# berkeley-hipie/HIPIE

Measured on AMD Instinct MI355X. Metric: images/sec @1024x1024 ViT-H bs=8 (single-image inference hot path: box, class and mask logits), higher is better.
Workload: dtype f16x3 (split-fp16 operands, fp32 accumulate: fp32-class); 1 GPU; BASELINE.json configs[2]: vit_huge, 1024x1024, batch 8 per GPU, 80 class prompts (L=194), detection; global_batch=8, parallelism=dp1, precision_policy=split, launch=eager

## Files before the change

### hipie_amd/_lib.py

```python
import ctypes
import os

_HERE = os.path.dirname(os.path.abspath(__file__))
LIB_PATH = os.environ.get("HIPIE_LIB_PATH") or os.path.join(_HERE, "csrc", "libhipie_mi355.so")

c_p = ctypes.c_void_p
c_i = ctypes.c_int
c_l = ctypes.c_int64
c_f = ctypes.c_float

SIGNATURES = {
    "hipie_version": [],
    "hipie_last_error": [],
    "hipie_msda_forward": [c_p, c_p, c_p, c_p, c_p, c_p] + [c_i] * 8 + [c_p],
    "hipie_msda_fused_forward": [c_p, c_p, c_p, c_p, c_p, c_p, c_p] + [c_i] * 10 + [c_l, c_l, c_p],
    "hipie_msda_fused_forward_strided": [c_p, c_l, c_p, c_p, c_p, c_p, c_p, c_p] + [c_i] * 10 + [c_l, c_l, c_p],
    "hipie_flash_attn": [c_p, c_p, c_p, c_p] + [c_i] * 5 + [c_l] * 12 + [c_p, c_p, c_i, c_i, c_p, c_f, c_f, c_i, c_p],
    "hipie_vit_attn": [c_p, c_p, c_p, c_p] + [c_i] * 5 + [c_f, c_i, c_p],
    "hipie_vit_attn_fused": [c_p, c_p, c_p, c_p] + [c_i] * 5 + [c_f, c_i, c_p],
    "hipie_vit_attn_rel": [c_p, c_p, c_p, c_p] + [c_i] * 7 + [c_p],
    "hipie_bi_xattn": [c_p, c_p, c_p, c_p, c_p, c_p, c_p] + [c_i] * 5 + [c_f, c_i, c_p],
    "hipie_bi_xattn_ws": [c_p, c_p, c_p, c_p, c_p, c_p, c_p, c_p, c_l] + [c_i] * 5 + [c_f, c_i, c_p],
    "hipie_bi_xattn_workspace": [c_i] * 5,
    "hipie_mask_einsum": [c_p, c_p, c_p] + [c_i] * 6 + [c_p],
    "hipie_mask_einsum_workspace": [c_i, c_i, c_i],
    "hipie_mask_einsum_ws": [c_p, c_p, c_p, c_p, c_p, c_l] + [c_i] * 6 + [c_p],
    "hipie_mask_einsum16": [c_p, c_p, c_p, c_p, c_p] + [c_i] * 6 + [c_p],
    "hipie_dynamic_mask": [c_p, c_p, c_p, c_p] + [c_i] * 7 + [c_p],
    "hipie_dynamic_mask16": [c_p, c_p, c_p, c_p] + [c_i] * 7 + [c_p],
    "hipie_dynamic_mask_backward": [c_p] * 7 + [c_i] * 6 + [c_p],
    "hipie_vit_relpos": [c_p, c_p, c_p, c_p, c_p] + [c_i] * 6 + [c_p],
    "hipie_add_layernorm": [c_p, c_p, c_p, c_p, c_p, c_p, c_l, c_i, c_f, c_i, c_i, c_i, c_p],
    "hipie_layernorm_backward": [c_p] * 8 + [c_l, c_l, c_i, c_f, c_p],
    "hipie_layernorm_backward_ws_bytes": [c_l, c_i],
    "hipie_act_forward": [c_p, c_p, c_l, c_i, c_i, c_p],
    "hipie_act_backward": [c_p] * 6 + [c_l, c_i, c_i, c_p],
    "hipie_act_backward_ws_bytes": [c_l, c_i],
    "hipie_add_layernorm_sum": [c_p, c_p, c_p, c_p, c_p, c_p, c_p, c_p, c_l, c_i, c_f, c_i, c_i, c_i, c_p],
    "hipie_add_layernorm_rows": [c_p, c_p, c_p, c_p, c_p, c_p, c_l, c_i, c_f, c_i, c_i, c_i, c_p, c_p, c_p],
    "hipie_batched_nms": [c_p, c_p, c_p, c_p, c_p, c_i, c_i, c_f, c_i, c_p],
    "hipie_mask_finalize": [c_p, c_i, c_p] + [c_i] * 8 + [c_f, c_p, c_p],
    "hipie_sem_pan": [c_p] * 8 + [c_i] * 11 + [c_p],
    "hipie_sine_embed": [c_p, c_p, c_p, c_l, c_i, c_i, c_i, c_f, c_i, c_p],
    "hipie_box_refine": [c_p, c_p, c_p, c_l, c_f, c_i, c_p],
    "hipie_ref_point_mlp": [c_p, c_p, c_p, c_p, c_p, c_p, c_p, c_l, c_i, c_f, c_i, c_p],
    "hipie_box_head": [c_p, c_p, c_p, c_p, c_p, c_p, c_p, c_p, c_p, c_l, c_f, c_p],
    "hipie_add_layernorm_dec": [c_p, c_p, c_p, c_p, c_p, c_p, c_p, c_p, c_l, c_i, c_f, c_i, c_i, c_p],
    "hipie_add_cast": [c_p, c_p, c_p, c_l, c_i, c_p],
    "hipie_group_norm": [c_p, c_p, c_p, c_p, c_p, c_p, c_i, c_i, c_i, c_i, c_i, c_f, c_i, c_i, c_i, c_p],
    "hipie_gemm": [c_p, c_l, c_p, c_l, c_p, c_p, c_l, c_p, c_l, c_p] + [c_i] * 6 + [c_f, c_f, c_p],
    "hipie_gemm_f8x": [c_p, c_l, c_p, c_l, c_p, c_p, c_p, c_l, c_p, c_l, c_p] + [c_i] * 6 + [c_f, c_f, c_p],
    "hipie_to_f8x": [c_p, c_l, c_p, c_l, c_p, c_l, c_i, c_p],
    "hipie_gemm_ln": [c_p, c_l, c_p, c_l, c_p, c_p, c_l, c_p, c_p, c_f, c_p, c_l, c_p, c_l, c_i, c_i, c_i, c_f, c_p],
    "hipie_gemm_gather": [c_p, c_l, c_l, c_p, c_p, c_l, c_p, c_p, c_l, c_p, c_l, c_p] + [c_i] * 6 + [c_f, c_f, c_p],
    "hipie_vit_attn_split": [c_p, c_p, c_p, c_p] + [c_i] * 5 + [c_p],
    "hipie_msda_backward": [c_p] * 9 + [c_i] * 8 + [c_p],
    "hipie_msda_backward_ws": [c_p] * 9 + [c_i] * 8 + [c_p, c_l, c_p],
    "hipie_msda_backward_workspace": [c_i] * 6,
    "hipie_gemm_batched": [c_p, c_l, c_l, c_l, c_p, c_l, c_l, c_l, c_p, c_l, c_l, c_l] + [c_i] * 6 + [c_f, c_p],
    "hipie_gemm_batched_softmax_bias": [c_p, c_l, c_l, c_l, c_p, c_l, c_l, c_l, c_p, c_l, c_l, c_l] + [c_i] * 5 + [c_p, c_i, c_p, c_f, c_f, c_p],
    "hipie_gemm_batched_resid": [c_p, c_l, c_l, c_l, c_p, c_l, c_l, c_l, c_p, c_p, c_l, c_l, c_l, c_p, c_l, c_l, c_l] + [c_i] * 5 + [c_f, c_p],
    "hipie_gemm_batched_softmax": [c_p, c_l, c_l, c_l, c_p, c_l, c_l, c_l, c_p, c_l, c_l, c_l] + [c_i] * 5 + [c_p, c_i, c_f, c_f, c_p],
    "hipie_softmax_hl8": [c_p, c_l, c_p, c_l, c_l, c_i, c_i, c_p, c_l, c_f, c_p],
    "hipie_attn_f32": [c_p] * 5 + [c_i] * 5 + [c_l] * 6 + [c_f, c_p],
    "hipie_attn_split": [c_p] * 5 + [c_i] * 5 + [c_l] * 6 + [c_f, c_p],
    "hipie_attn_f32_rows": [c_p] * 5 + [c_i] * 5 + [c_l] * 6 + [c_f, c_p],
    "hipie_attn_split_rows": [c_p] * 5 + [c_i] * 5 + [c_l] * 6 + [c_f, c_p],
    "hipie_conv3x3_split": [c_p, c_l, c_p, c_p, c_p, c_l, c_l] + [c_i] * 6 + [c_p],
    "hipie_ffn_fused": [c_p, c_l, c_p, c_p, c_p, c_p, c_p, c_l, c_i, c_i, c_i, c_p],
    "hipie_topk": [c_p, c_l, c_i, c_i, c_i, c_p, c_p, c_p],
    "hipie_fill_rows": [c_p, c_l, c_p, c_l, c_p, c_l, c_p],
    "hipie_to_hl8": [c_p, c_l, c_p, c_l, c_l, c_i, c_i, c_f, c_p],
    "hipie_to_hl8_t": [c_p, c_l, c_p, c_l, c_l, c_i, c_l, c_f, c_p],
    "hipie_attn_train_forward": [c_p] * 8 + [c_i, c_i, c_p],
    "hipie_to_f16_pair": [c_p, c_l, c_p, c_p, c_l, c_i, c_i, c_p, c_p],
    "hipie_attn_train_backward": [c_p] * 13 + [c_i, c_i, c_p],
    "hipie_selftest": [c_i, c_p, c_p, c_p, c_p],
}

_lib = None


class HipieLibraryError(RuntimeError):
    pass


def load():
    global _lib
    if _lib is not None:
        return _lib
    if not os.path.exists(LIB_PATH):
        raise HipieLibraryError(
            "libhipie_mi355.so not found at %s -- build it with `make -C hipie_amd/csrc` (hipcc, gfx950). "
            "There is no PyTorch fallback for the hand-written kernels." % LIB_PATH)
    import torch
    try:
        lib = ctypes.CDLL(LIB_PATH)
    except OSError as e:
        raise HipieLibraryError("cannot load %s: %s" % (LIB_PATH, e))
    for name, argtypes in SIGNATURES.items():
        try:
            fn = getattr(lib, name)
        except AttributeError:
            raise HipieLibraryError("%s does not export %s (stale build?)" % (LIB_PATH, name))
        fn.argtypes = argtypes
        fn.restype = (ctypes.c_char_p if name == "hipie_last_error" else
                      ctypes.c_int64 if name in ("hipie_bi_xattn_workspace", "hipie_mask_einsum_workspace", "hipie_msda_backward_workspace",
                                                      "hipie_layernorm_backward_ws_bytes", "hipie_act_backward_ws_bytes") else ctypes.c_int)
    _lib = lib
    return lib


def check(rc, what):
    if rc != 0:
        msg = load().hipie_last_error()
        raise RuntimeError("%s failed (rc=%d): %s" % (what, rc, msg.decode() if msg else ""))
```

### hipie_amd/csrc/gemm.hip

```cpp
#include "gemm_tile.h"

namespace hipie {

template <typename T>
__global__ __launch_bounds__(256) void to_hl8_kernel(const T* __restrict__ x, f16_t* __restrict__ out, long rows, int K, long ldx, long ldo,
                                                     float scale) {
  const long gid = (long)blockIdx.x * 256 + threadIdx.x;
  const int gpr = K / 8;
  if (gid >= rows * gpr) return;
  const long r = gid / gpr;
  const int g = (int)(gid - r * gpr);
  const T* src = x + r * ldx + 8 * g;
  f16x8 h, l;
#pragma unroll
  for (int e = 0; e < 8; ++e) {
    f16_t hh, ll;
    hl_split((float)src[e] * scale, hh, ll);
    h[e] = hh;
    l[e] = ll;
  }
  f16_t* dst = out + r * ldo + 16 * g;
  *reinterpret_cast<f16x8*>(dst) = h;
  *reinterpret_cast<f16x8*>(dst + 8) = l;
}


constexpr int kTrRows = 128, kTrCols = 64;
__global__ __launch_bounds__(256) void to_hl8_t_kernel(const float* __restrict__ x, f16_t* __restrict__ out, long rows, int C, long ldx,
                                                       long ldo, long rows_p, float scale) {
  __shared__ float tile[kTrRows][kTrCols + 1];
  const long r0 = (long)blockIdx.x * kTrRows;
  const int c0 = blockIdx.y * kTrCols;
  const int tid = threadIdx.x;
  for (int k = tid; k < kTrRows * (kTrCols / 4); k += 256) {
    const int i = k / (kTrCols / 4), j = (k % (kTrCols / 4)) * 4;
    float v[4] = {0.f, 0.f, 0.f, 0.f};
    if (r0 + i < rows) {
      const float* src = x + (r0 + i) * ldx + c0 + j;
      if (c0 + j + 3 < C && (((uintptr_t)src) & 15) == 0) {
        const float4 q = *reinterpret_cast<const float4*>(src);
        v[0] = q.x; v[1] = q.y; v[2] = q.z; v[3] = q.w;
      } else {
        for (int e = 0; e < 4; ++e) v[e] = c0 + j + e < C ? src[e] : 0.f;
      }
    }
    for (int e = 0; e < 4; ++e) tile[i][j + e] = v[e];
  }
  __syncthreads();
  for (int u = tid; u < kTrCols * (kTrRows / 8); u += 256) {
    const int g = u % (kTrRows / 8), c = u / (kTrRows / 8);
    const long m = r0 + 8 * g;
    if (c0 + c >= C || m >= rows_p) continue;
    f16x8 h, l;
#pragma unroll
    for (int e = 0; e < 8; ++e) {
      f16_t hh, ll;
      hl_split(tile[8 * g + e][c] * scale, hh, ll);
      h[e] = hh;
      l[e] = ll;
    }
    f16_t* dst = out + (long)(c0 + c) * ldo + 2 * m;
    *reinterpret_cast<f16x8*>(dst) = h;
    *reinterpret_cast<f16x8*>(dst + 8) = l;
  }
}

}

using namespace hipie;

namespace hipie {
int launch_gemm_k256(const void* X, long ldx_b, int x_f32, const void* W, long ldw_b, const float* bias, float* out, long ldo, int M, int N,
                     hipStream_t st);
}

static int gemm_impl(const void* A, int64_t lda, const void* W, int64_t ldw, const float* bias, const float* resid, int64_t ldr,
                     void* out, int64_t ldo, const int32_t* out_row, const int32_t* a_row, int64_t a_rows, int M, int N, int K, int in_fmt,
                     int out_fmt, int act, float alpha, float oscale, void* stream) {
  HIPIE_REQUIRE(A && W && out, "gemm: null pointer");
  HIPIE_REQUIRE(in_fmt == HIPIE_F16 || in_fmt == HIPIE_HL8 || in_fmt == HIPIE_F32, "gemm: operand format %d (HIPIE_F16 | HIPIE_HL8 | HIPIE_F32)",
                in_fmt);
  HIPIE_REQUIRE(out_fmt == HIPIE_F32 || out_fmt == HIPIE_F16 || out_fmt == HIPIE_HL8, "gemm: output format %d", out_fmt);
  HIPIE_REQUIRE(act >= 0 && act <= 3, "gemm: activation %d (0 none, 1 gelu, 2 relu, 3 quick-gelu)", act);
  HIPIE_REQUIRE(M > 0 && N > 0 && K > 0 && N % 8 == 0, "gemm: M=%d N=%d K=%d (N must be a multiple of 8)", M, N, K);
  const bool a_f32 = in_fmt == HIPIE_F32;
  const bool split = in_fmt == HIPIE_HL8 || a_f32;
  if (a_f32) lda *= 2;
  const int kq = split ? 32 : 64;
  HIPIE_REQUIRE(K % kq == 0, "gemm: K=%d must be a multiple of %d", K, kq);
  const int epr = split ? 2 * K : K;
  HIPIE_TRY(gm_check_operands("gemm", lda, ldw, epr, 320));
  HIPIE_TRY(gm_check_out("gemm", ldo, out_fmt, N));
  HIPIE_TRY(gm_check_resid("gemm", resid, ldr, N));
  HIPIE_TRY(gm_check_aligned("gemm", {A, W, out, bias, resid}));
  GemmParams p;
  gm_set_operands(p, A, lda, W, ldw, M, N, K, kq);
  p.bias = bias; p.resid = resid; p.ldr = ldr; p.out = (char*)out; p.ldo = ldo; p.out_row = out_row; p.a_row = a_row;
  p.out_fmt = out_fmt; p.act = act; p.alpha = alpha; p.oscale = oscale;
  hipStream_t st = (hipStream_t)stream;
  static const int k256_mode = [] { const char* e = study_env("HIPIE_GEMM_K256"); return e ? atoi(e) : 2; }();
  const bool k256_on = k256_mode == 1 || (k256_mode == 2 && N >= 384);
  if (k256_on && split && K == 256 && out_fmt == HIPIE_F32 && act == 0 && resid == nullptr && out_row == nullptr && a_row == nullptr &&
      alpha == 1.f && oscale == 1.f && N % 32 == 0 && M >= 8192 && ldw * 2 == 1024 && (long)M * p.lda_b < (1L << 32))
    return launch_gemm_k256(A, p.lda_b, a_f32 ? 1 : 0, W, p.ldw_b, bias, (float*)out, ldo, M, N, st);
  const bool wide = (N % 320 == 0);
  static const int small_on = [] { const char* e = study_env("HIPIE_GEMM_SMALL"); return e ? atoi(e) : 1; }();
  static const long small_tiles = [] { const char* e = study_env("HIPIE_GEMM_SMALL_MAXTILES"); return e ? atol(e) : 96L; }();
  const bool small_ok = small_on && (long)((M + 255) / 256) * ((N + (wide ? 319 : 255)) / (wide ? 320 : 256)) < small_tiles;
#ifdef HIPIE_GEMM_VARIANTS
  { const char* e = study_env("HIPIE_GEMM_VARIANT"); const int v = e ? atoi(e) : 0;
    if (split && wide && v == 1) return launch_gemm<320, true, 1>(p, st);
    if (split && wide && v == 3) return launch_gemm<320, true, 3>(p, st); }
  { const char* e = study_env("HIPIE_GEMM_VARIANT"); if (e) p.variant = atoi(e); }
  p.prio_mode = gemm2_prio();
  if (split && gemm2_mode() == 4) {
    const bool w160 = (N % 160 == 0);
    if (a_f32) return w160 ? launch_gemm4<5, 2>(p, st) : launch_gemm4<4, 2>(p, st);
    return w160 ? launch_gemm4<5, 0>(p, st) : launch_gemm4<4, 0>(p, st);
  }
  if (split && gemm2_mode() == 2) {
    const bool w160 = (N % 160 == 0);
    if (a_f32) return w160 ? launch_gemm3<5, 2>(p, st) : launch_gemm3<4, 2>(p, st);
    return w160 ? launch_gemm3<5, 0>(p, st) : launch_gemm3<4, 0>(p, st);
  }
  if (split && gemm2_mode() == 1) {
    const bool w160 = (N % 160 == 0);
    if (a_f32) return w160 ? launch_gemm2<5, 2>(p, st) : launch_gemm2<4, 2>(p, st);
    return w160 ? launch_gemm2<5, 0>(p, st) : launch_gemm2<4, 0>(p, st);
  }
#endif
  if (split && small_ok && a_row == nullptr) return a_f32 ? launch_gemm_small<2>(p, st) : launch_gemm_small<0>(p, st);
  if (a_f32) return wide ? launch_gemm<320, true, 2>(p, st) : launch_gemm<256, true, 2>(p, st);
  if (split) return wide ? launch_gemm<320, true>(p, st) : launch_gemm<256, true>(p, st);
  return wide ? launch_gemm<320, false>(p, st) : launch_gemm<256, false>(p, st);
}

extern "C" int hipie_gemm(const void* A, int64_t lda, const void* W, int64_t ldw, const float* bias, const float* resid, int64_t ldr,
                          void* out, int64_t ldo, const int32_t* out_row, int M, int N, int K, int in_fmt, int out_fmt, int act, float alpha,
                          float oscale, void* stream) {
  return gemm_impl(A, lda, W, ldw, bias, resid, ldr, out, ldo, out_row, nullptr, 0, M, N, K, in_fmt, out_fmt, act, alpha, oscale, stream);
}

extern "C" int hipie_gemm_gather(const void* A, int64_t lda, int64_t a_rows, const int32_t* a_row, const void* W, int64_t ldw, const float* bias,
                                 const float* resid, int64_t ldr, void* out, int64_t ldo, const int32_t* out_row, int M, int N, int K, int in_fmt,
                                 int out_fmt, int act, float alpha, float oscale, void* stream) {
  HIPIE_REQUIRE(a_row != nullptr && a_rows > 0, "gemm_gather: a_row map / operand row count missing");
  HIPIE_REQUIRE(in_fmt == HIPIE_HL8 || in_fmt == HIPIE_F32, "gemm_gather: split operands only (HIPIE_HL8 | HIPIE_F32 rows)");
  HIPIE_REQUIRE((long)a_rows * lda * (in_fmt == HIPIE_F32 ? 4 : 2) < (1L << 32), "gemm_gather: the gathered operand must stay below 4 GiB");
  return gemm_impl(A, lda, W, ldw, bias, resid, ldr, out, ldo, out_row, a_row, a_rows, M, N, K, in_fmt, out_fmt, act, alpha, oscale, stream);
}

extern "C" int hipie_gemm_batched(const void* A, int64_t lda, int64_t a_outer, int64_t a_inner, const void* W, int64_t ldw, int64_t w_outer,
                                  int64_t w_inner, void* out, int64_t ldo, int64_t o_outer, int64_t o_inner, int n_outer, int n_inner, int M,
                                  int N, int K, int out_fmt, float alpha, void* stream) {
  HIPIE_REQUIRE(A && W && out, "gemm_batched: null pointer");
  HIPIE_REQUIRE(out_fmt == HIPIE_F32 || out_fmt == HIPIE_HL8, "gemm_batched: output format %d (HIPIE_F32 | HIPIE_HL8)", out_fmt);
  HIPIE_REQUIRE(M > 0 && N > 0 && K > 0 && N % 8 == 0 && K % 32 == 0, "gemm_batched: M=%d N=%d K=%d (N %% 8, K %% 32)", M, N, K);
  HIPIE_TRY(gm_check_batch_shape("gemm_batched", n_outer, n_inner));
  HIPIE_TRY(gm_check_operands("gemm_batched", lda, ldw, 2 * K, 320));
  HIPIE_TRY(gm_check_out("gemm_batched", ldo, out_fmt, N));
  HIPIE_TRY(gm_check_batch_offsets("gemm_batched", a_outer, a_inner, w_outer, w_inner, o_outer, o_inner));
  HIPIE_TRY(gm_check_aligned("gemm_batched", {A, W, out}));
  GemmParams p;
  gm_set_operands(p, A, lda, W, ldw, M, N, K);
  gm_set_batch(p, n_inner, a_outer, a_inner, w_outer, w_inner, o_outer, o_inner, out_fmt == HIPIE_F32 ? 4 : 2);
  p.out = (char*)out; p.ldo = ldo; p.out_fmt = out_fmt; p.alpha = alpha;
  hipStream_t st = (hipStream_t)stream;
  const int batches = n_outer * n_inner;
#ifdef HIPIE_GEMM_VARIANTS
  if (gemm2_mode() == 1) return (N % 160 == 0) ? launch_gemm2<5, 0>(p, st, batches) : launch_gemm2<4, 0>(p, st, batches);
#endif
  return (N % 320 == 0) ? launch_gemm<320, true>(p, st, batches) : launch_gemm<256, true>(p, st, batches);
}

extern "C" int hipie_gemm_batched_resid(const void* A, int64_t lda, int64_t a_outer, int64_t a_inner, const void* W, int64_t ldw, int64_t w_outer,
                                        int64_t w_inner, const float* bias, const float* resid, int64_t ldr, int64_t r_outer, int64_t r_inner,
                                        float* out, int64_t ldo, int64_t o_outer, int64_t o_inner, int n_outer, int n_inner, int M, int N, int K,
                                        float alpha, void* stream) {
  HIPIE_REQUIRE(A && W && out, "gemm_batched_resid: null pointer");
  HIPIE_REQUIRE(M > 0 && N > 0 && K > 0 && N % 8 == 0 && K % 32 == 0, "gemm_batched_resid: M=%d N=%d K=%d (N %% 8, K %% 32)", M, N, K);
  HIPIE_TRY(gm_check_batch_shape("gemm_batched_resid", n_outer, n_inner));
  HIPIE_TRY(gm_check_operands("gemm_batched_resid", lda, ldw, 2 * K, 320));
  HIPIE_TRY(gm_check_out("gemm_batched_resid", ldo, HIPIE_F32, N));
  HIPIE_REQUIRE(resid == nullptr || (ldr >= N && ldr % 4 == 0 && ((r_outer | r_inner) % 4) == 0), "gemm_batched_resid: residual strides %ld / %ld / %ld",
                (long)ldr, (long)r_outer, (long)r_inner);
  HIPIE_TRY(gm_check_batch_offsets("gemm_batched_resid", a_outer, a_inner, w_outer, w_inner, o_outer, o_inner));
  HIPIE_TRY(gm_check_aligned("gemm_batched_resid", {A, W, out, bias, resid}));
  GemmParams p;
  gm_set_operands(p, A, lda, W, ldw, M, N, K);
  gm_set_batch(p, n_inner, a_outer, a_inner, w_outer, w_inner, o_outer, o_inner, 4);
  p.out = (char*)out; p.ldo = ldo; p.alpha = alpha;
  p.bias = bias; p.resid = resid; p.ldr = ldr; p.r_bo = r_outer; p.r_bi = r_inner;
  return (N % 320 == 0) ? launch_gemm<320, true>(p, (hipStream_t)stream, n_outer * n_inner) : launch_gemm<256, true>(p, (hipStream_t)stream, n_outer * n_inner);
}

extern "C" int hipie_gemm_batched_softmax(const void* A, int64_t lda, int64_t a_outer, int64_t a_inner, const void* W, int64_t ldw, int64_t w_outer,
                                          int64_t w_inner, void* out, int64_t ldo, int64_t o_outer, int64_t o_inner, int n_outer, int n_inner,
                                          int M, int N, int K, const unsigned char* mask, int L, float clamp, float alpha, void* stream) {
  HIPIE_REQUIRE(A && W && out, "gemm_batched_softmax: null pointer");
  HIPIE_REQUIRE(M > 0 && N > 0 && N <= 256 && N % 8 == 0 && K > 0 && K % 32 == 0 && L > 0 && L <= N,
                "gemm_batched_softmax: M=%d N=%d K=%d L=%d (N <= 256: the row must fit one column tile)", M, N, K, L);
  HIPIE_TRY(gm_check_batch_shape("gemm_batched_softmax", n_outer, n_inner));
  HIPIE_TRY(gm_check_operands("gemm_batched_softmax", lda, ldw, 2 * K, 320));
  HIPIE_TRY(gm_check_out("gemm_batched_softmax", ldo, HIPIE_HL8, N));
  HIPIE_TRY(gm_check_batch_offsets("gemm_batched_softmax", a_outer, a_inner, w_outer, w_inner, o_outer, o_inner));
  HIPIE_TRY(gm_check_aligned("gemm_batched_softmax", {A, W, out}));
  GemmParams p;
  gm_set_operands(p, A, lda, W, ldw, M, N, K);
  gm_set_batch(p, n_inner, a_outer, a_inner, w_outer, w_inner, o_outer, o_inner, 2);
  p.out = (char*)out; p.ldo = ldo; p.out_fmt = HIPIE_HL8; p.alpha = alpha;
  p.softmax = 1; p.sm_L = L; p.sm_clamp = clamp; p.sm_mask = mask;
  return launch_gemm<256, true>(p, (hipStream_t)stream, n_outer * n_inner);
}

extern "C" int hipie_conv3x3_split(const void* x, int64_t ldx, const void* w, const float* bias, void* out, int64_t ldo, int64_t rows, int Wp,
                                   int C, int N, int in_fmt, int out_fmt, int act, void* stream) {
  HIPIE_REQUIRE(x && w && out, "conv3x3_split: null pointer");
  HIPIE_REQUIRE(in_fmt == HIPIE_HL8 || in_fmt == HIPIE_F32, "conv3x3_split: input format %d (HIPIE_HL8 | HIPIE_F32 rows)", in_fmt);
  HIPIE_REQUIRE(out_fmt == HIPIE_F32 || out_fmt == HIPIE_HL8, "conv3x3_split: output format %d (HIPIE_F32 | HIPIE_HL8)", out_fmt);
  HIPIE_REQUIRE(act >= 0 && act <= 2, "conv3x3_split: activation %d", act);
  HIPIE_REQUIRE(rows > 0 && rows < (1L << 31) && Wp >= 3 && C > 0 && C % 32 == 0 && N > 0 && N % 8 == 0, "conv3x3_split: rows=%ld Wp=%d C=%d N=%d",
                (long)rows, Wp, C, N);
  if (in_fmt == HIPIE_F32) ldx *= 2;
  HIPIE_REQUIRE(ldx >= 2 * C && ldx % 8 == 0, "conv3x3_split: input row stride %ld", (long)ldx);
  HIPIE_REQUIRE((long)(256 + Wp + 2) * ldx * 2 < (1L << 31), "conv3x3_split: row stride too large");
  HIPIE_TRY(gm_check_out("conv3x3_split", ldo, out_fmt, N));
  HIPIE_TRY(gm_check_aligned("conv3x3_split", {x, w, out, bias}));
  GemmParams p;
  gm_set_operands(p, x, ldx, w, (long)2 * 9 * C, (int)rows, N, 9 * C);
  p.bias = bias; p.out = (char*)out; p.ldo = ldo; p.out_fmt = out_fmt; p.act = act;
  p.conv_kpt = C / 32; p.conv_wp = Wp;
  hipStream_t st = (hipStream_t)stream;
  const bool wide = (N % 320 == 0);
  if (in_fmt == HIPIE_F32) return wide ? launch_gemm<320, true, 2>(p, st) : launch_gemm<256, true, 2>(p, st);
  return wide ? launch_gemm<320, true>(p, st) : launch_gemm<256, true>(p, st);
}

extern "C" int hipie_to_hl8(const void* x, int64_t ldx, void* out, int64_t ldo, int64_t rows, int K, int x_dtype, float scale, void* stream) {
  HIPIE_REQUIRE(x && out && rows > 0 && K > 0 && K % 8 == 0, "to_hl8: rows=%ld K=%d (K must be a multiple of 8)", (long)rows, K);
  HIPIE_REQUIRE(ldx >= K && ldo >= 2 * K && ldo % 8 == 0, "to_hl8: row strides %ld / %ld", (long)ldx, (long)ldo);
  const long n = rows * (K / 8);
  const dim3 grid((unsigned)((n + 255) / 256));
  hipStream_t st = (hipStream_t)stream;
  switch (x_dtype) {
    case HIPIE_F32: hipLaunchKernelGGL(to_hl8_kernel<float>, grid, dim3(256), 0, st, (const float*)x, (f16_t*)out, rows, K, ldx, ldo, scale); break;
    case HIPIE_F16: hipLaunchKernelGGL(to_hl8_kernel<f16_t>, grid, dim3(256), 0, st, (const f16_t*)x, (f16_t*)out, rows, K, ldx, ldo, scale); break;
    default: return set_err(HIPIE_EINVAL, "to_hl8: dtype %d", x_dtype);
  }
  return check_launch("to_hl8");
}

extern "C" int hipie_to_hl8_t(const void* x, int64_t ldx, void* out, int64_t ldo, int64_t rows, int C, int64_t rows_p, float scale, void* stream) {
  HIPIE_REQUIRE(x && out && rows > 0 && C > 0, "to_hl8_t: rows=%ld C=%d", (long)rows, C);
  HIPIE_REQUIRE(rows_p >= rows && rows_p % 8 == 0 && ldx >= C && ldo >= 2 * rows_p && ldo % 8 == 0, "to_hl8_t: rows_p=%ld (>= rows, multiple of 8), strides %ld / %ld",
                (long)rows_p, (long)ldx, (long)ldo);
  HIPIE_REQUIRE(((uintptr_t)out % 16) == 0, "to_hl8_t: output must be 16-byte aligned");
  const long tiles_r = (rows_p + kTrRows - 1) / kTrRows, tiles_c = (C + kTrCols - 1) / kTrCols;
  HIPIE_REQUIRE(tiles_c <= 65535, "to_hl8_t: C=%d too wide", C);
  hipLaunchKernelGGL(to_hl8_t_kernel, dim3((unsigned)tiles_r, (unsigned)tiles_c), dim3(256), 0, (hipStream_t)stream, (const float*)x, (f16_t*)out,
                     (long)rows, C, (long)ldx, (long)ldo, (long)rows_p, scale);
  return check_launch("to_hl8_t");
}
```

### hipie_amd/csrc/groupnorm.hip

```cpp
#include "common.h"

namespace hipie {

constexpr int GN_CPG = 8;
constexpr int GN_MAXK = 512;

template <typename T> struct V8 {
  static __device__ __forceinline__ void ld(const T* p, float (&v)[8]) {
    typedef T t8 __attribute__((ext_vector_type(8)));
    const t8 r = *reinterpret_cast<const t8*>(p);
#pragma unroll
    for (int i = 0; i < 8; ++i) v[i] = (float)r[i];
  }
  static __device__ __forceinline__ void st(T* p, const float (&v)[8]) {
    typedef T t8 __attribute__((ext_vector_type(8)));
    t8 r;
#pragma unroll
    for (int i = 0; i < 8; ++i) r[i] = (T)v[i];
    *reinterpret_cast<t8*>(p) = r;
  }
};

template <typename T>
__global__ __launch_bounds__(256) void gn_stats_nhwc_kernel(const T* __restrict__ x, const float* __restrict__ prebias,
                                                            float* __restrict__ part, int HW, int G, int nchunk, int per) {
  __shared__ float red[2][256];
  const int b = blockIdx.y, chunk = blockIdx.x;
  const int g = threadIdx.x % G, pl = threadIdx.x / G, npl = 256 / G;
  const int C = G * GN_CPG;
  float pb[8];
#pragma unroll
  for (int i = 0; i < 8; ++i) pb[i] = prebias ? prebias[g * 8 + i] : 0.f;
  const int p1 = min(HW, (chunk + 1) * per);
  const float K = (float)x[(long)b * HW * C + g * 8] + pb[0];
  float s = 0.f, ss = 0.f;
  for (int p = chunk * per + pl; p < p1; p += npl) {
    float v[8];
    V8<T>::ld(x + ((long)b * HW + p) * C + g * 8, v);
#pragma unroll
    for (int i = 0; i < 8; ++i) { const float a = v[i] + pb[i] - K; s += a; ss = fmaf(a, a, ss); }
  }
  red[0][threadIdx.x] = s;
  red[1][threadIdx.x] = ss;
  __syncthreads();
  if (threadIdx.x < G) {
    for (int k = 1; k < npl; ++k) { s += red[0][threadIdx.x + k * G]; ss += red[1][threadIdx.x + k * G]; }
    float* o = part + (((long)b * G + g) * nchunk + chunk) * 2;
    o[0] = s; o[1] = ss;
  }
}

template <typename T, typename OutT>
__global__ __launch_bounds__(256) void gn_apply_nhwc_kernel(const T* __restrict__ x, const float* __restrict__ prebias,
                                                            const float* __restrict__ part, const float* __restrict__ gamma,
                                                            const float* __restrict__ beta, OutT* __restrict__ out, int HW, int G,
                                                            int nchunk, int per, float eps, int relu) {
  __shared__ float stat[2][64];
  const int b = blockIdx.y, chunk = blockIdx.x;
  const int g = threadIdx.x % G, pl = threadIdx.x / G, npl = 256 / G;
  const int C = G * GN_CPG;
  if (threadIdx.x < G) {
    float s = 0.f, ss = 0.f;
    const float* pp = part + ((long)b * G + threadIdx.x) * nchunk * 2;
    for (int k = 0; k < nchunk; ++k) { s += pp[2 * k]; ss += pp[2 * k + 1]; }
    const float n = (float)HW * GN_CPG;
    const float ms = s / n;
    const float K = (float)x[(long)b * HW * C + threadIdx.x * 8] + (prebias ? prebias[threadIdx.x * 8] : 0.f);
    stat[0][threadIdx.x] = K + ms;
    stat[1][threadIdx.x] = rsqrtf(fmaxf(ss / n - ms * ms, 0.f) + eps);
  }
  __syncthreads();
  const float mean = stat[0][g], rstd = stat[1][g];
  float sc[8], sh[8];
#pragma unroll
  for (int i = 0; i < 8; ++i) {
    sc[i] = rstd * gamma[g * 8 + i];
    sh[i] = beta[g * 8 + i] + ((prebias ? prebias[g * 8 + i] : 0.f) - mean) * sc[i];
  }
  const int p1 = min(HW, (chunk + 1) * per);
  for (int p = chunk * per + pl; p < p1; p += npl) {
    const long off = ((long)b * HW + p) * C + g * 8;
    float v[8];
    V8<T>::ld(x + off, v);
#pragma unroll
    for (int i = 0; i < 8; ++i) { v[i] = fmaf(v[i], sc[i], sh[i]); if (relu) v[i] = fmaxf(v[i], 0.f); }
    V8<OutT>::st(out + off, v);
  }
}

constexpr int GN_TP = 64;
template <typename T, typename OutT>
__global__ __launch_bounds__(256) void gn_apply_nhwc_to_nchw_kernel(const T* __restrict__ x, const float* __restrict__ prebias,
                                                                    const float* __restrict__ part, const float* __restrict__ gamma,
                                                                    const float* __restrict__ beta, OutT* __restrict__ out, int HW, int G,
                                                                    int nchunk, float eps, int relu) {
  extern __shared__ __attribute__((aligned(16))) float gn_tile[];
  __shared__ float stat[2][64];
  const int b = blockIdx.y, p0 = blockIdx.x * GN_TP;
  const int g = threadIdx.x % G, pl = threadIdx.x / G, npl = 256 / G;
  const int C = G * GN_CPG;
  if (threadIdx.x < G) {
    float s = 0.f, ss = 0.f;
    const float* pp = part + ((long)b * G + threadIdx.x) * nchunk * 2;
    for (int k = 0; k < nchunk; ++k) { s += pp[2 * k]; ss += pp[2 * k + 1]; }
    const float n = (float)HW * GN_CPG;
    const float ms = s / n;
    const float K = (float)x[(long)b * HW * C + threadIdx.x * 8] + (prebias ? prebias[threadIdx.x * 8] : 0.f);
    stat[0][threadIdx.x] = K + ms;
    stat[1][threadIdx.x] = rsqrtf(fmaxf(ss / n - ms * ms, 0.f) + eps);
  }
  __syncthreads();
  const float mean = stat[0][g], rstd = stat[1][g];
  float sc[8], sh[8];
#pragma unroll
  for (int i = 0; i < 8; ++i) {
    sc[i] = rstd * gamma[g * 8 + i];
    sh[i] = beta[g * 8 + i] + ((prebias ? prebias[g * 8 + i] : 0.f) - mean) * sc[i];
  }
  for (int p = pl; p < GN_TP; p += npl) {
    float v[8];
    V8<T>::ld(x + ((long)b * HW + p0 + p) * C + g * 8, v);
#pragma unroll
    for (int i = 0; i < 8; ++i) {
      v[i] = fmaf(v[i], sc[i], sh[i]);
      if (relu) v[i] = fmaxf(v[i], 0.f);
      gn_tile[(g * 8 + i) * (GN_TP + 1) + p] = v[i];
    }
  }
  __syncthreads();
  struct alignas(sizeof(OutT) * 4) Pack { OutT v[4]; };
  const int q = threadIdx.x & 15, cr = threadIdx.x >> 4;
  for (int c = cr; c < C; c += 16) {
    Pack o;
#pragma unroll
    for (int i = 0; i < 4; ++i) o.v[i] = elem<OutT>::from_f32(gn_tile[c * (GN_TP + 1) + 4 * q + i]);
    *reinterpret_cast<Pack*>(out + ((long)b * C + c) * HW + p0 + 4 * q) = o;
  }
}

template <typename T>
__global__ __launch_bounds__(256) void gn_stats_nchw_kernel(const T* __restrict__ x, const float* __restrict__ prebias,
                                                            float* __restrict__ part, int HW, int C, int nchunk, int per) {
  __shared__ float red[2][4];
  const int bc = blockIdx.y, chunk = blockIdx.x;
  const int c = bc % C, b = bc / C;
  const float pb = prebias ? prebias[c] : 0.f;
  const T* xp = x + (long)bc * HW;
  const int e1 = min(HW, (chunk + 1) * per);
  const int c0 = (c / GN_CPG) * GN_CPG;
  const float K = (float)x[((long)b * C + c0) * HW] + (prebias ? prebias[c0] : 0.f);
  float s = 0.f, ss = 0.f;
  for (int e = chunk * per + threadIdx.x * 8; e < e1; e += 256 * 8) {
    float v[8];
    V8<T>::ld(xp + e, v);
#pragma unroll
    for (int i = 0; i < 8; ++i) { const float a = v[i] + pb - K; s += a; ss = fmaf(a, a, ss); }
  }
#pragma unroll
  for (int o = 32; o > 0; o >>= 1) { s += __shfl_xor(s, o); ss += __shfl_xor(ss, o); }
  if ((threadIdx.x & 63) == 0) { red[0][threadIdx.x >> 6] = s; red[1][threadIdx.x >> 6] = ss; }
  __syncthreads();
  if (threadIdx.x == 0) {
    const int G = C / GN_CPG, g = c / GN_CPG, K = nchunk * GN_CPG;
    float* o = part + (((long)b * G + g) * K + (c % GN_CPG) * nchunk + chunk) * 2;
    o[0] = red[0][0] + red[0][1] + red[0][2] + red[0][3];
    o[1] = red[1][0] + red[1][1] + red[1][2] + red[1][3];
  }
}

template <typename T, typename OutT>
__global__ __launch_bounds__(256) void gn_apply_nchw_kernel(const T* __restrict__ x, const float* __restrict__ prebias,
                                                            const float* __restrict__ part, const float* __restrict__ gamma,
                                                            const float* __restrict__ beta, OutT* __restrict__ out, int HW, int C,
                                                            int nchunk, int per, float eps, int relu) {
  __shared__ float stat[2];
  const int bc = blockIdx.y, chunk = blockIdx.x;
  const int c = bc % C, b = bc / C;
  if (threadIdx.x < 64) {
    const int G = C / GN_CPG, g = c / GN_CPG, K = nchunk * GN_CPG;
    const float* pp = part + ((long)b * G + g) * K * 2;
    float s = 0.f, ss = 0.f;
    for (int k = threadIdx.x; k < K; k += 64) { s += pp[2 * k]; ss += pp[2 * k + 1]; }
#pragma unroll
    for (int o = 32; o > 0; o >>= 1) { s += __shfl_xor(s, o); ss += __shfl_xor(ss, o); }
    if (threadIdx.x == 0) {
      const float n = (float)HW * GN_CPG;
      const float ms = s / n;
      const int c0 = g * GN_CPG;
      const float K = (float)x[((long)b * C + c0) * HW] + (prebias ? prebias[c0] : 0.f);
      stat[0] = K + ms;
      stat[1] = rsqrtf(fmaxf(ss / n - ms * ms, 0.f) + eps);
    }
  }
  __syncthreads();
  const float sc = stat[1] * gamma[c];
  const float sh = beta[c] + ((prebias ? prebias[c] : 0.f) - stat[0]) * sc;
  const T* xp = x + (long)bc * HW;
  OutT* op = out + (long)bc * HW;
  const int e1 = min(HW, (chunk + 1) * per);
  for (int e = chunk * per + threadIdx.x * 8; e < e1; e += 256 * 8) {
    float v[8];
    V8<T>::ld(xp + e, v);
#pragma unroll
    for (int i = 0; i < 8; ++i) { v[i] = fmaf(v[i], sc, sh); if (relu) v[i] = fmaxf(v[i], 0.f); }
    V8<OutT>::st(op + e, v);
  }
}

template <typename T, typename OutT>
static int launch_gn(const void* x, const float* prebias, const float* gamma, const float* beta, void* out, float* part, int B,
                     int C, int HW, int nhwc, float eps, int relu, hipStream_t st) {
  const int G = C / GN_CPG;
  if (nhwc) {
    const int npl = 256 / G;
    int nchunk = max(1, min(64, HW / (npl * 16)));
    const int per = (HW + nchunk - 1) / nchunk;
    nchunk = (HW + per - 1) / per;
    hipLaunchKernelGGL((gn_stats_nhwc_kernel<T>), dim3(nchunk, B), dim3(256), 0, st, (const T*)x, prebias, part, HW, G, nchunk, per);
    if (nhwc == 2) {
      const size_t lds = (size_t)C * (GN_TP + 1) * sizeof(float);
      auto kern = gn_apply_nhwc_to_nchw_kernel<T, OutT>;
      static LdsLimit limit;
      limit.raise((const void*)kern, lds);
      hipLaunchKernelGGL(kern, dim3(HW / GN_TP, B), dim3(256), lds, st, (const T*)x, prebias, part, gamma, beta, (OutT*)out, HW, G, nchunk,
                         eps, relu);
      return check_launch("group_norm");
    }
    hipLaunchKernelGGL((gn_apply_nhwc_kernel<T, OutT>), dim3(nchunk, B), dim3(256), 0, st, (const T*)x, prebias, part, gamma, beta,
                       (OutT*)out, HW, G, nchunk, per, eps, relu);
  } else {
    int nchunk = max(1, min(GN_MAXK / GN_CPG, HW / 8192));
    int per = (HW + nchunk - 1) / nchunk;
    per = (per + 7) / 8 * 8;
    nchunk = (HW + per - 1) / per;
    hipLaunchKernelGGL((gn_stats_nchw_kernel<T>), dim3(nchunk, B * C), dim3(256), 0, st, (const T*)x, prebias, part, HW, C, nchunk, per);
    hipLaunchKernelGGL((gn_apply_nchw_kernel<T, OutT>), dim3(nchunk, B * C), dim3(256), 0, st, (const T*)x, prebias, part, gamma,
                       beta, (OutT*)out, HW, C, nchunk, per, eps, relu);
  }
  return check_launch("group_norm");
}

template <typename T>
static int gn_out(int od, const void* x, const float* prebias, const float* gamma, const float* beta, void* out, float* part, int B,
                  int C, int HW, int nhwc, float eps, int relu, hipStream_t st) {
  switch (od) {
    case HIPIE_F32: return launch_gn<T, float>(x, prebias, gamma, beta, out, part, B, C, HW, nhwc, eps, relu, st);
    case HIPIE_F16: return launch_gn<T, f16_t>(x, prebias, gamma, beta, out, part, B, C, HW, nhwc, eps, relu, st);
    case HIPIE_BF16: return launch_gn<T, bf16_t>(x, prebias, gamma, beta, out, part, B, C, HW, nhwc, eps, relu, st);
    default: return set_err(HIPIE_EINVAL, "group_norm: bad out dtype %d", od);
  }
}

}

extern "C" int hipie_group_norm(const void* x, const float* prebias, const float* gamma, const float* beta, void* out,
                                float* workspace, int B, int C, int HW, int groups, int channels_last, float eps, int relu,
                                int x_dtype, int out_dtype, void* stream) {
  using namespace hipie;
  HIPIE_REQUIRE(x && gamma && beta && out && workspace, "group_norm: null pointer");
  HIPIE_REQUIRE(B >= 0 && C > 0 && HW > 0, "group_norm: bad shape");
  HIPIE_REQUIRE(groups > 0 && C == groups * GN_CPG && groups <= 64 && 256 % groups == 0,
                "group_norm: %d channels in %d groups unsupported (8 channels per group, 256 %% groups == 0)", C, groups);
  HIPIE_REQUIRE(channels_last || HW % 8 == 0, "group_norm: NCHW needs H*W %% 8 == 0 (got %d)", HW);
  HIPIE_REQUIRE(channels_last >= 0 && channels_last <= 2 && (channels_last != 2 || HW % 64 == 0),
                "group_norm: channels_last %d (0 NCHW, 1 channels-last, 2 channels-last in / NCHW out: H*W %% 64 == 0, got %d)", channels_last, HW);
  if (B == 0) return HIPIE_OK;
  hipStream_t st = (hipStream_t)stream;
  switch (x_dtype) {
    case HIPIE_F32: return gn_out<float>(out_dtype, x, prebias, gamma, beta, out, workspace, B, C, HW, channels_last, eps, relu, st);
    case HIPIE_F16: return gn_out<f16_t>(out_dtype, x, prebias, gamma, beta, out, workspace, B, C, HW, channels_last, eps, relu, st);
    case HIPIE_BF16: return gn_out<bf16_t>(out_dtype, x, prebias, gamma, beta, out, workspace, B, C, HW, channels_last, eps, relu, st);
    default: return set_err(HIPIE_EINVAL, "group_norm: bad x dtype %d", x_dtype);
  }
}
```

### hipie_amd/modeling/ddetrs_dn.py

```python
import torch
import torch.nn as nn
import torch.nn.functional as F

from .. import ops
from .maskdino import MaskDINOHead
from .transformer import (MLP, FeatureResizer, NestedTensor, PConv2d, _get_clones, agg_lang_feat, expand_tokens, geo_cached, inverse_sigmoid,
                          nested_tensor_from_images)


_SIDE_STREAMS = {}


def _side_stream(device):
    key = str(device)
    st = _SIDE_STREAMS.get(key)
    if st is None:
        st = _SIDE_STREAMS[key] = torch.cuda.Stream(device=device)
    return st


class MaskHeadSmallConv(nn.Module):

    def __init__(self, dim, context_dim):
        super().__init__()
        self.lay1 = PConv2d(dim, dim // 4, 3, padding=1)
        self.lay2 = PConv2d(dim // 4, dim // 32, 3, padding=1)
        self.lay3 = PConv2d(context_dim, context_dim, 3, padding=1)
        self.lay4 = PConv2d(context_dim, context_dim, 3, padding=1)
        self.jia_dcn = PConv2d(context_dim, context_dim, 3, padding=1)

    def forward(self, x, fpns=None):
        f = F.relu(self.lay3(x[-1]))
        f = x[-2] + F.interpolate(f, size=x[-2].shape[-2:], mode="nearest")
        f = F.relu(self.lay4(f))
        f = x[-3] + F.interpolate(f, size=x[-3].shape[-2:], mode="nearest")
        f = F.relu(self.jia_dcn(f))
        f = F.relu(self.lay1(f))
        return F.relu(self.lay2(f))


class DDETRSegmUniDN(nn.Module):
    def __init__(self, detr, cfg, precision):
        super().__init__()
        self.detr = detr
        d = cfg.hidden_dim
        self.mask_out_stride = cfg.mask_stride
        self.up_rate = 8 // cfg.mask_stride
        self.num_gen_params = 169
        self.controller = MLP(d, d, self.num_gen_params, cfg.ctrl_layers)
        self.mask_head = MaskHeadSmallConv(d, d)
        self.resizer = FeatureResizer(cfg.lang_dim, d)
        self.mask_dino = MaskDINOHead(cfg, detr.backbone.num_channels, precision)
        self.mask_logit_dtype = precision.act
        self.mask_mlp_dtype = "split" if getattr(precision, "split", False) else (
            precision.head if precision.head in (torch.float16, torch.bfloat16) else None)
        self.feature_keys = ["res3", "res4", "res5"]
        self.mask_dino_cls_embed = _get_clones(self.detr.class_embed[0], cfg.md_dec_layers + 2)
        self.cfg = cfg
        import os
        self.overlap_branches = os.environ.get("HIPIE_BRANCH_STREAMS", "1") != "0"

    def post_process_maskdino(self, outputs, language_feat, idx=-1):
        outputs["pred_logits"] = self.mask_dino_cls_embed[idx](outputs["pred_logits"], language_feat)
        return outputs

    def coco_inference(self, samples, gt_targets=None, criterion=None, train=False, language_dict_features=None,
                       task=None, bg_queries_lang=None):
        assert not train
        image_sizes = samples.image_sizes
        if not isinstance(samples, NestedTensor):
            div = getattr(self.detr.backbone[0].backbone, "size_divisibility", 32)
            samples = nested_tensor_from_images(list(samples), size_divisibility=div, stacked=getattr(samples, "tensor", None))
        features, pos = self.detr.backbone(samples)
        features_maskdino = {k: v.tensors for k, v in zip(self.feature_keys, features)}
        overlap = self.overlap_branches and features[0].tensors.is_cuda
        if overlap:
            main, side = torch.cuda.current_stream(), _side_stream(features[0].tensors.device)
            side.wait_stream(main)
            with torch.cuda.stream(side):
                outputs_maskdino, _ = self.mask_dino(features_maskdino)
        if task in ("grounding", "sot"):
            lang_feat_pool = agg_lang_feat(language_dict_features["hidden"], language_dict_features["masks"]).unsqueeze(1)
        elif task != "detection":
            raise ValueError("task must be detection or grounding")
        srcs, masks, poses = [], [], []
        for l, feat in enumerate(features):
            src, mask = feat.decompose()
            srcs.append(self.detr.input_proj[l](src))
            masks.append(mask)
            poses.append(pos[l])
        gk = samples.geo_key
        for l in range(len(features), self.detr.num_feature_levels):
            src = self.detr.input_proj[l](features[-1].tensors if l == len(features) else srcs[-1])
            hw = tuple(src.shape[-2:])
            mask = geo_cached(gk, ("level_mask0", hw),
                              lambda: F.interpolate(masks[0][None].float(), size=hw).to(torch.bool)[0])
            srcs.append(src)
            masks.append(mask)
            poses.append(geo_cached(gk, ("pos0", hw, src.dtype), lambda: self.detr.backbone[1](mask).to(src.dtype)))
        hs, memory, init_reference, inter_references, _, _, language_dict_features, spatial_shapes = \
            self.detr.transformer(srcs, masks, poses, language_dict_features, task=task, geo_key=gk)

        lang = lang_feat_pool if task in ("grounding", "sot") else language_dict_features["hidden"]
        if overlap:
            main.wait_stream(side)
        else:
            outputs_maskdino, _ = self.mask_dino(features_maskdino)
        outputs_maskdino = self.post_process_maskdino(outputs_maskdino, lang)
        full_len = None if task in ("grounding", "sot") else language_dict_features.get("full_len")
        outputs_maskdino["pred_logits"] = expand_tokens(outputs_maskdino["pred_logits"], full_len)

        outputs = {}
        lvl = hs.shape[0] - 1
        reference = inverse_sigmoid(init_reference if lvl == 0 else inter_references[lvl - 1])
        outputs["pred_logits"] = expand_tokens(self.detr.class_embed[lvl](hs[lvl], lang), full_len)
        outputs["pred_boxes"] = (self.detr.bbox_embed[lvl](hs[lvl]) + reference).sigmoid()
        outputs["pred_boxious"] = self.detr.iou_head[lvl](hs[lvl])
        outputs["reference_points"] = inter_references[-2, :, :, :2]
        params = self.controller(hs[lvl])
        bs, nq, _ = params.shape
        key = (tuple(image_sizes), str(params.device))
        if getattr(self, "_scale_key", None) != key:
            self._scale = torch.tensor([[float(w), float(h)] for (h, w) in image_sizes], device=params.device)
            self._scale_key = key
        scale = self._scale
        ref_px = (outputs["reference_points"] * scale[:, None, :]).reshape(bs * nq, 2)
        outputs["pred_masks"] = self.forward_mask_head(memory, spatial_shapes, ref_px, params.reshape(bs * nq, -1), bs, nq)
        outputs["pred_masks_maskdino"] = outputs_maskdino["pred_masks"]
        outputs["pred_logits_maskdino"] = outputs_maskdino["pred_logits"]
        outputs["pred_boxes_maskdino"] = outputs_maskdino["pred_boxes"]
        return outputs, None

    def forward_mask_head(self, feats, spatial_shapes, reference_points, mask_head_params, bs, nq):
        c = feats.shape[-1]
        enc, st = [], 0
        for (h, w) in spatial_shapes[:self.detr.num_feature_levels - 1]:
            enc.append(feats[:, st:st + h * w, :].reshape(bs, h, w, c).permute(0, 3, 1, 2))
            st += h * w
        mask_feats = self.mask_head(enc, fpns=None)
        logits = ops.dynamic_mask(mask_feats.float().contiguous(), reference_points.float().contiguous(),
                                  mask_head_params.float().contiguous(), nq, stride=8, up=self.up_rate,
                                  out_dtype=self.mask_logit_dtype, mlp_dtype=self.mask_mlp_dtype)
        return logits.view(bs, nq, 1, logits.shape[-2], logits.shape[-1])
```

### hipie_amd/modeling/maskdino.py

```python
import os

import torch
import torch.nn as nn
import torch.nn.functional as F

from .. import ops
from .transformer import (MLP, _select_topk, DeformableTransformerDecoderLayer, DeformableTransformerEncoderLayer, FeatureResizer, geo_cached, level_pos_flat,
                          PConv2d, PGroupNorm, PLayerNorm, PLinear, PositionEmbeddingSine, _get_clones, encoder_reference_points,
                          gen_encoder_output_proposals, level_tensors,
                          batched_decoder_values, decoder_box_refine, decoder_split_values, selected_proposal_boxes, decoder_fast_path, decoder_query_pos)


class NormConv2d(PConv2d):

    def __init__(self, cin, cout, k, padding=0, relu=False):
        super().__init__(cin, cout, kernel_size=k, padding=padding, bias=False)
        self.norm = PGroupNorm(32, cout)
        self.relu = relu

    def forward(self, x):
        return self.norm(super().forward(x), relu=self.relu)


class FoldedMaskFeatures(object):

    def __init__(self, pre, weight, bias, owner=None):
        self.pre, self.weight, self.bias, self.owner = pre, weight, bias, owner

    def fold(self, e32):
        w, b = self.weight, self.bias
        if self.owner is not None and e32.is_cuda and w.dtype == torch.float32 and ops.split_ok(w.shape[0]):
            cin = w.shape[1]
            y = ops.split_linear(e32.contiguous(), self.owner, "fold_aug", self.owner.weight, None,
                                 weight_fn=lambda: torch.cat([w.float().t(), b.float()[None]], 0), params=[self.owner.weight, self.owner.bias])
            return y[..., :cin].contiguous(), y[..., cin].contiguous()
        return (e32 @ w.float()).contiguous(), e32 @ b.float()


class MSDeformAttnTransformerEncoder(nn.Module):
    def __init__(self, encoder_layer, num_layers):
        super().__init__()
        self.layers = _get_clones(encoder_layer, num_layers)


class MSDeformAttnTransformerEncoderOnly(nn.Module):

    def __init__(self, d_model, nhead, num_layers, dim_feedforward, num_levels, value_dtype):
        super().__init__()
        layer = DeformableTransformerEncoderLayer(d_model, dim_feedforward, num_levels, nhead, 4, value_dtype)
        self.encoder = MSDeformAttnTransformerEncoder(layer, num_layers)
        self.level_embed = nn.Parameter(torch.randn(num_levels, d_model))

    def forward(self, srcs, pos_embeds):
        shapes_list = [tuple(int(v) for v in s.shape[-2:]) for s in srcs]
        src = torch.cat([s.flatten(2).transpose(1, 2) for s in srcs], 1)
        B = src.shape[0]
        gk = ("md_enc", B, tuple(shapes_list), str(src.device), src.dtype)
        pos = level_pos_flat(self, pos_embeds, src.dtype, gk)
        spatial_shapes, level_start_index = level_tensors(shapes_list, src.device)
        refs = geo_cached(gk, "enc_refs", lambda: encoder_reference_points(
            shapes_list, torch.ones(B, len(srcs), 2, device=src.device), src.device))
        q, n = None, len(self.encoder.layers)
        for i, layer in enumerate(self.encoder.layers):
            if i + 1 < n:
                src, q = layer(src, pos, refs, spatial_shapes, level_start_index, None, query=q, want_query=True)
            else:
                src = layer(src, pos, refs, spatial_shapes, level_start_index, None, query=q)
        return src, shapes_list


class MaskDINOEncoder(nn.Module):

    def __init__(self, cfg, in_channels, precision):
        super().__init__()
        cd = cfg.md_conv_dim
        self.input_proj = nn.ModuleList(
            [nn.Sequential(PConv2d(c, cd, kernel_size=1), PGroupNorm(32, cd)) for c in in_channels] +
            [nn.Sequential(PConv2d(max(in_channels), cd, kernel_size=3, stride=2, padding=1), PGroupNorm(32, cd))])
        self.transformer = MSDeformAttnTransformerEncoderOnly(cd, 8, cfg.md_enc_layers, cfg.md_enc_dim_feedforward, 4, precision.value)
        self.pe_layer = PositionEmbeddingSine(cd // 2, offset=0.0)
        self.mask_features = nn.Sequential(nn.ConvTranspose2d(cd, cd, 2, stride=2), PGroupNorm(32, cd), nn.ReLU(),
                                           PConv2d(cd, cfg.md_mask_dim, kernel_size=1))
        self.adapter_1 = NormConv2d(in_channels[0], cd, 1)
        self.layer_1 = NormConv2d(cd, cd, 3, padding=1, relu=True)
        self.precision = precision

    def _mask_features_front(self, z, out_dtype=None):
        ct, gn = self.mask_features[0], self.mask_features[1]
        C = ct.weight.shape[0]
        if getattr(self.precision, "split", False) and z.is_cuda and ct.weight.dtype == torch.float32 and ops.split_ok(C):
            B, _, H, W = z.shape
            wt = ct.weight
            rows = z.permute(0, 2, 3, 1).reshape(B * H * W, C)
            y = ops.convt2x2_split(rows, ct, "convt", wt, None, B, H, W).permute(0, 3, 1, 2)
        else:
            y = F.conv_transpose2d(z.contiguous().to(ct.weight.dtype), ct.weight, None, ct.stride, ct.padding, ct.output_padding, ct.groups, ct.dilation)
        if out_dtype is not None:
            y = y.to(out_dtype)
        return gn(y, relu=True, prebias=ct.bias.float(), out_nchw=True)

    def forward_features(self, features, masks=None):
        f3, f4, f5 = features["res3"], features["res4"], features["res5"]
        extra = self.input_proj[3](f5)
        srcs = [self.input_proj[i](f) for i, f in enumerate((f3, f4, f5))] + [extra]
        pos = [geo_cached(("md_pe", tuple(s.shape[0:1]) + tuple(s.shape[2:]), str(s.device)), "pos", lambda s=s: self.pe_layer(
            torch.zeros(s.shape[0], s.shape[2], s.shape[3], dtype=torch.bool, device=s.device))) for s in srcs]
        y, shapes = self.transformer(srcs, pos)
        B = y.shape[0]
        out, st = [], 0
        y = y.contiguous()
        for (H, W) in shapes:
            out.append(y[:, st:st + H * W].transpose(1, 2).unflatten(2, (H, W)))
            st += H * W
        cur = self.adapter_1(f3)
        top = out[0]
        if tuple(top.shape[-2:]) != tuple(cur.shape[-2:]):
            top = F.interpolate(top, size=cur.shape[-2:], mode="bilinear", align_corners=False)
        z = cur + top
        z = self.layer_1(z)
        if self.precision.einsum >= 3:
            x = self._mask_features_front(z)
            conv = self.mask_features[3]
            mf = FoldedMaskFeatures(x.to(self.precision.act).contiguous(), conv.weight.reshape(conv.weight.shape[0], -1), conv.bias)
        elif self.precision.einsum in (1, 2) and z.is_cuda:
            x = self._mask_features_front(z, torch.float32)
            conv = self.mask_features[3]
            mf = FoldedMaskFeatures(x.float().contiguous(), conv.weight.reshape(conv.weight.shape[0], -1), conv.bias,
                                    owner=conv if getattr(self.precision, "split", False) else None)
        else:
            mf = self.mask_features[3](self._mask_features_front(z, torch.float32))
            mf = mf.float().contiguous()
        return mf, out[0], out


class TransformerDecoder(nn.Module):

    def __init__(self, decoder_layer, num_layers, norm, d_model):
        super().__init__()
        self.layers = _get_clones(decoder_layer, num_layers)
        self.norm = norm
        self.ref_point_head = MLP(2 * d_model, d_model, d_model, 2)
        self.bbox_embed = None


class MaskDINODecoder(nn.Module):

    def __init__(self, cfg, precision):
        super().__init__()
        d = cfg.hidden_dim
        self.num_queries, self.num_layers, self.hidden_dim = cfg.md_num_queries, cfg.md_dec_layers, d
        self.enc_output = PLinear(d, d)
        self.enc_output_norm = PLayerNorm(d)
        self.class_embed = PLinear(d, d)
        self.resizer = FeatureResizer(768, d)
        self.mask_embed = MLP(d, d, cfg.md_mask_dim, 3)
        self.decoder_norm = PLayerNorm(d)
        layer = DeformableTransformerDecoderLayer(d, cfg.md_dim_feedforward, 4, 8, 4, precision.value, precision.attn)
        self.decoder = TransformerDecoder(layer, self.num_layers, self.decoder_norm, d)
        self._bbox_embed = MLP(d, d, 4, 3)
        self.bbox_embed = nn.ModuleList([self._bbox_embed for _ in range(self.num_layers)])
        self.decoder.bbox_embed = self.bbox_embed
        self.precision = precision
        self.pinned_topk = None
        self.last_topk = None
        self.initial_pred_masks = True

    def forward_prediction_heads(self, output, mask_features, pred_mask=True):
        dec = self.decoder_norm(output)
        cls = self.class_embed(dec)
        masks = None
        if pred_mask:
            emb = self.mask_embed(dec)
            if isinstance(mask_features, FoldedMaskFeatures):
                e32 = emb.float()
                pre = mask_features.pre
                ew, eb = mask_features.fold(e32)
                if pre.dtype == torch.float32:
                    masks = ops.mask_einsum(ew, pre, precision=self.precision.einsum, out_dtype=self.precision.act, row_bias=eb)
                elif e32.shape[1] <= 320 and (pre.shape[-1] * pre.shape[-2]) % 8 == 0:
                    masks = ops.mask_einsum16(ew, pre, split=self.precision.einsum == 4, row_bias=eb)
                else:
                    masks = ops.mask_einsum(ew, pre.float().contiguous(), precision=1, out_dtype=self.precision.act)
                    masks = masks + eb.to(masks.dtype)[..., None, None]
            else:
                masks = ops.mask_einsum(emb.float().contiguous(), mask_features, precision=self.precision.einsum,
                                        out_dtype=self.precision.act)
        return cls, masks

    def forward(self, x, mask_features):
        nl = len(x)
        xs = [x[nl - 1 - i] for i in range(nl)]
        shapes_list = [tuple(int(v) for v in t.shape[-2:]) for t in xs]
        src = torch.cat([t.flatten(2).transpose(1, 2) for t in xs], 1)
        B = src.shape[0]
        gk = ("md_dec", B, tuple(shapes_list), str(src.device))
        mask = geo_cached(gk, "mask_flat", lambda: torch.zeros(B, src.shape[1], dtype=torch.bool, device=src.device))
        spatial_shapes, level_start_index = level_tensors(shapes_list, src.device)
        vr2 = geo_cached(gk, "vr2", lambda: torch.ones(B, 1, nl, 4, device=src.device))
        om, prop = gen_encoder_output_proposals(src, mask, shapes_list, gk)
        om = self.enc_output_norm(self.enc_output(om))
        cls_un = self.class_embed(om)
        if self.pinned_topk is not None:
            topk = self.pinned_topk.to(src.device)
        else:
            topk = _select_topk(cls_un.max(-1)[0], self.num_queries)
        self.last_topk = topk
        ref_un = selected_proposal_boxes(self._bbox_embed, om, prop, topk)
        tgt = torch.gather(om, 1, topk.unsqueeze(-1).repeat(1, 1, self.hidden_dim))
        interm_cls, interm_mask = self.forward_prediction_heads(tgt, mask_features, pred_mask=self.initial_pred_masks)
        ref = ref_un.sigmoid()
        sdt = torch.float32
        wdt = self.decoder.ref_point_head.layers[0].weight.dtype
        refs, out, hs = [ref], tgt.to(sdt), []
        layers = self.decoder.layers
        if decoder_fast_path(layers, sdt) and wdt == layers[0].linear1.weight.dtype:
            values = batched_decoder_values(self.decoder, layers, src, None)
            t32 = out.contiguous()
            t16 = t32.to(wdt)
            for lid, layer in enumerate(layers):
                ref_in = ref[:, :, None] * vr2
                qp16 = decoder_query_pos(self.decoder.ref_point_head, ref_in[:, :, 0, :], wdt)
                t32, t16 = layer.forward16(t32, t16, qp16, ref_in, values[lid], spatial_shapes, level_start_index)
                ref = decoder_box_refine(self.decoder.bbox_embed[lid], t32, ref)
                refs.append(ref)
            hs.append(self.decoder.norm(t32).float())
            layers = []
        values = batched_decoder_values(self.decoder, layers, src, None) if layers and decoder_split_values(self.decoder, src) else None
        for lid, layer in enumerate(layers):
            ref_in = ref[:, :, None] * vr2
            query_pos = self.decoder.ref_point_head(ops.sine_embed(ref_in[:, :, 0, :], out_dtype=wdt))
            out = layer(out, query_pos, ref_in, src, spatial_shapes, level_start_index, None, value=None if values is None else values[lid])
            new_ref = ops.box_refine(self.decoder.bbox_embed[lid](out), ref)
            ref = new_ref
            refs.append(new_ref)
            if lid == len(self.decoder.layers) - 1:
                hs.append(self.decoder.norm(out).float())
        cls, masks = self.forward_prediction_heads(hs[-1], mask_features)
        boxes = ops.box_refine(self.bbox_embed[-1](hs[-1]), refs[-2])
        return {"pred_logits": cls, "pred_masks": masks, "pred_boxes": boxes,
                "interm_outputs": {"pred_logits": interm_cls, "pred_masks": interm_mask, "pred_boxes": ref_un.sigmoid()}}


class MaskDINOHead(nn.Module):

    def __init__(self, cfg, in_channels, precision):
        super().__init__()
        self.pixel_decoder = MaskDINOEncoder(cfg, in_channels, precision)
        self.predictor = MaskDINODecoder(cfg, precision)

    def forward(self, features, mask=None):
        mask_features, _, multi_scale = self.pixel_decoder.forward_features(features, mask)
        return self.predictor(multi_scale, mask_features), None
```

### hipie_amd/modeling/transformer.py

```python
import collections
import copy
import os
import math

import torch
import torch.nn as nn
import torch.nn.functional as F

from .. import ops
from ..derived import derived


def _lin(owner, key, x, w, b, act=ops.ACT_NONE, out_fmt=ops.F32, x_hl8=False, rows=None):
    if getattr(owner, "split", False) and x.is_cuda and w.dtype == torch.float32 and ops.split_ok(w.shape[1] if not x_hl8 else w.shape[1]):
        fns = {} if rows is None else dict(weight_fn=lambda: w[rows], bias_fn=lambda: b[rows])
        return ops.split_linear(x, owner, key, w, b, act=act, out_fmt=out_fmt, x_hl8=x_hl8, **fns)
    if rows is not None:
        w, b = w[rows], b[rows]
    y = F.linear(x.to(w.dtype), w, b)
    return F.relu(y) if act == ops.ACT_RELU else y


def set_split(module, on=True):
    for m in module.modules():
        m.split = bool(on)
    return module


class PLinear(nn.Linear):
    out_dtype = torch.float32
    split = False

    def forward(self, x, x_hl8=False, out_fmt=ops.F32):
        if self.split and x.is_cuda and self.weight.dtype == torch.float32 and ops.split_ok(self.in_features):
            return ops.split_linear(x, self, "w", self.weight, self.bias, out_fmt=out_fmt, x_hl8=x_hl8)
        return F.linear(x.to(self.weight.dtype), self.weight, self.bias).to(self.out_dtype)

    def forward_relu(self, x, out_fmt=ops.F32, x_hl8=False):
        if self.split and x.is_cuda and self.weight.dtype == torch.float32 and ops.split_ok(self.in_features):
            return ops.split_linear(x, self, "w", self.weight, self.bias, act=ops.ACT_RELU, out_fmt=out_fmt, x_hl8=x_hl8)
        x = x.to(self.weight.dtype)
        if x.is_cuda and self.bias is not None:
            y = torch._addmm_activation(self.bias, x.reshape(-1, x.shape[-1]), self.weight.t(), use_gelu=False)
            return y.view(*x.shape[:-1], -1).to(self.out_dtype)
        return F.relu(F.linear(x, self.weight, self.bias)).to(self.out_dtype)


class PConv2d(nn.Conv2d):
    out_dtype = torch.float32
    nhwc = False
    split = False

    def forward(self, x):
        if (self.split and x.is_cuda and x.dim() == 4 and self.kernel_size == (1, 1) and self.stride == (1, 1) and self.padding == (0, 0)
                and self.groups == 1 and self.weight.dtype == torch.float32 and ops.split_ok(self.in_channels)):
            xb = x.permute(0, 2, 3, 1)
            if xb.is_contiguous():
                B, H, W, C = xb.shape
                w = self.weight
                y = ops.split_linear(xb.float().reshape(B * H * W, C), self, "w1x1", w, self.bias, weight_fn=lambda: w.reshape(w.shape[0], C))
                return y.view(B, H, W, -1).permute(0, 3, 1, 2).to(self.out_dtype)
        if self.split and ops.conv3x3_split_ok(x, self):
            return ops.conv3x3_split(x, self).to(self.out_dtype)
        x = x.to(self.weight.dtype)
        if self.nhwc:
            x = x.contiguous(memory_format=torch.channels_last)
        return self._conv_forward(x, self.weight, self.bias).to(self.out_dtype)


class PLayerNorm(nn.LayerNorm):

    def forward(self, x):
        C = x.shape[-1]
        if x.is_cuda and C % 4 == 0 and C <= 2048 and self.weight.dtype == torch.float32 and x.dtype in ops._DT:
            return ops.add_layernorm(x.contiguous(), None, self.weight, self.bias, self.eps, x.dtype)[1]
        return F.layer_norm(x, self.normalized_shape, self.weight.to(x.dtype), self.bias.to(x.dtype), self.eps)


class PGroupNorm(nn.GroupNorm):

    def forward(self, x, relu=False, prebias=None, out_nchw=False):
        if self.weight.dtype == torch.float32 and ops.group_norm_ok(x, self.num_groups):
            return ops.group_norm(x, self.num_groups, self.weight, self.bias, self.eps, relu=relu, prebias=prebias, out_nchw=out_nchw)
        if prebias is not None:
            x = x + prebias.view(1, -1, 1, 1).to(x.dtype)
        y = F.group_norm(x, self.num_groups, self.weight.to(x.dtype), self.bias.to(x.dtype), self.eps)
        return F.relu(y) if relu else y


def cast_head(module, dtype, act=torch.float32):
    for m in module.modules():
        if isinstance(m, (PLinear, PConv2d, nn.ConvTranspose2d)):
            m.weight.data = m.weight.data.to(dtype)
            if m.bias is not None:
                m.bias.data = m.bias.data.to(dtype)
            if isinstance(m, (PLinear, PConv2d)):
                m.out_dtype = act
            if isinstance(m, PConv2d) and dtype != torch.float32:
                m.weight.data = m.weight.data.contiguous(memory_format=torch.channels_last)
                m.nhwc = True
        elif isinstance(m, MultiheadAttention):
            m.in_proj_weight.data = m.in_proj_weight.data.to(dtype)
            m.in_proj_bias.data = m.in_proj_bias.data.to(dtype)
    return module


_CONST_CACHE = {}


def level_tensors(shapes_list, device):
    key = (tuple(shapes_list), str(device))
    v = _CONST_CACHE.get(key)
    if v is None:
        ss = torch.as_tensor(shapes_list, dtype=torch.long, device=device)
        v = (ss, torch.cat((ss.new_zeros((1,)), ss.prod(1).cumsum(0)[:-1])))
        _CONST_CACHE[key] = v
    return v


def _add_norm(x, delta, norm):
    x = x.contiguous()
    return ops.add_layernorm(x, delta.to(x.dtype).contiguous(), norm.weight, norm.bias, norm.eps, x.dtype, want_res=False)[1]


def _get_clones(module, n):
    return nn.ModuleList([copy.deepcopy(module) for _ in range(n)])


def inverse_sigmoid(x, eps=1e-5):
    x = x.clamp(min=0, max=1)
    return torch.log(x.clamp(min=eps) / (1 - x).clamp(min=eps))


class MLP(nn.Module):
    def __init__(self, input_dim, hidden_dim, output_dim, num_layers):
        super().__init__()
        self.num_layers = num_layers
        h = [hidden_dim] * (num_layers - 1)
        self.layers = nn.ModuleList(PLinear(n, k) for n, k in zip([input_dim] + h, h + [output_dim]))

    def forward(self, x):
        for i, layer in enumerate(self.layers):
            x = layer.forward_relu(x) if i < self.num_layers - 1 else layer(x)
        return x


class FeatureResizer(nn.Module):
    def __init__(self, input_feat_size, output_feat_size):
        super().__init__()
        self.fc = PLinear(input_feat_size, output_feat_size)
        self.layer_norm = PLayerNorm(output_feat_size, eps=1e-12)

    def forward(self, x):
        return self.layer_norm(self.fc(x))


_GEO_CACHE = collections.OrderedDict()


def geo_cached(geo_key, what, build):
    if geo_key is None:
        return build()
    cache = _GEO_CACHE
    key = (geo_key, what)
    v = cache.get(key)
    if v is None:
        v = build()
        cache[key] = v
        if len(cache) > 512:
            cache.popitem(last=False)
    else:
        cache.move_to_end(key)
    return v


def level_pos_flat(enc, pos_embeds, dtype, geo_key):
    def build():
        return torch.cat([p.flatten(2).transpose(1, 2) + enc.level_embed[i].view(1, 1, -1) for i, p in enumerate(pos_embeds)], 1).to(dtype)
    return build() if geo_key is None else derived(enc, "pos_flat", [enc.level_embed], build, extra=geo_key, keep=32)


class NestedTensor(object):
    def __init__(self, tensors, mask, geo_key=None):
        self.tensors, self.mask, self.geo_key = tensors, mask, geo_key

    def decompose(self):
        return self.tensors, self.mask


def nested_tensor_from_images(images, size_divisibility=32, stacked=None):
    H = max(int(im.shape[1]) for im in images)
    W = max(int(im.shape[2]) for im in images)
    H = (H + size_divisibility - 1) // size_divisibility * size_divisibility
    W = (W + size_divisibility - 1) // size_divisibility * size_divisibility
    dev = images[0].device
    if stacked is not None and tuple(stacked.shape[-2:]) == (H, W) and all(tuple(im.shape[1:]) == (H, W) for im in images):
        geo_key = (tuple((H, W) for _ in images), (H, W), str(dev))
        return NestedTensor(stacked, geo_cached(geo_key, "pixel_mask", lambda: torch.zeros(
            len(images), H, W, dtype=torch.bool, device=dev)), geo_key)
    t = torch.zeros(len(images), 3, H, W, dtype=images[0].dtype, device=dev)
    geo_key = (tuple((int(im.shape[1]), int(im.shape[2])) for im in images), (H, W), str(dev))

    def build_mask():
        m = torch.ones(len(images), H, W, dtype=torch.bool, device=dev)
        for i, im in enumerate(images):
            m[i, :im.shape[1], :im.shape[2]] = False
        return m
    for i, im in enumerate(images):
        t[i, :, :im.shape[1], :im.shape[2]].copy_(im)
    return NestedTensor(t, geo_cached(geo_key, "pixel_mask", build_mask), geo_key)


class PositionEmbeddingSine(nn.Module):

    def __init__(self, num_pos_feats=128, offset=-0.5):
        super().__init__()
        self.num_pos_feats, self.offset = num_pos_feats, offset

    def forward(self, mask):
        not_mask = ~mask
        y = not_mask.cumsum(1, dtype=torch.float32)
        x = not_mask.cumsum(2, dtype=torch.float32)
        y = (y + self.offset) / (y[:, -1:, :] + 1e-6) * (2 * math.pi)
        x = (x + self.offset) / (x[:, :, -1:] + 1e-6) * (2 * math.pi)
        dim_t = torch.arange(self.num_pos_feats, dtype=torch.float32, device=mask.device)
        dim_t = 10000 ** (2 * torch.div(dim_t, 2, rounding_mode="floor") / self.num_pos_feats)
        px, py = x[:, :, :, None] / dim_t, y[:, :, :, None] / dim_t
        px = torch.stack((px[:, :, :, 0::2].sin(), px[:, :, :, 1::2].cos()), dim=4).flatten(3)
        py = torch.stack((py[:, :, :, 0::2].sin(), py[:, :, :, 1::2].cos()), dim=4).flatten(3)
        return torch.cat((py, px), dim=3).permute(0, 3, 1, 2)


class MaskedBackbone(nn.Module):

    def __init__(self, backbone, strides, channels):
        super().__init__()
        self.backbone = backbone
        self.feature_strides, self.num_channels = strides, channels

    def forward(self, tensor_list):
        xs = self.backbone(tensor_list.tensors)
        out = {}
        gk = tensor_list.geo_key
        for name, x in xs.items():
            hw = tuple(x.shape[-2:])
            mask = geo_cached(gk, ("level_mask", hw),
                              lambda: F.interpolate(tensor_list.mask[None].float(), size=hw).to(torch.bool)[0])
            out[name] = NestedTensor(x, mask, gk)
        return out


class Joiner(nn.Sequential):

    def __init__(self, backbone, position_embedding):
        super().__init__(backbone, position_embedding)

    def forward(self, tensor_list):
        xs = self[0](tensor_list)
        out = [x for _, x in sorted(xs.items())]
        pos = [geo_cached(x.geo_key, ("pos", tuple(x.mask.shape), x.tensors.dtype, self[1].offset),
                          lambda x=x: self[1](x.mask).to(x.tensors.dtype)) for x in out]
        return out, pos


class MSDeformAttn(nn.Module):

    def __init__(self, d_model=256, n_levels=4, n_heads=8, n_points=4, value_dtype=torch.float32):
        super().__init__()
        self.d_model, self.n_levels, self.n_heads, self.n_points = d_model, n_levels, n_heads, n_points
        self.sampling_offsets = PLinear(d_model, n_heads * n_levels * n_points * 2)
        self.attention_weights = PLinear(d_model, n_heads * n_levels * n_points)
        self.value_proj = PLinear(d_model, d_model)
        self.output_proj = PLinear(d_model, d_model)
        self.value_dtype = value_dtype

    def project_value(self, input_flatten, input_padding_mask=None, x_hl8=False):
        N, S, _ = input_flatten.shape
        vp = self.value_proj
        value = _lin(vp, "w", input_flatten, vp.weight, vp.bias, x_hl8=x_hl8)
        if input_padding_mask is not None:
            value.masked_fill_(input_padding_mask[..., None], 0.0)
        return value.to(self.value_dtype).view(N, S, self.n_heads, self.d_model // self.n_heads)

    def forward(self, query, reference_points, input_flatten, input_spatial_shapes, input_level_start_index,
                input_padding_mask=None):
        N, Lq, _ = query.shape
        value = self.project_value(input_flatten, input_padding_mask)
        if reference_points.shape[-1] not in (2, 4):
            raise ValueError("Last dim of reference_points must be 2 or 4, but get {} instead.".format(reference_points.shape[-1]))
        w, b = self._fused_proj()
        no = self.n_heads * self.n_levels * self.n_points * 2
        proj = _lin(self, "offlog", query, w, b)
        off = proj[..., :no].unflatten(-1, (self.n_heads, self.n_levels, self.n_points, 2))
        logits = proj[..., no:].unflatten(-1, (self.n_heads, self.n_levels * self.n_points))
        out = ops.msda_fused(value.contiguous(), input_spatial_shapes, input_level_start_index,
                             reference_points.float().contiguous(), off, logits)
        return self.output_proj(out)

    def forward_projected(self, query, reference_points, value, input_spatial_shapes, input_level_start_index, x_hl8=False, project=True):
        w, b = self._fused_proj()
        no = self.n_heads * self.n_levels * self.n_points * 2
        proj = _lin(self, "offlog", query, w, b, x_hl8=x_hl8)
        off = proj[..., :no].unflatten(-1, (self.n_heads, self.n_levels, self.n_points, 2))
        logits = proj[..., no:].unflatten(-1, (self.n_heads, self.n_levels * self.n_points))
        out = ops.msda_fused(value, input_spatial_shapes, input_level_start_index, reference_points.float().contiguous(), off, logits)
        return self.output_proj(out) if project else out

    def _fused_proj(self):
        so, aw = self.sampling_offsets, self.attention_weights
        return derived(self, "fused_proj", (so.weight, aw.weight, so.bias, aw.bias), lambda: (
            torch.cat([so.weight, aw.weight], 0).contiguous(), torch.cat([so.bias, aw.bias], 0).contiguous()))


class BiMultiHeadAttention(nn.Module):

    def __init__(self, v_dim, l_dim, embed_dim, num_heads, attn_dtype):
        super().__init__()
        self.embed_dim, self.num_heads, self.head_dim = embed_dim, num_heads, embed_dim // num_heads
        self.scale = self.head_dim ** (-0.5)
        self.v_proj, self.l_proj = PLinear(v_dim, embed_dim), PLinear(l_dim, embed_dim)
        self.values_v_proj, self.values_l_proj = PLinear(v_dim, embed_dim), PLinear(l_dim, embed_dim)
        self.out_v_proj, self.out_l_proj = PLinear(embed_dim, v_dim), PLinear(embed_dim, l_dim)
        self.attn_dtype = attn_dtype

    def forward(self, v, l, attention_mask_l=None, gamma_v=None, n_keys=None, resid_v=None):
        B, Nv, _ = v.shape
        L = l.shape[1]
        H, hd, dt = self.num_heads, self.head_dim, self.attn_dtype
        wq, bq = self._scaled_q()
        if getattr(self, "split", False) and v.is_cuda and self.v_proj.weight.dtype == torch.float32 and hd % 32 == 0 and ops.split_ok(v.shape[-1]):
            return self._forward_split(v, l, attention_mask_l, gamma_v, wq, bq, n_keys, resid_v)
        self.resid_fused = False
        of = ops.F16 if (getattr(self, "split", False) and dt == torch.float16) else ops.F32
        q = _lin(self, "q_scaled", v, wq, bq, out_fmt=of).to(dt).view(B, Nv, H, hd)
        k = self.l_proj(l, out_fmt=of).to(dt).view(B, L, H, hd)
        vv = self.values_v_proj(v, out_fmt=of).to(dt).view(B, Nv, H, hd)
        vl = self.values_l_proj(l, out_fmt=of).to(dt).view(B, L, H, hd)
        if attention_mask_l is None:
            attention_mask_l = torch.ones(B, L, dtype=torch.uint8, device=v.device)
        ov, ol = ops.bi_xattn(q, k, vv, vl, attention_mask_l != 0, clamp=50000.0, out_f32=getattr(self, "split", False))
        if gamma_v is None:
            return self.out_v_proj(ov), self.out_l_proj(ol)
        wo, bo = self._scaled_out(gamma_v)
        return _lin(self, "out_scaled", ov, wo, bo).to(self.out_v_proj.out_dtype), self.out_l_proj(ol)

    def _forward_split(self, v, l, attention_mask_l, gamma_v, wq, bq, n_keys=None, resid_v=None):
        B, Nv, _ = v.shape
        L = l.shape[1]
        H, hd = self.num_heads, self.head_dim
        if attention_mask_l is None:
            attention_mask_l = torch.ones(B, L, dtype=torch.uint8, device=v.device)
        keep = attention_mask_l != 0
        if ops.bi_i2t_folded_ok(v, L, n_keys):
            return self._forward_folded(v, l, keep, gamma_v, wq, bq, n_keys, resid_v)
        vh = ops.to_hl8(v.float().contiguous())
        q_hl8 = _lin(self, "q_scaled", vh, wq, bq, out_fmt=ops.HL8, x_hl8=True)
        vv16 = self.values_v_proj(vh, x_hl8=True, out_fmt=ops.F16).view(B, Nv, H, hd)
        k32 = self.l_proj(l)
        vl32 = self.values_l_proj(l)
        ov = ops.bi_i2t_split(q_hl8.view(B, Nv, -1), k32.view(B, L, -1), vl32.view(B, L, -1), keep, H, clamp=50000.0, n_keys=n_keys)
        ol = ops.flash_attn(k32.half().view(B, L, H, hd), q_hl8.view(B, Nv, 2 * H * hd), vv16, 1.0, clamp=50000.0, out_f32=True, k_hl8=True)
        self.resid_fused = False
        if gamma_v is None:
            return self.out_v_proj(ov), self.out_l_proj(ol)
        wo, bo = self._scaled_out(gamma_v)
        if resid_v is not None and resid_v.dtype == torch.float32 and resid_v.is_contiguous() and self.out_v_proj.out_dtype == torch.float32:
            self.resid_fused = True
            return ops.split_linear(ov, self, "out_scaled", wo, bo, resid=resid_v), self.out_l_proj(ol)
        return _lin(self, "out_scaled", ov, wo, bo).to(self.out_v_proj.out_dtype), self.out_l_proj(ol)

    def _forward_folded(self, v, l, keep, gamma_v, wq, bq, n_keys, resid_v):
        B, Nv, C = v.shape
        L = l.shape[1]
        H, hd = self.num_heads, self.head_dim
        v = v.contiguous()
        vh = ops.to_hl8(v)
        k32 = self.l_proj(l)
        vl32 = self.values_l_proj(l)
        kh = k32.view(B, L, H, hd).permute(0, 2, 1, 3)
        M = torch.matmul(kh, wq.float().view(1, H, hd, C))
        cb = (kh * bq.float().view(1, H, 1, hd)).sum(-1)
        Lk = L if not n_keys or n_keys >= L else int(n_keys)
        if gamma_v is None:
            wo, bo = self.out_v_proj.weight, self.out_v_proj.bias
        else:
            wo, bo = self._scaled_out(gamma_v)
        fuse_resid = resid_v is not None and resid_v.dtype == torch.float32 and resid_v.is_contiguous() and gamma_v is not None
        ov = ops.bi_i2t_folded(vh, M[:, :, :Lk].contiguous(), cb[:, :, :Lk].contiguous(), vl32[:, :Lk].contiguous(), keep[:, :Lk], H, wo, bo,
                               resid=resid_v if fuse_resid else None, clamp=50000.0)
        self.resid_fused = fuse_resid
        x16 = v.half()
        kx = x16.view(B, Nv, 1, C).expand(B, Nv, H, C)
        q16 = M.half().permute(0, 2, 1, 3)
        olx = ops.flash_attn(q16, kx, kx, 1.0, clamp=50000.0, out_f32=True)
        wv = self.values_v_proj
        ol = torch.einsum("blhc,hec->blhe", olx.view(B, L, H, C), wv.weight.float().view(H, hd, C)).reshape(B, L, H * hd) + wv.bias.float()
        return ov.to(self.out_v_proj.out_dtype), self.out_l_proj(ol)

    def _scaled_out(self, gamma):
        p = self.out_v_proj
        return derived(self, "scaled_out", (p.weight, p.bias, gamma), lambda: (
            (p.weight.float() * gamma.float()[:, None]).to(p.weight.dtype), (p.bias.float() * gamma.float()).to(p.bias.dtype)))

    def _scaled_q(self):
        p = self.v_proj
        return derived(self, "scaled_q", (p.weight, p.bias), lambda: (
            (p.weight.float() * self.scale).to(p.weight.dtype), (p.bias.float() * self.scale).to(p.bias.dtype)))


class BiAttentionBlockForCheckpoint(nn.Module):

    def __init__(self, v_dim, l_dim, embed_dim, num_heads, init_values, attn_dtype):
        super().__init__()
        self.layer_norm_v, self.layer_norm_l = PLayerNorm(v_dim), PLayerNorm(l_dim)
        self.attn = BiMultiHeadAttention(v_dim, l_dim, embed_dim, num_heads, attn_dtype)
        self.gamma_v = nn.Parameter(init_values * torch.ones(v_dim))
        self.gamma_l = nn.Parameter(init_values * torch.ones(l_dim))

    def forward(self, v, l, attention_mask_l=None, task=None, n_keys=None):
        v, l = self.layer_norm_v(v), self.layer_norm_l(l)
        dv, dl = self.attn(v, l, attention_mask_l=attention_mask_l, gamma_v=self.gamma_v, n_keys=n_keys, resid_v=v)
        if self.attn.resid_fused:
            return dv, l + self.gamma_l * dl
        return v + dv.to(v.dtype), l + self.gamma_l * dl


class VLFuse(nn.Module):

    def __init__(self, cfg, precision):
        super().__init__()
        self.b_attn = BiAttentionBlockForCheckpoint(cfg.hidden_dim, cfg.lang_dim, cfg.vl_hidden_dim, 8,
                                                    1.0 / cfg.enc_layers, precision.attn)

    def forward(self, x, task=None):
        lang = x["lang"]
        fv, fl = self.b_attn(x["visual"], lang["hidden"], lang["masks"], task, n_keys=lang.get("n_keys"))
        lang["hidden"] = fl
        return {"visual": fv, "lang": lang}


class DeformableTransformerEncoderLayer(nn.Module):
    def __init__(self, d_model, d_ffn, n_levels, n_heads, n_points, value_dtype):
        super().__init__()
        self.self_attn = MSDeformAttn(d_model, n_levels, n_heads, n_points, value_dtype)
        self.norm1 = PLayerNorm(d_model)
        self.linear1, self.linear2 = PLinear(d_model, d_ffn), PLinear(d_ffn, d_model)
        self.norm2 = PLayerNorm(d_model)

    def forward(self, src, pos, reference_points, spatial_shapes, level_start_index, padding_mask=None, query=None, want_query=False):
        if getattr(self, "split", False) and src.is_cuda and src.dtype == torch.float32 and self.linear1.weight.dtype == torch.float32:
            return self._forward_split(src, pos, reference_points, spatial_shapes, level_start_index, padding_mask, query, want_query)
        q = src + pos if query is None else query
        src2 = self.self_attn(q, reference_points, src, spatial_shapes, level_start_index, padding_mask)
        src = _add_norm(src, src2, self.norm1)
        src2 = self.linear2(self.linear1.forward_relu(src))
        if want_query and src.is_cuda and src.dtype == pos.dtype and src.dtype in ops._DT:
            n = self.norm2
            return ops.add_layernorm_sum(src.contiguous(), src2.to(src.dtype).contiguous(), n.weight, n.bias, n.eps, pos.contiguous())
        out = _add_norm(src, src2, self.norm2)
        return (out, None) if want_query else out


def _enc_layer_forward_split(self, src, pos, reference_points, spatial_shapes, level_start_index, padding_mask, carry, want_query):
    attn = self.self_attn
    src = src.contiguous()
    if isinstance(carry, dict):
        src_h, q_h = carry["src_h"], carry["q_h"]
    elif carry is None:
        src_h, q_h = ops.to_hl8(src), ops.add_to_hl8(src, _pos_hl8(self, pos))
    else:
        src_h, q_h = ops.to_hl8(src), ops.to_hl8(carry)
    value = attn.project_value(src_h, padding_mask, x_hl8=True)
    n, op = self.norm1, attn.output_proj
    if ops.split_linear_ln_ok(src, op.weight, n.weight):
        sampled = attn.forward_projected(q_h, reference_points, value.contiguous(), spatial_shapes, level_start_index, x_hl8=True, project=False)
        src, s_h = ops.split_linear_ln(sampled, op, "w", op.weight, op.bias, src, n.weight, n.bias, n.eps)
    else:
        src2 = attn.forward_projected(q_h, reference_points, value.contiguous(), spatial_shapes, level_start_index, x_hl8=True)
        src, s_h, _ = ops.add_layernorm_dec(src, src2.contiguous(), n.weight, n.bias, n.eps, "hl8", want16=True)
    if ops.ffn_fused_ok(s_h, self.linear1, self.linear2):
        src2 = ops.ffn_fused(s_h, self.linear1, self.linear2)
    else:
        src2 = self.linear2(self.linear1.forward_relu(s_h, out_fmt=ops.HL8, x_hl8=True), x_hl8=True)
    n = self.norm2
    if not want_query:
        return ops.add_layernorm_dec(src, src2, n.weight, n.bias, n.eps, "hl8")[0]
    out, o_h, q_h = ops.add_layernorm_dec(src, src2, n.weight, n.bias, n.eps, "hl8", want16=True, addend=_pos_hl8(self, pos))
    return out, {"src_h": o_h, "q_h": q_h}


def _pos_hl8(layer, pos):
    return derived(layer, "pos_hl8", [pos], lambda: ops.to_hl8(pos.contiguous()))


DeformableTransformerEncoderLayer._forward_split = _enc_layer_forward_split


def encoder_reference_points(spatial_shapes, valid_ratios, device):
    refs = []
    for lvl, (H_, W_) in enumerate(spatial_shapes):
        ref_y, ref_x = torch.meshgrid(torch.linspace(0.5, H_ - 0.5, H_, dtype=torch.float32, device=device),
                                      torch.linspace(0.5, W_ - 0.5, W_, dtype=torch.float32, device=device), indexing="ij")
        ref_y = ref_y.reshape(-1)[None] / (valid_ratios[:, None, lvl, 1] * H_)
        ref_x = ref_x.reshape(-1)[None] / (valid_ratios[:, None, lvl, 0] * W_)
        refs.append(torch.stack((ref_x, ref_y), -1))
    r = torch.cat(refs, 1)
    return r[:, :, None] * valid_ratios[:, None]


class DeformableTransformerEncoderVL(nn.Module):

    def __init__(self, vl_fusion_layer, encoder_layer, num_layers, num_vl_layers):
        super().__init__()
        self.vl_layers = nn.ModuleList([copy.deepcopy(vl_fusion_layer) if i < num_vl_layers else nn.Identity()
                                        for i in range(num_layers)])
        self.layers = _get_clones(encoder_layer, num_layers)
        self.lang_layers = nn.ModuleList([nn.Identity() for _ in range(num_layers)])

    def forward(self, src, shapes_list, spatial_shapes, level_start_index, valid_ratios, pos, padding_mask, lang, task=None,
                geo_key=None):
        output = {"visual": src, "lang": lang}
        refs = geo_cached(geo_key, "enc_refs", lambda: encoder_reference_points(shapes_list, valid_ratios, src.device))
        q, n = None, len(self.layers)
        for i, (vl_layer, layer) in enumerate(zip(self.vl_layers, self.layers)):
            if not isinstance(vl_layer, nn.Identity):
                output = vl_layer(output, task=task)
                q = None
            nxt_plain = i + 1 < n and isinstance(self.vl_layers[i + 1], nn.Identity)
            res = layer(output["visual"], pos, refs, spatial_shapes, level_start_index, padding_mask, query=q, want_query=nxt_plain)
            output["visual"], q = res if nxt_plain else (res, None)
        return output


class MultiheadAttention(nn.Module):

    def __init__(self, d_model, n_heads, attn_dtype=torch.float16):
        super().__init__()
        self.in_proj_weight = nn.Parameter(torch.empty(3 * d_model, d_model))
        self.in_proj_bias = nn.Parameter(torch.zeros(3 * d_model))
        self.out_proj = PLinear(d_model, d_model)
        self.n_heads = n_heads
        self.attn_dtype = attn_dtype
        nn.init.xavier_uniform_(self.in_proj_weight)

    def forward(self, x_qk, x_v):
        B, N, C = x_qk.shape
        w, b = self.in_proj_weight, self.in_proj_bias
        hd = C // self.n_heads
        split = getattr(self, "split", False)
        if split and x_qk.is_cuda and w.dtype == torch.float32 and ops.attn_f32_ok(hd):
            qk = _lin(self, "in_qk", x_qk, w, b, rows=slice(0, 2 * C)).view(B, N, 2, self.n_heads, hd)
            v = _lin(self, "in_v", x_v, w, b, rows=slice(2 * C, None)).view(B, N, self.n_heads, hd)
            return self.out_proj(ops.attn_split(qk[:, :, 0], qk[:, :, 1], v, hd ** -0.5))
        of = ops.F16 if (split and self.attn_dtype == torch.float16) else ops.F32
        qk = _lin(self, "in_qk", x_qk, w, b, out_fmt=of, rows=slice(0, 2 * C)).to(self.attn_dtype).view(B, N, 2, self.n_heads, hd)
        v = _lin(self, "in_v", x_v, w, b, out_fmt=of, rows=slice(2 * C, None)).to(self.attn_dtype).view(B, N, self.n_heads, hd)
        o = ops.flash_attn(qk[:, :, 0], qk[:, :, 1], v, hd ** -0.5, out_f32=split)
        return self.out_proj(o)


class DeformableTransformerDecoderLayer(nn.Module):

    def __init__(self, d_model, d_ffn, n_levels, n_heads, n_points, value_dtype, attn_dtype=torch.float16):
        super().__init__()
        self.cross_attn = MSDeformAttn(d_model, n_levels, n_heads, n_points, value_dtype)
        self.norm1 = PLayerNorm(d_model)
        self.self_attn = MultiheadAttention(d_model, n_heads, attn_dtype)
        self.norm2 = PLayerNorm(d_model)
        self.linear1, self.linear2 = PLinear(d_model, d_ffn), PLinear(d_ffn, d_model)
        self.norm3 = PLayerNorm(d_model)

    def forward(self, tgt, query_pos, reference_points, src, spatial_shapes, level_start_index, src_padding_mask=None, value=None):
        qk = tgt + query_pos
        tgt = _add_norm(tgt, self.self_attn(qk, tgt), self.norm2)
        if value is not None:
            tgt2 = self.cross_attn.forward_projected(tgt + query_pos, reference_points, value, spatial_shapes, level_start_index)
        else:
            tgt2 = self.cross_attn(tgt + query_pos, reference_points, src, spatial_shapes, level_start_index, src_padding_mask)
        tgt = _add_norm(tgt, tgt2, self.norm1)
        tgt2 = self.linear2(self.linear1.forward_relu(tgt))
        return _add_norm(tgt, tgt2, self.norm3)


    def forward16(self, t32, t16, qp16, reference_points, value, spatial_shapes, level_start_index):
        wd = t16.dtype
        sa = self.self_attn(ops.add_cast(t32, qp16), t16)
        n = self.norm2
        t32, _, q16 = ops.add_layernorm_dec(t32, sa, n.weight, n.bias, n.eps, wd, addend=qp16)
        ca = self.cross_attn.forward_projected(q16, reference_points, value, spatial_shapes, level_start_index)
        n = self.norm1
        t32, t16, _ = ops.add_layernorm_dec(t32, ca, n.weight, n.bias, n.eps, wd, want16=True)
        ff = self.linear2(self.linear1.forward_relu(t16))
        n = self.norm3
        t32, t16, _ = ops.add_layernorm_dec(t32, ff, n.weight, n.bias, n.eps, wd, want16=True)
        return t32, t16


def decoder_fast_path(layers, stream_dtype):
    l0 = layers[0]
    wd = l0.linear1.weight.dtype
    return (stream_dtype == torch.float32 and wd in (torch.float16, torch.bfloat16) and l0.cross_attn.value_dtype == wd
            and l0.linear1.out_dtype == wd and l0.linear1.weight.is_cuda)


def decoder_split_values(decoder, src):
    l0 = decoder.layers[0].cross_attn
    return (bool(getattr(decoder, "split", False)) and src.is_cuda and src.dtype == torch.float32 and not torch.is_grad_enabled()
            and l0.value_proj.weight.dtype == torch.float32 and l0.value_dtype == torch.float32)


def batched_decoder_values(owner, layers, src, padding_mask=None):
    ps = [l.cross_attn.value_proj for l in layers]
    w, b = derived(owner, "bv", [t for p in ps for t in (p.weight, p.bias)], lambda: (
        torch.cat([p.weight for p in ps], 0).contiguous(), torch.cat([p.bias for p in ps], 0).contiguous()))
    v = _lin(owner, "bv", src, w, b)
    if padding_mask is not None:
        v.masked_fill_(padding_mask[..., None], 0.0)
    N, S, _ = v.shape
    d, H = ps[0].weight.shape[0], layers[0].cross_attn.n_heads
    return [v[:, :, i * d:(i + 1) * d].unflatten(-1, (H, d // H)) for i in range(len(ps))]


def ref_point_query(ref_point_head, sine):
    l0, l1 = ref_point_head.layers
    h = torch._addmm_activation(l0.bias, sine.reshape(-1, sine.shape[-1]), l0.weight.t(), use_gelu=False)
    return F.linear(h, l1.weight, l1.bias).view(*sine.shape[:-1], -1)


def _fused_heads(module):
    return bool(getattr(module, "split", False))


def decoder_query_pos(ref_point_head, ref, wdt):
    if _fused_heads(ref_point_head) and ops.ref_point_mlp_ok(ref, ref_point_head) and ref_point_head.layers[0].weight.dtype == wdt:
        return ops.ref_point_mlp(ref, ref_point_head)
    return ref_point_query(ref_point_head, ops.sine_embed(ref, out_dtype=wdt))


def decoder_box_refine(bbox_embed, t32, ref):
    if _fused_heads(bbox_embed) and ops.box_head_ok(t32, bbox_embed):
        return ops.box_head(t32, ref, bbox_embed)
    return ops.box_refine(bbox_embed(t32), ref)


def get_sine_pos_embed(pos_tensor, num_pos_feats=128, temperature=10000, exchange_xy=True):
    scale = 2 * math.pi
    dim_t = torch.arange(num_pos_feats, dtype=torch.float32, device=pos_tensor.device)
    dim_t = temperature ** (2 * torch.div(dim_t, 2, rounding_mode="floor") / num_pos_feats)

    def sine_func(x):
        s = x * scale / dim_t
        return torch.stack((s[..., 0::2].sin(), s[..., 1::2].cos()), dim=-1).flatten(-2)
    res = [sine_func(x) for x in pos_tensor.split([1] * pos_tensor.shape[-1], dim=-1)]
    if exchange_xy:
        res[0], res[1] = res[1], res[0]
    return torch.cat(res, dim=-1)


class DeformableTransformerDecoder(nn.Module):

    def __init__(self, embed_dim, decoder_layer, num_layers):
        super().__init__()
        self.layers = _get_clones(decoder_layer, num_layers)
        self.num_layers = num_layers
        self.ref_point_head = MLP(2 * embed_dim, embed_dim, embed_dim, 2)
        self.bbox_embed = None
        self.class_embed = None

    def forward(self, tgt, reference_points, src, spatial_shapes, level_start_index, valid_ratios, src_padding_mask=None):
        sdt = torch.float32
        output, inter, inter_refs = tgt.to(sdt), [], []
        vr2 = torch.cat([valid_ratios, valid_ratios], -1)[:, None]
        wdt = self.ref_point_head.layers[0].weight.dtype
        if decoder_fast_path(self.layers, sdt) and wdt == self.layers[0].linear1.weight.dtype:
            values = batched_decoder_values(self, self.layers, src, src_padding_mask)
            t32 = output.contiguous()
            t16 = t32.to(wdt)
            for lid, layer in enumerate(self.layers):
                ref_in = reference_points[:, :, None] * vr2
                qp16 = decoder_query_pos(self.ref_point_head, ref_in[:, :, 0, :], wdt)
                t32, t16 = layer.forward16(t32, t16, qp16, ref_in, values[lid], spatial_shapes, level_start_index)
                reference_points = decoder_box_refine(self.bbox_embed[lid], t32, reference_points)
                inter.append(t32)
                inter_refs.append(reference_points)
            return torch.stack(inter), torch.stack(inter_refs)
        values = batched_decoder_values(self, self.layers, src, src_padding_mask) if decoder_split_values(self, src) else None
        for lid, layer in enumerate(self.layers):
            ref_in = reference_points[:, :, None] * vr2
            query_pos = self.ref_point_head(ops.sine_embed(ref_in[:, :, 0, :], out_dtype=wdt))
            output = layer(output, query_pos, ref_in, src, spatial_shapes, level_start_index, src_padding_mask,
                           value=None if values is None else values[lid])
            new_ref = ops.box_refine(self.bbox_embed[lid](output), reference_points)
            reference_points = new_ref
            inter.append(output)
            inter_refs.append(new_ref)
        return torch.stack(inter).float(), torch.stack(inter_refs)


def gen_encoder_output_proposals(memory, memory_padding_mask, shapes_list, geo_key=None):
    keep, prop = geo_cached(geo_key, ("proposals", tuple(shapes_list)),
                            lambda: _proposal_geometry(memory_padding_mask, shapes_list, memory.shape[0], memory.device))
    return torch.where(keep, memory, memory.new_zeros(())), prop


def _proposal_geometry(memory_padding_mask, shapes_list, N_, device):
    memory = None
    proposals, _cur = [], 0
    for lvl, (H_, W_) in enumerate(shapes_list):
        m = memory_padding_mask[:, _cur:_cur + H_ * W_].view(N_, H_, W_, 1)
        valid_H = torch.sum(~m[:, :, 0, 0], 1)
        valid_W = torch.sum(~m[:, 0, :, 0], 1)
        gy, gx = torch.meshgrid(torch.linspace(0, H_ - 1, H_, dtype=torch.float32, device=device),
                                torch.linspace(0, W_ - 1, W_, dtype=torch.float32, device=device), indexing="ij")
        grid = torch.cat([gx.unsqueeze(-1), gy.unsqueeze(-1)], -1)
        scale = torch.cat([valid_W.unsqueeze(-1), valid_H.unsqueeze(-1)], 1).view(N_, 1, 1, 2)
        grid = (grid.unsqueeze(0).expand(N_, -1, -1, -1) + 0.5) / scale
        wh = torch.ones_like(grid) * 0.05 * (2.0 ** lvl)
        proposals.append(torch.cat((grid, wh), -1).view(N_, -1, 4))
        _cur += H_ * W_
    prop = torch.cat(proposals, 1)
    valid = ((prop > 0.01) & (prop < 0.99)).all(-1, keepdim=True)
    prop = torch.log(prop / (1 - prop))
    prop = prop.masked_fill(memory_padding_mask.unsqueeze(-1), float("inf")).masked_fill(~valid, float("inf"))
    keep = (~memory_padding_mask.unsqueeze(-1)) & valid
    return keep, prop


def get_valid_ratio(mask):
    _, H, W = mask.shape
    vh = torch.sum(~mask[:, :, 0], 1).float() / H
    vw = torch.sum(~mask[:, 0, :], 1).float() / W
    return torch.stack([vw, vh], -1)


def expand_tokens(logits, full_len):
    n = logits.shape[-1]
    if full_len is None or n >= full_len:
        return logits
    out = logits.new_empty(*logits.shape[:-1], full_len)
    out[..., :n] = logits
    out[..., n:] = logits[..., -1:]
    return out


def agg_lang_feat(features, mask):
    return (features * mask.unsqueeze(-1).float()).sum(1) / mask.sum(-1).unsqueeze(-1).float()


class DeformableTransformerVLDINO(nn.Module):

    def __init__(self, cfg, precision):
        super().__init__()
        d = cfg.hidden_dim
        self.d_model, self.nhead = d, cfg.nheads
        self.two_stage_num_proposals = cfg.num_queries
        enc_layer = DeformableTransformerEncoderLayer(d, cfg.dim_feedforward, cfg.num_feature_levels, cfg.nheads,
                                                      cfg.enc_n_points, precision.value)
        self.encoder = DeformableTransformerEncoderVL(VLFuse(cfg, precision), enc_layer, cfg.enc_layers, cfg.num_vl_layers)
        dec_layer = DeformableTransformerDecoderLayer(d, cfg.dim_feedforward, cfg.num_feature_levels, cfg.nheads,
                                                      cfg.dec_n_points, precision.value, precision.attn)
        self.decoder = DeformableTransformerDecoder(d, dec_layer, cfg.dec_layers)
        self.level_embed = nn.Parameter(torch.randn(cfg.num_feature_levels, d))
        self.tgt_embed = nn.Embedding(cfg.num_queries, d)
        self.background_proposals = cfg.num_bg_queries
        if cfg.num_bg_queries > 0:
            self.tgt_embed_bg = nn.Embedding(cfg.num_bg_queries, d)
            self.bg_query_refs = nn.Embedding(cfg.num_bg_queries, 4)
        self.enc_output = PLinear(d, d)
        self.enc_output_norm = PLayerNorm(d)
        self.resizer = FeatureResizer(cfg.lang_dim, d)
        self.pinned_topk = None
        self.last_topk = None

    def forward(self, srcs, masks, pos_embeds, language_dict_features, task=None, geo_key=None):
        shapes_list = [tuple(int(v) for v in s.shape[-2:]) for s in srcs]
        src = torch.cat([s.flatten(2).transpose(1, 2) for s in srcs], 1)
        gk = None if geo_key is None else (geo_key, tuple(shapes_list), src.dtype)
        mask = geo_cached(gk, "mask_flat", lambda: torch.cat([m.flatten(1) for m in masks], 1))
        pos = level_pos_flat(self, pos_embeds, src.dtype, gk)
        spatial_shapes, level_start_index = level_tensors(shapes_list, src.device)
        valid_ratios = geo_cached(gk, "valid_ratios", lambda: torch.stack([get_valid_ratio(m) for m in masks], 1))

        no_pad = geo_key is not None and all(tuple(sz) == tuple(geo_key[1]) for sz in geo_key[0])
        layer_mask = None if no_pad else mask
        enc = self.encoder(src, shapes_list, spatial_shapes, level_start_index, valid_ratios, pos, layer_mask,
                           language_dict_features, task=task, geo_key=gk)
        memory, language_dict_features = enc["visual"], enc["lang"]
        bs = memory.shape[0]
        om, prop = gen_encoder_output_proposals(memory, mask, shapes_list, gk)
        om = self.enc_output_norm(self.enc_output(om))
        nd = self.decoder.num_layers
        enc_cls = self.decoder.class_embed[nd](om, None)
        lazy_boxes = not torch.is_grad_enabled()
        enc_coord = None if lazy_boxes else self.decoder.bbox_embed[nd](om) + prop
        if self.pinned_topk is not None:
            topk = self.pinned_topk.to(src.device)
        else:
            topk = _select_topk(enc_cls[..., 0], self.two_stage_num_proposals)
        self.last_topk = topk
        if lazy_boxes:
            ref = selected_proposal_boxes(self.decoder.bbox_embed[nd], om, prop, topk).sigmoid()
        else:
            ref = torch.gather(enc_coord, 1, topk.unsqueeze(-1).repeat(1, 1, 4)).sigmoid()
        tgt = self.tgt_embed.weight[None].repeat(bs, 1, 1)
        if self.background_proposals > 0:
            tgt = torch.cat([self.tgt_embed_bg.weight[None].repeat(bs, 1, 1), tgt], dim=1)
            ref = torch.cat([self.bg_query_refs.weight[None].repeat(bs, 1, 1), ref], dim=1)
        init_ref = ref
        hs, inter_refs = self.decoder(tgt.float(), ref.float(), memory, spatial_shapes, level_start_index, valid_ratios, layer_mask)
        return hs, memory, init_ref, inter_refs, enc_cls, enc_coord, language_dict_features, shapes_list


def selected_proposal_boxes(bbox_embed, om, prop, topk):
    om_k = torch.gather(om, 1, topk.unsqueeze(-1).expand(-1, -1, om.shape[-1]))
    prop_k = torch.gather(prop.expand(om.shape[0], -1, -1), 1, topk.unsqueeze(-1).expand(-1, -1, prop.shape[-1]))
    return bbox_embed(om_k) + prop_k


def _select_topk(scores, k):
    scores = scores.float().contiguous()
    if not ops.topk_ok(scores, k):
        if scores.is_cuda and not torch.cuda.is_current_stream_capturing():
            return torch.topk(scores, k, dim=1)[1]
        raise RuntimeError("two-stage selection: k=%d of %s scores on %s is outside hipie_topk's range (device tensor, k <= 1024) and "
                           "torch.topk is not usable here (host tensor or hipGraph capture)" % (k, tuple(scores.shape), scores.device))
    return ops.topk(scores, k)


class VL_Align(nn.Module):

    def __init__(self, cfg):
        super().__init__()
        bias_value = -math.log((1 - cfg.prior_prob) / cfg.prior_prob)
        self.dot_product_projection_text = PLinear(cfg.lang_dim, cfg.hidden_dim)
        self.log_scale = nn.Parameter(torch.Tensor([cfg.log_scale]))
        self.bias_lang = nn.Parameter(torch.zeros(cfg.lang_dim))
        self.bias0 = nn.Parameter(torch.Tensor([bias_value]))

    def forward(self, x, embedding):
        embedding = F.normalize(embedding, p=2, dim=-1)
        p = self.dot_product_projection_text
        if (getattr(p, "split", False) and x.is_cuda and x.dim() == 3 and embedding.dim() == 3 and p.weight.dtype == torch.float32
                and ops.split_ok(embedding.shape[-1]) and ops.split_ok(p.weight.shape[0])):
            d = p.weight.shape[0]
            ta = ops.split_linear((embedding * 0.5).contiguous(), self, "tok_aug", p.weight, p.bias,
                                  weight_fn=lambda: torch.cat([p.weight.float(), 2.0 * self.bias_lang.float()[None]], 0),
                                  bias_fn=lambda: torch.cat([p.bias.float(), torch.zeros(1, device=p.bias.device)], 0),
                                  params=[p.weight, p.bias, self.bias_lang])
            tok, bias = ta[..., :d], ta[..., d] + self.bias0
            logit = ops.matmul_nt_batched(x.float(), tok.contiguous()) / self.log_scale.exp() + bias.unsqueeze(1)
            return logit.clamp(max=50000).clamp(min=-50000)
        tok = p(embedding / 2.0)
        bias = torch.matmul(embedding, self.bias_lang) + self.bias0
        logit = torch.matmul(x, tok.transpose(-1, -2)) / self.log_scale.exp() + bias.unsqueeze(1)
        return logit.clamp(max=50000).clamp(min=-50000)


class Still_Classifier(nn.Module):
    def __init__(self, hidden_dim):
        super().__init__()
        self.body = PLinear(hidden_dim, 1)

    def forward(self, x, lang_feat=None):
        return self.body(x)


def input_proj_list(channels, hidden_dim, num_levels):
    lst = [nn.Sequential(PConv2d(c, hidden_dim, kernel_size=1), PGroupNorm(32, hidden_dim)) for c in channels]
    c = channels[-1]
    for _ in range(num_levels - len(channels)):
        lst.append(nn.Sequential(PConv2d(c, hidden_dim, kernel_size=3, stride=2, padding=1), PGroupNorm(32, hidden_dim)))
        c = hidden_dim
    return nn.ModuleList(lst)


class DeformableDETRDINO(nn.Module):

    def __init__(self, backbone, transformer, cfg):
        super().__init__()
        self.transformer = transformer
        d = cfg.hidden_dim
        num_pred = cfg.dec_layers + 1
        self.class_embed = _get_clones(VL_Align(cfg), num_pred)
        self.bbox_embed = _get_clones(MLP(d, d, 4, 3), num_pred)
        self.iou_head = _get_clones(PLinear(d, 1), num_pred - 1)
        self.num_feature_levels = cfg.num_feature_levels
        self.input_proj = input_proj_list(backbone.num_channels, d, cfg.num_feature_levels)
        self.backbone = backbone
        self.transformer.decoder.bbox_embed = self.bbox_embed
        self.transformer.decoder.class_embed = self.class_embed
        self.transformer.decoder.class_embed[-1] = Still_Classifier(d)
```

### hipie_amd/ops.py

```python
import torch

from . import _lib
from .derived import derived

_DT = {torch.float32: 0, torch.float16: 1, torch.bfloat16: 2}
F32, F16, BF16, HL8 = 0, 1, 2, 4
OUT_F32 = 0x100
K_HL8_HI = 0x200


class _Profile(object):

    def __init__(self):
        self.tags, self.events = set(), {}
        self.shapes = False

    def enable(self, *tags):
        self.tags, self.events = set(tags), {}

    def disable(self):
        self.tags = set()

    def begin(self, tag):
        if tag not in self.tags and "all" not in self.tags:
# ... 418 lines not shown

@_timed("mask_einsum")
def mask_einsum(mask_embed, mask_features, precision=1, out_dtype=torch.float32, row_bias=None, workspace=True):
    lib = _lib.load()
    B, Q, C = mask_embed.shape
    _, _, Hh, Ww = mask_features.shape
    out = torch.empty(B, Q, Hh, Ww, dtype=out_dtype, device=mask_embed.device)
    e, f = _chk(mask_embed, "mask_embed", torch.float32), _chk(mask_features, "mask_features", torch.float32)
    if int(precision) == 0 or not workspace:
        if row_bias is not None:
            raise RuntimeError("mask_einsum: row_bias needs precision 1 | 2 and the workspace form")
        rc = lib.hipie_mask_einsum(e, f, out.data_ptr(), B, Q, C, Hh * Ww, int(precision), _DT[out_dtype], _stream())
    else:
        rb = None
        if row_bias is not None:
            rbt = row_bias.float().contiguous()
            if tuple(rbt.shape) != (B, Q):
                raise ValueError("mask_einsum: row_bias must be (B, Q) = (%d, %d), got %s" % (B, Q, tuple(rbt.shape)))
            rb = _chk(rbt, "row_bias", torch.float32)
        need = int(lib.hipie_mask_einsum_workspace(B, Q, C))
        ws = _ME_WS.get(need, mask_embed.device)
        rc = lib.hipie_mask_einsum_ws(e, f, rb, out.data_ptr(), ws.data_ptr(), need, B, Q, C, Hh * Ww, int(precision), _DT[out_dtype], _stream())
    _lib.check(rc, "hipie_mask_einsum")
    return out


def _pad_last(x, n):
    if x.shape[-1] == n:
        return x.contiguous()
    out = torch.zeros(*x.shape[:-1], n, dtype=x.dtype, device=x.device)
    out[..., :x.shape[-1]] = x
    return out


@_timed("mask_einsum_bwd")
def mask_einsum_backward(mask_embed, mask_features, grad_out):
    lib = _lib.load()
    B, Q, C = mask_embed.shape
    _, _, Hh, Ww = mask_features.shape
    HW = Hh * Ww
    if tuple(grad_out.shape) != (B, Q, Hh, Ww) or tuple(mask_features.shape[:2]) != (B, C) or not grad_out.is_cuda:
        raise RuntimeError("mask_einsum_backward: mask_embed (B,Q,C), mask_features (B,C,H,W), grad_out (B,Q,H,W) device tensors")
    if C % 8:
        raise RuntimeError("mask_einsum_backward: C must be a multiple of 8")
    dev = grad_out.device
    G = grad_out.float().reshape(B, Q, HW)
    F_ = mask_features.float().reshape(B, C, HW)
    HWp = (HW + 31) // 32 * 32
    nk = max(n for n in range(1, 33) if (HWp // 32) % n == 0)
    Kc = HWp // nk
    gh, fh = to_hl8(_pad_last(G, HWp)), to_hl8(_pad_last(F_, HWp))
    part = torch.empty(B, nk, Q, C, dtype=torch.float32, device=dev)
    rc = lib.hipie_gemm_batched(gh.data_ptr(), 2 * HWp, Q * 2 * HWp, 2 * Kc, fh.data_ptr(), 2 * HWp, C * 2 * HWp, 2 * Kc,
                                part.data_ptr(), C, nk * Q * C, Q * C, B, nk, Q, C, Kc, F32, 1.0, _stream())
    _lib.check(rc, "hipie_gemm_batched")
    grad_e = part.sum(1) if nk > 1 else part[:, 0]
    Qp = (Q + 31) // 32 * 32
    N8 = (HW + 7) // 8 * 8
    eT = to_hl8(_pad_last(mask_embed.float().transpose(1, 2), Qp))
    gT = torch.zeros(B, N8, Qp, dtype=torch.float32, device=dev) if (N8 != HW or Qp != Q) else torch.empty(B, N8, Qp, dtype=torch.float32, device=dev)
    gT[:, :HW, :Q] = G.transpose(1, 2)
    gTh = to_hl8(gT)
    gf = torch.empty(B, C, N8, dtype=torch.float32, device=dev)
    rc = lib.hipie_gemm_batched(eT.data_ptr(), 2 * Qp, C * 2 * Qp, 0, gTh.data_ptr(), 2 * Qp, N8 * 2 * Qp, 0, gf.data_ptr(), N8, C * N8, 0,
                                B, 1, C, N8, Qp, F32, 1.0, _stream())
    _lib.check(rc, "hipie_gemm_batched")
    if N8 != HW:
        gf = gf[..., :HW].contiguous()
    return grad_e, gf.view(B, C, Hh, Ww)


@_timed("mask_einsum")
def mask_einsum16(mask_embed, mask_features, split=True, out_dtype=None, row_bias=None):
    lib = _lib.load()
    B, Q, C = mask_embed.shape
    _, _, Hh, Ww = mask_features.shape
    dt = mask_features.dtype
    out_dtype = out_dtype or dt
    hi = mask_embed.to(dt).contiguous()
    lo = (mask_embed.float() - hi.float()).to(dt).contiguous() if split else None
    out = torch.empty(B, Q, Hh, Ww, dtype=out_dtype, device=mask_embed.device)
    rb = None if row_bias is None else _chk(row_bias.float().contiguous(), "row_bias", torch.float32)
    rc = lib.hipie_mask_einsum16(_chk(hi, "embed_hi"), None if lo is None else _chk(lo, "embed_lo"), _chk(mask_features, "mask_features"),
                                 rb, out.data_ptr(), B, Q, C, Hh * Ww, _DT[dt], _DT[out_dtype], _stream())
    _lib.check(rc, "hipie_mask_einsum16")
    return out


@_timed("dynamic_mask")
def dynamic_mask(mask_feats, ref_points, params, num_queries, stride=8, up=2, out_dtype=torch.float32, mlp_dtype=None):
    lib = _lib.load()
    B, C, H, W = mask_feats.shape
    if C != 8 or params.shape[-1] != 169:
        raise RuntimeError("dynamic_mask: expects 8 feature channels and 169 parameters per instance")
    n = B * num_queries
    out = torch.empty(n, up * H, up * W, dtype=out_dtype, device=mask_feats.device)
    split = mlp_dtype == "split" and out_dtype in (torch.float32, torch.float16)
    if (split or mlp_dtype in (torch.float16, torch.bfloat16)) and up == 2 and W % 4 == 0 and stride % 4 == 0 and stride * max(H, W) <= 8192:
        rc = lib.hipie_dynamic_mask16(_chk(mask_feats, "mask_feats", torch.float32), _chk(ref_points, "ref_points", torch.float32),
                                      _chk(params, "params", torch.float32), out.data_ptr(), B, num_queries, H, W,
                                      int(stride), HL8 if split else _DT[mlp_dtype], _DT[out_dtype], _stream())
        _lib.check(rc, "hipie_dynamic_mask16")
        return out
    rc = lib.hipie_dynamic_mask(_chk(mask_feats, "mask_feats", torch.float32), _chk(ref_points, "ref_points", torch.float32),
                                _chk(params, "params", torch.float32), out.data_ptr(), B, num_queries, H, W,
                                int(stride), int(up), _DT[out_dtype], _stream())
    _lib.check(rc, "hipie_dynamic_mask")
    return out


@_timed("dynamic_mask_bwd")
def dynamic_mask_backward(mask_feats, ref_points, params, grad_out, num_queries, stride=8, up=2):
    lib = _lib.load()
    B, C, H, W = mask_feats.shape
    n = B * num_queries
    if C != 8 or params.shape[-1] != 169 or params.numel() != n * 169 or ref_points.numel() != n * 2:
        raise RuntimeError("dynamic_mask_backward: expects 8 feature channels, (B*Q, 169) parameters and (B*Q, 2) reference points")
    if tuple(grad_out.shape[-2:]) != (up * H, up * W) or grad_out.numel() != n * up * up * H * W:
        raise RuntimeError("dynamic_mask_backward: grad_out must be (B*Q, up*H, up*W), got %s" % (tuple(grad_out.shape),))
    dev = mask_feats.device
    gf = torch.empty(B, 8, H, W, dtype=torch.float32, device=dev)
    gr = torch.empty(n, 2, dtype=torch.float32, device=dev)
    gp = torch.empty(n, 169, dtype=torch.float32, device=dev)
    rc = lib.hipie_dynamic_mask_backward(_chk(mask_feats, "mask_feats", torch.float32), _chk(ref_points, "ref_points", torch.float32),
                                         _chk(params, "params", torch.float32), _chk(grad_out, "grad_out", torch.float32),
                                         gf.data_ptr(), gr.data_ptr(), gp.data_ptr(), B, num_queries, H, W, int(stride), int(up), _stream())
    _lib.check(rc, "hipie_dynamic_mask_backward")
    return gf, gr, gp


@_timed("vit_relpos")
def vit_relpos(qkv, tab_h, tab_w, grid_hw, heads):
    lib = _lib.load()
    gh, gw = grid_hw
    B, N, C3 = qkv.shape
    hd = C3 // (3 * heads)
    rel_h = torch.empty(B * heads, gh, N, dtype=torch.float32, device=qkv.device)
    rel_w = torch.empty(B * heads, N, gw, dtype=torch.float32, device=qkv.device)
    rc = lib.hipie_vit_relpos(_chk(qkv, "qkv"), _chk(tab_h, "tab_h", qkv.dtype), _chk(tab_w, "tab_w", qkv.dtype),
                              rel_h.data_ptr(), rel_w.data_ptr(), B, gh, gw, heads, hd, _DT[qkv.dtype], _stream())
    _lib.check(rc, "hipie_vit_relpos")
    return rel_h, rel_w


@_timed("add_layernorm")
def add_layernorm(x, delta, weight, bias, eps, norm_dtype, want_res=True, delta_row=None, out_src=None):
    lib = _lib.load()
    C = x.shape[-1]
    rows = x.numel() // C
    res = torch.empty_like(x) if (want_res and delta is not None) else None
    if out_src is None:
        out = _alloc(tuple(x.shape), norm_dtype, x.device)
        out_rows = rows
    else:
        out_rows = int(out_src.shape[0])
        out = _alloc((out_rows, C), norm_dtype, x.device)
    args = (_chk(x, "x"), None if delta is None else _chk(delta, "delta"),
            _chk(weight, "weight", torch.float32), _chk(bias, "bias", torch.float32),
            None if res is None else res.data_ptr(), out.data_ptr(), out_rows, C, float(eps),
            _DT[x.dtype], _DT[x.dtype if delta is None else delta.dtype], _code(norm_dtype))
    if delta_row is None and out_src is None:
        rc = lib.hipie_add_layernorm(*args, _stream())
    else:
        rc = lib.hipie_add_layernorm_rows(*args, None if delta_row is None else _chk(delta_row, "delta_row", torch.int32),
                                          None if out_src is None else _chk(out_src, "out_src", torch.int32), _stream())
    _lib.check(rc, "hipie_add_layernorm")
    return (x if delta is None else res), out


@_timed("layernorm_bwd")
def layernorm_backward(s, gy, weight, eps, gres=None, want_param_grads=True):
    for n, t in (("s", s), ("gy", gy), ("weight", weight), ("gres", gres)):
        if t is not None and not t.is_cuda:
            raise RuntimeError("Not implemented on the CPU (%s must be a CUDA/HIP tensor)" % n)
    lib = _lib.load()
    C = s.shape[-1]
    rows = s.numel() // C if C else 0
    if gy.shape != s.shape or (gres is not None and gres.shape != s.shape) or weight.numel() != C:
        raise RuntimeError("layernorm_backward: gy / gres must have the shape of s %s and weight its last dimension" % (tuple(s.shape),))

    def rows16(t):
        t = t.contiguous()
        return t if t.data_ptr() % 16 == 0 else t.clone()
    s, gy, weight = rows16(s), rows16(gy), rows16(weight)
    gres = None if gres is None else rows16(gres)
    dx = torch.empty_like(s)
    dgamma = dbeta = ws = None
    ws_bytes = 0
    if want_param_grads:
        dgamma, dbeta = torch.empty_like(weight), torch.empty_like(weight)
        ws_bytes = int(lib.hipie_layernorm_backward_ws_bytes(rows, C))
        ws = torch.empty(ws_bytes, dtype=torch.uint8, device=s.device)
    rc = lib.hipie_layernorm_backward(_chk(s, "s", torch.float32), _chk(gy, "gy", torch.float32),
                                      None if gres is None else _chk(gres, "gres", torch.float32), _chk(weight, "weight", torch.float32),
                                      dx.data_ptr(), None if dgamma is None else dgamma.data_ptr(), None if dbeta is None else dbeta.data_ptr(),
                                      None if ws is None else ws.data_ptr(), ws_bytes, rows, C, float(eps), _stream())
    _lib.check(rc, "hipie_layernorm_backward")
    return dx, dgamma, dbeta


def _act_rows16(t, name):
    if not t.is_cuda:
        raise RuntimeError("Not implemented on the CPU (%s must be a CUDA/HIP tensor)" % name)
    if t.dtype != torch.float32:
        raise RuntimeError("%s must be torch.float32, got %s" % (name, t.dtype))
    t = t.contiguous()
    if t.data_ptr() % 16:
        t = t.clone()
    N = t.shape[-1] if t.dim() else 1
    return t, (t.numel() // N if N else 0), N


@_timed("act_fwd")
def act_forward(u, act):
    u, rows, N = _act_rows16(u, "u")
    a = torch.empty_like(u)
    rc = _lib.load().hipie_act_forward(u.data_ptr(), a.data_ptr(), rows, N, int(act), _stream())
    _lib.check(rc, "hipie_act_forward")
    return a


@_timed("act_bwd")
def act_backward(u, g, act, want_a=False, want_bias_grad=False, out=None):
    u, rows, N = _act_rows16(u, "u")
    if g.shape != u.shape:
        raise RuntimeError("act_backward: g %s must have the shape of u %s" % (tuple(g.shape), tuple(u.shape)))
    g_in = g
    g, _, _ = _act_rows16(g, "g")
    if out is not None and not out.is_cuda:
        raise RuntimeError("Not implemented on the CPU (out must be a CUDA/HIP tensor)")
    if out is not None and out is g_in:
        out = g
    usable = (out is not None and out.dtype == torch.float32 and out.shape == u.shape and out.is_contiguous() and out.data_ptr() % 16 == 0
              and out.data_ptr() != u.data_ptr())
    du = out if usable else torch.empty_like(u)
    a = torch.empty_like(u) if want_a else None
    dbias = ws = None
    lib = _lib.load()
    if want_bias_grad:
        dbias = torch.empty(N, dtype=torch.float32, device=u.device)
        ws = torch.empty(int(lib.hipie_act_backward_ws_bytes(rows, N)), dtype=torch.uint8, device=u.device)
    rc = lib.hipie_act_backward(u.data_ptr(), g.data_ptr(), du.data_ptr(), None if a is None else a.data_ptr(),
                                None if dbias is None else dbias.data_ptr(), None if ws is None else ws.data_ptr(), rows, N, int(act), _stream())
    _lib.check(rc, "hipie_act_backward")
    return du, a, dbias


@_timed("add_layernorm")
def add_layernorm_sum(x, delta, weight, bias, eps, addend):
    lib = _lib.load()
    C = x.shape[-1]
    rows = x.numel() // C
    if addend.dtype != x.dtype or addend.shape != x.shape:
        raise RuntimeError("add_layernorm_sum: addend must match x")
    out, s = torch.empty_like(x), torch.empty_like(x)
    rc = lib.hipie_add_layernorm_sum(_chk(x, "x"), _chk(delta, "delta"), _chk(weight, "weight", torch.float32),
                                     _chk(bias, "bias", torch.float32), None, out.data_ptr(), _chk(addend, "addend"), s.data_ptr(),
                                     rows, C, float(eps), _DT[x.dtype], _DT[delta.dtype], _DT[x.dtype], _stream())
    _lib.check(rc, "hipie_add_layernorm_sum")
    return out, s


@_timed("add_layernorm")
def add_layernorm_dec(x, delta, weight, bias, eps, aux_dtype, want16=False, addend=None):
    lib = _lib.load()
    C = x.shape[-1]
    rows = x.numel() // C
    out = torch.empty_like(x)
    n16 = _alloc(tuple(x.shape), aux_dtype, x.device) if want16 else None
    s16 = _alloc(tuple(x.shape), aux_dtype, x.device) if addend is not None else None
    if addend is not None and ((addend.dtype != aux_dtype or addend.shape != x.shape) if aux_dtype != "hl8" else
                               (addend.dtype != torch.float16 or addend.numel() != 2 * x.numel())):
        raise RuntimeError("add_layernorm_dec: addend must match x's shape in aux_dtype")
    rc = lib.hipie_add_layernorm_dec(_chk(x, "x", torch.float32), _chk(delta, "delta"), _chk(weight, "weight", torch.float32),
                                     _chk(bias, "bias", torch.float32), out.data_ptr(), None if n16 is None else n16.data_ptr(),
                                     None if addend is None else _chk(addend, "addend"), None if s16 is None else s16.data_ptr(),
                                     rows, C, float(eps), _DT[delta.dtype], _code(aux_dtype), _stream())
    _lib.check(rc, "hipie_add_layernorm_dec")
    return out, n16, s16


_GN_WS = {}


def group_norm_ok(x, groups):
    if not x.is_cuda or x.dim() != 4 or x.dtype not in _DT or x.shape[1] != groups * 8 or groups > 64 or 256 % groups:
        return False
    return x.is_contiguous(memory_format=torch.channels_last) or (x.is_contiguous() and (x.shape[2] * x.shape[3]) % 8 == 0)


@_timed("group_norm")
def group_norm(x, groups, weight, bias, eps, relu=False, prebias=None, out_dtype=None, out_nchw=False):
    lib = _lib.load()
    B, C, H, W = x.shape
    nhwc = x.is_contiguous(memory_format=torch.channels_last) and not (x.is_contiguous() and C > 1 and H * W > 1)
    if not nhwc and not x.is_contiguous():
        raise RuntimeError("group_norm: x must be NCHW- or channels-last-contiguous")
    out_dtype = out_dtype or x.dtype
    if out_nchw and nhwc and (H * W) % 64 == 0:
        nhwc = 2
        out = torch.empty(B, C, H, W, dtype=out_dtype, device=x.device)
    else:
        out = torch.empty_like(x, dtype=out_dtype)
    key = (str(x.device), B * groups, torch.cuda.current_stream(x.device).cuda_stream)
    ws = _GN_WS.get(key)
    if ws is None:
        ws = _GN_WS[key] = torch.empty(2 * B * groups * 512, dtype=torch.float32, device=x.device)
    rc = lib.hipie_group_norm(x.data_ptr(), None if prebias is None else _chk(prebias, "prebias", torch.float32),
                              _chk(weight, "weight", torch.float32), _chk(bias, "bias", torch.float32), out.data_ptr(),
                              ws.data_ptr(), B, C, H * W, groups, int(nhwc), float(eps), 1 if relu else 0,
                              _DT[x.dtype], _DT[out_dtype], _stream())
    _lib.check(rc, "hipie_group_norm")
    return out


@_timed("add_cast")
def add_cast(a, b):
    lib = _lib.load()
    if a.shape != b.shape:
        raise RuntimeError("add_cast: shapes differ")
    out = torch.empty_like(b)
    rc = lib.hipie_add_cast(_chk(a, "a", torch.float32), _chk(b, "b"), out.data_ptr(), a.numel(), _DT[b.dtype], _stream())
    _lib.check(rc, "hipie_add_cast")
    return out


@_timed("add_cast")
def add_to_hl8(a, b_hl8):
    lib = _lib.load()
    if b_hl8.dtype != torch.float16 or b_hl8.numel() != 2 * a.numel() or a.shape[-1] % 8 or not a.is_cuda:
        raise RuntimeError("add_to_hl8: a (.., C) fp32 and b (.., 2C) HL8 device tensors, C %% 8 == 0")
    out = torch.empty_like(b_hl8)
    rc = lib.hipie_add_cast(_chk(a, "a", torch.float32), _chk(b_hl8, "b"), out.data_ptr(), a.numel(), HL8, _stream())
    _lib.check(rc, "hipie_add_cast")
    return out


@_timed("batched_nms")
def batched_nms(boxes, scores, classes, iou_threshold, coordinate_trick=None):
    lib = _lib.load()
    B, Q = scores.shape
    if coordinate_trick is None:
        coordinate_trick = Q * 4 <= 4000
    order = scores.sort(dim=1, descending=True, stable=True)[1].to(torch.int32)
    keep = torch.empty(B, Q, dtype=torch.int32, device=boxes.device)
    count = torch.empty(B, dtype=torch.int32, device=boxes.device)
    rc = lib.hipie_batched_nms(_chk(boxes, "boxes", torch.float32), _chk(classes, "classes", torch.int64), order.data_ptr(),
                               keep.data_ptr(), count.data_ptr(), B, Q, float(iou_threshold), int(coordinate_trick), _stream())
    _lib.check(rc, "hipie_batched_nms")
    return keep, count


@_timed("mask_finalize")
def mask_finalize(masks, qidx, up, crop_hw, out_hw, threshold):
    lib = _lib.load()
    Q, hm, wm = masks.shape
    n = Q if qidx is None else int(qidx.shape[0])
    out = torch.empty(n, out_hw[0], out_hw[1], dtype=torch.uint8, device=masks.device)
    rc = lib.hipie_mask_finalize(_chk(masks, "masks"), _DT[masks.dtype], None if qidx is None else _chk(qidx, "qidx", torch.int32),
                                 n, hm, wm, int(up), int(crop_hw[0]), int(crop_hw[1]), int(out_hw[0]), int(out_hw[1]),
                                 float(threshold), out.data_ptr(), _stream())
    _lib.check(rc, "hipie_mask_finalize")
    return out


SEM_PAN_CLASSES = 160


def sem_pan_ok(n_queries, n_classes):
    return 0 < n_classes and 0 < n_queries <= 8192


@_timed("sem_pan")
def sem_pan(masks_lo, cls_all, pscore, up, crop_hw, out_hw, precision=0):
    lib = _lib.load()
    N, C = cls_all.shape
    _, hm, wm = masks_lo.shape
    dev = masks_lo.device
    npad = (N + 15) // 16 * 16
    ps = torch.full((npad,), -1.0, dtype=torch.float32, device=dev)
    ps[:N] = pscore
    oh, ow = int(out_hw[0]), int(out_hw[1])
    sem = torch.empty(C, oh, ow, dtype=torch.float32, device=dev)
    pan_idx = torch.empty(oh, ow, dtype=torch.int32, device=dev)
    pan_own = torch.empty(oh, ow, dtype=torch.uint8, device=dev)
    area = torch.zeros(npad, dtype=torch.int32, device=dev)
    masks_ptr = _chk(masks_lo, "masks", torch.float32)
    spare = None
    for c0 in range(0, C, SEM_PAN_CLASSES):
        cn = min(SEM_PAN_CLASSES, C - c0)
        cp = 32 if cn <= 32 else 96 if cn <= 96 else 160
        cls_t = torch.zeros(cp, npad, dtype=torch.float32, device=dev)
        cls_t[:cn, :N] = cls_all[:, c0:c0 + cn].t()
        hi = cls_t.to(torch.bfloat16)
        lo = (cls_t - hi.float()).to(torch.bfloat16) if precision == 0 else None
        if c0 == 0:
            outs = (pan_idx, pan_own, area)
        else:
            if spare is None:
                spare = (torch.empty_like(pan_idx), torch.empty_like(pan_own), torch.zeros_like(area))
            outs = spare
        rc = lib.hipie_sem_pan(masks_ptr, hi.data_ptr(), None if lo is None else lo.data_ptr(),
                               ps.data_ptr(), sem[c0:c0 + cn].data_ptr(), outs[0].data_ptr(), outs[1].data_ptr(), outs[2].data_ptr(),
                               N, npad, cn, hm, wm, int(up), int(crop_hw[0]), int(crop_hw[1]), oh, ow, int(precision), _stream())
        _lib.check(rc, "hipie_sem_pan")
    return sem, pan_idx, pan_own.bool(), area[:N]


_DIM_T = {}


@_timed("sine_embed")
def sine_embed(ref, num_pos_feats=128, temperature=10000, out_dtype=torch.float32):
    import math
    lib = _lib.load()
    nc = ref.shape[-1]
    ref = ref.float()
    rs = nc
    if ref.dim() == 3 and ref.stride(-1) == 1 and ref.stride(0) == ref.shape[1] * ref.stride(1) and ref.stride(1) >= nc:
        rs = ref.stride(1)
    elif not ref.is_contiguous():
        ref = ref.contiguous()
    key = (num_pos_feats, temperature, str(ref.device))
    dim_t = _DIM_T.get(key)
    if dim_t is None:
        d = torch.arange(num_pos_feats, dtype=torch.float32, device=ref.device)
        dim_t = (temperature ** (2 * torch.div(d, 2, rounding_mode="floor") / num_pos_feats)).contiguous()
        _DIM_T[key] = dim_t
    n = ref.numel() // nc
    out = torch.empty(ref.shape[:-1] + (nc * num_pos_feats,), dtype=out_dtype, device=ref.device)
    if not ref.is_cuda:
        raise RuntimeError("Not implemented on the CPU (ref must be a CUDA/HIP tensor)")
    rc = lib.hipie_sine_embed(ref.data_ptr(), dim_t.data_ptr(), out.data_ptr(), n, nc, num_pos_feats, rs,
                              2 * math.pi, _DT[out_dtype], _stream())
    _lib.check(rc, "hipie_sine_embed")
    return out


def _transposed(mod_layers, dtype=None):
    return derived(mod_layers[0], "wt", [p for l in mod_layers for p in (l.weight, l.bias)],
                   lambda: [(l.weight.t().contiguous(), l.bias.contiguous()) for l in mod_layers])


def ref_point_mlp_ok(ref, head):
    ls = getattr(head, "layers", None)
    return (ls is not None and len(ls) == 2 and ref.is_cuda and ref.shape[-1] == 4 and tuple(ls[0].weight.shape) == (256, 512)
            and tuple(ls[1].weight.shape) == (256, 256) and ls[0].weight.dtype == ls[1].weight.dtype and ls[0].weight.dtype in _DT)


@_timed("ref_point_mlp")
def ref_point_mlp(ref, head, num_pos_feats=128, temperature=10000):
    import math
    lib = _lib.load()
    ref = ref.float()
    rs = 4
    if ref.dim() == 3 and ref.stride(-1) == 1 and ref.stride(0) == ref.shape[1] * ref.stride(1) and ref.stride(1) >= 4:
        rs = ref.stride(1)
    elif not ref.is_contiguous():
        ref = ref.contiguous()
    key = (num_pos_feats, temperature, str(ref.device))
    dim_t = _DIM_T.get(key)
    if dim_t is None:
        d = torch.arange(num_pos_feats, dtype=torch.float32, device=ref.device)
        dim_t = (temperature ** (2 * torch.div(d, 2, rounding_mode="floor") / num_pos_feats)).contiguous()
        _DIM_T[key] = dim_t
    (w1t, b1), (w2t, b2) = _transposed(list(head.layers))
    dt = w1t.dtype
    n = ref.numel() // 4
    out = torch.empty(ref.shape[:-1] + (256,), dtype=dt, device=ref.device)
    rc = lib.hipie_ref_point_mlp(ref.data_ptr(), dim_t.data_ptr(), w1t.data_ptr(), b1.data_ptr(), w2t.data_ptr(), b2.data_ptr(),
                                 out.data_ptr(), n, rs, 2 * math.pi, _DT[dt], _stream())
    _lib.check(rc, "hipie_ref_point_mlp")
    return out


def box_head_ok(x, mlp):
    ls = getattr(mlp, "layers", None)
    return (ls is not None and len(ls) == 3 and x.is_cuda and x.dtype == torch.float32 and x.shape[-1] == 256
            and [tuple(l.weight.shape) for l in ls] == [(256, 256), (256, 256), (4, 256)]
            and all(l.weight.dtype == torch.float32 for l in ls))


@_timed("box_head")
def box_head(x, ref, mlp, eps=1e-5):
    lib = _lib.load()
    x, ref = x.contiguous(), ref.float().contiguous()
    (w1t, b1), (w2t, b2), (w3t, b3) = _transposed(list(mlp.layers))
    out = torch.empty_like(ref)
    rc = lib.hipie_box_head(_chk(x, "x", torch.float32), _chk(ref, "ref", torch.float32), w1t.data_ptr(), b1.data_ptr(), w2t.data_ptr(),
                            b2.data_ptr(), w3t.data_ptr(), b3.data_ptr(), out.data_ptr(), ref.numel() // 4, float(eps), _stream())
    _lib.check(rc, "hipie_box_head")
    return out


@_timed("box_refine")
def box_refine(delta, ref, eps=1e-5):
    lib = _lib.load()
    delta, ref = delta.contiguous(), ref.float().contiguous()
    out = torch.empty_like(ref)
    rc = lib.hipie_box_refine(_chk(delta, "delta"), _chk(ref, "ref", torch.float32), out.data_ptr(), ref.numel(), float(eps),
                              _DT[delta.dtype], _stream())
    _lib.check(rc, "hipie_box_refine")
    return out


def selftest(which, a, b=None):
    lib = _lib.load()
    out = torch.empty(32 * 32 if which == 0 else 256, dtype=torch.float32, device=a.device)
    rc = lib.hipie_selftest(which, a.data_ptr(), None if b is None else b.data_ptr(), out.data_ptr(), _stream())
    _lib.check(rc, "hipie_selftest")
    return out


def hl8_pack(x, scale=1.0):
    K = x.shape[-1]
    assert K % 8 == 0
    xs = (x.float() * scale).clamp(-65504.0, 65504.0)
    hi = xs.half()
    lo = (xs - hi.float()).half()
    return torch.stack([hi.reshape(*x.shape[:-1], K // 8, 8), lo.reshape(*x.shape[:-1], K // 8, 8)], dim=-2).reshape(*x.shape[:-1], 2 * K).contiguous()


def hl8_unpack(x):
    K2 = x.shape[-1]
    g = x.reshape(*x.shape[:-1], K2 // 16, 2, 8).float()
    return (g[..., 0, :] + g[..., 1, :]).reshape(*x.shape[:-1], K2 // 2)


@_timed("to_hl8")
def to_hl8(x, scale=1.0):
    lib = _lib.load()
    K = x.shape[-1]
    x2 = x.reshape(-1, K)
    if x2.stride(-1) != 1:
        x2 = x2.contiguous()
    out = torch.empty(*x.shape[:-1], 2 * K, dtype=torch.float16, device=x.device)
    if not x.is_cuda:
        raise RuntimeError("Not implemented on the CPU (to_hl8)")
    rc = lib.hipie_to_hl8(x2.data_ptr(), x2.stride(0), out.data_ptr(), 2 * K, x2.shape[0], K, _DT[x.dtype], float(scale), _stream())
    _lib.check(rc, "hipie_to_hl8")
    return out


@_timed("to_hl8_t")
def to_hl8_t(x, pad_to=32, scale=1.0):
    lib = _lib.load()
    if x.dim() != 2 or x.dtype != torch.float32 or not x.is_cuda:
        raise RuntimeError("to_hl8_t: a 2-D fp32 device tensor")
    if x.stride(1) != 1:
        x = x.contiguous()
    M, C = x.shape
    Mp = -(-M // pad_to) * pad_to
    out = torch.empty(C, 2 * Mp, dtype=torch.float16, device=x.device)
    rc = lib.hipie_to_hl8_t(x.data_ptr(), x.stride(0), out.data_ptr(), 2 * Mp, M, C, Mp, float(scale), _stream())
    _lib.check(rc, "hipie_to_hl8_t")
    return out


def f16_pair(x, cols=None, scale=None):
    C = x.shape[-1]
    Cp = C if cols is None else max(cols, C)
    if x.is_cuda and x.dtype == torch.float32 and Cp % 8 == 0:
        lib = _lib.load()
        x2 = x.reshape(-1, C)
        if x2.stride(1) != 1 or (x2.shape[0] > 1 and x2.stride(0) < C):
            x2 = x2.contiguous()
        hi = torch.empty(*x.shape[:-1], Cp, dtype=torch.float16, device=x.device)
        lo = torch.empty_like(hi)
        sc = 0 if scale is None else scale.float().reshape(1).data_ptr()
        rc = lib.hipie_to_f16_pair(x2.data_ptr(), x2.stride(0) if x2.shape[0] > 1 else C, hi.data_ptr(), lo.data_ptr(), x2.shape[0], C, Cp, sc, _stream())
        _lib.check(rc, "hipie_to_f16_pair")
        return hi, lo
    raise RuntimeError("f16_pair: an fp32 device tensor and a column count that is a multiple of 8 (got %s %s on %s, %d columns)"
                       % (x.dtype, tuple(x.shape), x.device, Cp))


@_timed("attn_train_fwd")
def attn_train_forward(q_pair, k_pair, v_pair):
    lib = _lib.load()
    qh, ql = q_pair
    kh, kl = k_pair
    vh, vl = v_pair
    BH, N, DQ = qh.shape
    if DQ != 224 or kh.shape != qh.shape or tuple(vh.shape) != (BH, N, 80) or N % 128 or not qh.is_cuda:
        raise RuntimeError("attn_train_forward: q', k' (BH, N, 224), v (BH, N, 80) device pairs with N %% 128 == 0, got %s / %s / %s"
                           % (tuple(qh.shape), tuple(kh.shape), tuple(vh.shape)))
    for t in (qh, ql, kh, kl, vh, vl):
        if t.dtype != torch.float16 or not t.is_contiguous():
            raise RuntimeError("attn_train_forward: contiguous fp16 planes")
    out = torch.empty(BH, N, 80, dtype=torch.float32, device=qh.device)
    lse = torch.empty(BH, N, dtype=torch.float32, device=qh.device)
    rc = lib.hipie_attn_train_forward(qh.data_ptr(), ql.data_ptr(), kh.data_ptr(), kl.data_ptr(), vh.data_ptr(), vl.data_ptr(), out.data_ptr(),
                                      lse.data_ptr(), BH, N, _stream())
    _lib.check(rc, "hipie_attn_train_forward")
    return out, lse


@_timed("attn_train_bwd")
def attn_train_backward(q_pair, k_pair, v96_pair, do96_pair, lse, delta):
    lib = _lib.load()
    qh, ql = q_pair
    kh, kl = k_pair
    vh, vl = v96_pair
    dh, dl = do96_pair
    BH, N, _ = qh.shape
    if tuple(vh.shape) != (BH, N, 96) or tuple(dh.shape) != (BH, N, 96) or tuple(lse.shape) != (BH, N) or tuple(delta.shape) != (BH, N):
        raise RuntimeError("attn_train_backward: v / dO as (BH, N, 96) pairs, lse / delta (BH, N)")
    for t in (qh, ql, kh, kl, vh, vl, dh, dl):
        if t.dtype != torch.float16 or not t.is_contiguous() or not t.is_cuda:
            raise RuntimeError("attn_train_backward: contiguous fp16 device planes")
    lse, delta = lse.float().contiguous(), delta.float().contiguous()
    dq = torch.empty(BH, N, 224, dtype=torch.float32, device=qh.device)
    dk = torch.empty(BH, N, 80, dtype=torch.float32, device=qh.device)
    dv = torch.empty(BH, N, 80, dtype=torch.float32, device=qh.device)
    rc = lib.hipie_attn_train_backward(qh.data_ptr(), ql.data_ptr(), kh.data_ptr(), kl.data_ptr(), vh.data_ptr(), vl.data_ptr(), dh.data_ptr(),
                                       dl.data_ptr(), lse.data_ptr(), delta.data_ptr(), dq.data_ptr(), dk.data_ptr(), dv.data_ptr(), BH, N, _stream())
    _lib.check(rc, "hipie_attn_train_backward")
    return dq, dk, dv


@_timed("fill_rows")
def fill_rows(dst, rows, src_row):
    lib = _lib.load()
    if dst.dim() != 2 or not dst.is_cuda or src_row.dtype != dst.dtype or src_row.numel() != dst.shape[1]:
        raise RuntimeError("fill_rows: dst (R, W) on the device, src_row (W,) of the same dtype")
    rc = lib.hipie_fill_rows(_chk(dst, "dst"), dst.stride(0) * dst.element_size(), _chk(rows, "rows", torch.int32), rows.numel(),
                             _chk(src_row, "src_row"), dst.shape[1] * dst.element_size(), _stream())
    _lib.check(rc, "hipie_fill_rows")
    return dst


ACT_NONE, ACT_GELU, ACT_RELU, ACT_QGELU = 0, 1, 2, 3


def _gemm_tag(a, w, *args, **kw):
    tag = kw.get("tag", "gemm")
    if PROFILE.shapes and tag == "gemm":
        split = kw.get("split")
        K = w.shape[1] // 2 if split else w.shape[1]
        tag = "gemm M%d N%d K%d %s->%s%s" % (a.numel() // a.shape[-1], w.shape[0], K, "f32" if a.dtype == torch.float32 else ("hl8" if split else "f16"),
                                          {F32: "f32", F16: "f16", HL8: "hl8"}.get(kw.get("out_fmt", F32), "?"), " +res" if kw.get("resid") is not None else "")
    return tag


@_timed(_gemm_tag)
def gemm(a, w, bias=None, resid=None, out_fmt=F32, act=ACT_NONE, alpha=1.0, oscale=1.0, split=None, out=None, tag="gemm", out_row=None,
         out_rows=None, a_row=None):
    lib = _lib.load()
    a_f32 = a.dtype == torch.float32 and bool(split)
    if (a.dtype != torch.float16 and not a_f32) or w.dtype != torch.float16 or not a.is_cuda:
        raise RuntimeError("gemm: operands must be fp16 (plain or HL8) device tensors (a may be fp32 against HL8 weights)")
    if split is None:
        raise RuntimeError("gemm: say split=True (HL8 operands) or split=False (plain fp16)")
    N = w.shape[0]
    Kw = w.shape[1] // 2 if split else w.shape[1]
    lead = a.shape[:-1]
    a2 = a if a.dim() == 2 else a.reshape(-1, a.shape[-1])
    if a2.stride(-1) != 1 or a2.shape[-1] != (Kw if a_f32 else w.shape[1]):
        raise RuntimeError("gemm: a rows must be contiguous and as long as w rows (%s vs %s)" % (tuple(a.shape), tuple(w.shape)))
    if a_f32 and (a2.stride(0) % 4 or a2.data_ptr() % 16):
        raise RuntimeError("gemm: fp32 a rows must be 16-byte aligned")
    M = a2.shape[0]
    if a_row is not None:
        if a_row.dtype != torch.int32 or not a_row.is_contiguous() or not split:
            raise RuntimeError("gemm: a_row must be a contiguous int32 vector (split operands only)")
        M = a_row.numel()
        lead = (M,)
        if out is not None and out_row is None and out.numel() // out.shape[-1] < M:
            raise RuntimeError("gemm: `out` has fewer rows (%d) than the row map (%d)" % (out.numel() // out.shape[-1], M))
        if resid is not None and resid.numel() // N < M:
            raise RuntimeError("gemm: `resid` has fewer rows (%d) than the row map (%d)" % (resid.numel() // N, M))
    if out_row is not None:
        if out is None:
            lead = (int(out_rows),)
        if out_row.dtype != torch.int32 or out_row.numel() != M or not out_row.is_contiguous():
            raise RuntimeError("gemm: out_row must be a contiguous int32 vector with one entry per row of a")
    if out is None:
        if out_fmt == F32:
            out = torch.empty(*lead, N, dtype=torch.float32, device=a.device)
        elif out_fmt == F16:
            out = torch.empty(*lead, N, dtype=torch.float16, device=a.device)
        else:
            out = torch.empty(*lead, 2 * N, dtype=torch.float16, device=a.device)
    o2 = out.reshape(-1, out.shape[-1])
    r2 = None
    if resid is not None:
        r2 = resid.reshape(-1, N)
        if r2.dtype != torch.float32 or r2.stride(-1) != 1:
            raise RuntimeError("gemm: resid must be fp32 with contiguous rows")
    if bias is not None and (bias.dtype != torch.float32 or not bias.is_contiguous()):
        raise RuntimeError("gemm: bias must be contiguous fp32")
    if a_row is not None:
        rc = lib.hipie_gemm_gather(a2.data_ptr(), a2.stride(0), a2.shape[0], a_row.data_ptr(), _chk(w, "w"), w.shape[1],
                                   None if bias is None else bias.data_ptr(), None if r2 is None else r2.data_ptr(), 0 if r2 is None else r2.stride(0),
                                   o2.data_ptr(), o2.stride(0), None if out_row is None else out_row.data_ptr(), M, N, Kw,
                                   F32 if a_f32 else HL8, int(out_fmt), int(act), float(alpha), float(oscale), _stream())
        _lib.check(rc, "hipie_gemm_gather")
        return out
    rc = lib.hipie_gemm(a2.data_ptr(), a2.stride(0), _chk(w, "w"), w.shape[1], None if bias is None else bias.data_ptr(),
                        None if r2 is None else r2.data_ptr(), 0 if r2 is None else r2.stride(0), o2.data_ptr(), o2.stride(0),
                        None if out_row is None else out_row.data_ptr(), M, N, Kw, F32 if a_f32 else (HL8 if split else F16), int(out_fmt), int(act), float(alpha), float(oscale), _stream())
    _lib.check(rc, "hipie_gemm")
    return out


@_timed(lambda qkv, tab_h, tab_w, grid_hw, heads: "vit_attn_global" if grid_hw[0] * grid_hw[1] > 256 else "vit_attn_window")
def vit_attn_split(qkv, tab_h, tab_w, grid_hw, heads):
    lib = _lib.load()
    gh, gw = grid_hw
    B, N, C6 = qkv.shape
    hd = C6 // (6 * heads)
    if qkv.dtype != torch.float16 or tab_h.dtype != torch.float16 or tab_w.dtype != torch.float16:
        raise RuntimeError("vit_attn_split: HL8 (fp16) operands expected")
    out = torch.empty(B, N, 2 * heads * hd, dtype=torch.float16, device=qkv.device)
    rc = lib.hipie_vit_attn_split(_chk(qkv, "qkv"), _chk(tab_h, "tab_h"), _chk(tab_w, "tab_w"), out.data_ptr(), B, gh, gw, heads, hd, _stream())
    _lib.check(rc, "hipie_vit_attn_split")
    return out


@_timed("gemm_split_k")
def gemm_split_k(a_hl8, w_hl8, nk):
    lib = _lib.load()
    M, K2 = a_hl8.shape
    N = w_hl8.shape[0]
    K = K2 // 2
    if w_hl8.shape[1] != K2 or K % (32 * nk) or a_hl8.dtype != torch.float16 or w_hl8.dtype != torch.float16 or not a_hl8.is_cuda:
        raise RuntimeError("gemm_split_k: HL8 device operands (M, 2K) / (N, 2K), K a multiple of 32 * nk")
    if N % 8:
        raise RuntimeError("gemm_split_k: N must be a multiple of 8")
    Kc = K // nk
    part = torch.empty(nk, M, N, dtype=torch.float32, device=a_hl8.device)
    rc = lib.hipie_gemm_batched(a_hl8.data_ptr(), K2, 0, 2 * Kc, w_hl8.data_ptr(), K2, 0, 2 * Kc, part.data_ptr(), N, 0, M * N, 1, nk, M, N, Kc,
                                F32, 1.0, _stream())
    _lib.check(rc, "hipie_gemm_batched")
    return part.sum(0)


@_timed("gemm_batched")
def matmul_nt_batched(a, w, alpha=1.0):
    lib = _lib.load()
    B, M, K = a.shape
    N = w.shape[1]
    if w.shape[0] != B or w.shape[2] != K or K % 32 or not a.is_cuda:
        raise RuntimeError("matmul_nt_batched: a (B, M, K), w (B, N, K) device tensors with K %% 32 == 0, got %s / %s" % (tuple(a.shape), tuple(w.shape)))
    Np = (N + 7) // 8 * 8
    if Np != N:
        wp = torch.zeros(B, Np, K, dtype=torch.float32, device=w.device)
        wp[:, :N] = w
        w = wp
    ah, wh = to_hl8(a.float().contiguous()), to_hl8(w.float().contiguous())
    out = torch.empty(B, M, Np, dtype=torch.float32, device=a.device)
    rc = lib.hipie_gemm_batched(ah.data_ptr(), 2 * K, M * 2 * K, 0, wh.data_ptr(), 2 * K, Np * 2 * K, 0, out.data_ptr(), Np, M * Np, 0,
                                B, 1, M, Np, K, F32, float(alpha), _stream())
    _lib.check(rc, "hipie_gemm_batched")
    return out if Np == N else out[..., :N]


def vit_attn_split_ok(grid_hw, hd):
    gh, gw = grid_hw

    def rows_ok(kh, kw):
        return (kw <= 32 and kh <= 160) or (kw <= 64 and kh <= 132) or (64 < kw <= 96 and kh <= 160)
    return hd in (64, 80) and ((gw == 14 and gh <= 96) or rows_ok(gh, gw) or (gw > 96 and gh <= 96 and rows_ok(gw, gh)))


def _padded_f32(weight_fn, bias_fn):
    w = weight_fn().detach().float()
    b = None if bias_fn is None else bias_fn()
    b = None if b is None else b.detach().float()
    N = w.shape[0]
    Np = (N + 7) // 8 * 8
    if Np != N:
        w = torch.nn.functional.pad(w, (0, 0, 0, Np - N))
        b = None if b is None else torch.nn.functional.pad(b, (0, Np - N))
    return w, None if b is None else b.contiguous(), N


def split_weight(owner, key, params, weight_fn, bias_fn=None):
    def build():
        w, b, N = _padded_f32(weight_fn, bias_fn)
        return hl8_pack(w), b, N
    return derived(owner, ("hl8", key), params, build)


def conv3x3_split_ok(x, conv):
    return (x.is_cuda and x.dim() == 4 and conv.kernel_size == (3, 3) and conv.stride == (1, 1) and conv.padding == (1, 1) and conv.dilation == (1, 1)
            and conv.padding_mode == "zeros" and conv.groups == 1 and conv.weight.dtype == torch.float32 and conv.in_channels % 32 == 0 and conv.out_channels % 256 == 0
            and x.shape[0] * (x.shape[2] + 2) * (x.shape[3] + 2) >= 16384)


_CONV_STAGE = {}
_RETIRED = []


@_timed("conv3x3_split")
def conv3x3_split(x, conv, act=ACT_NONE):
    lib = _lib.load()
    B, C, H, W = x.shape
    N = conv.out_channels
    Hp, Wp = H + 2, W + 2
    guard = Wp + 1
    rows = B * Hp * Wp
    skey = (B, C, H, W, str(x.device), torch.cuda.current_stream(x.device).cuda_stream)
    buf = _CONV_STAGE.get(skey)
    if buf is None:
        if len(_CONV_STAGE) >= 8:
            _RETIRED.append(_CONV_STAGE.pop(next(iter(_CONV_STAGE))))
        buf = _CONV_STAGE[skey] = torch.zeros(rows + 2 * guard, C, dtype=torch.float32, device=x.device)
    buf[guard:guard + rows].view(B, Hp, Wp, C)[:, 1:-1, 1:-1].copy_(x.permute(0, 2, 3, 1))
    w, b, _ = split_weight(conv, "w3x3", [conv.weight] + ([conv.bias] if conv.bias is not None else []),
                           lambda: conv.weight.permute(0, 2, 3, 1).reshape(N, 9 * C), (lambda: conv.bias) if conv.bias is not None else None)
    out = torch.empty(rows, N, dtype=torch.float32, device=x.device)
    xin = buf[guard:]
    rc = lib.hipie_conv3x3_split(xin.data_ptr(), C, w.data_ptr(), None if b is None else b.data_ptr(), out.data_ptr(), N, rows, Wp, C, N,
                                 F32, F32, int(act), _stream())
    _lib.check(rc, "hipie_conv3x3_split")
    return out.view(B, Hp, Wp, N)[:, 1:-1, 1:-1].permute(0, 3, 1, 2).contiguous(memory_format=torch.channels_last)


_FFN_PERM = {}


def ffn_fused_ok(x_hl8, lin1, lin2):
    return (x_hl8.is_cuda and lin1.weight.shape == (2048, 256) and lin2.weight.shape == (256, 2048) and lin1.bias is not None
            and lin2.bias is not None and lin1.weight.dtype == torch.float32 and x_hl8.numel() // 512 >= 4096)


@_timed("ffn_fused")
def ffn_fused(x_hl8, lin1, lin2):
    lib = _lib.load()
    w1, b1, _ = split_weight(lin1, "w", [lin1.weight, lin1.bias], lambda: lin1.weight, lambda: lin1.bias)
    F_ = lin2.weight.shape[1]
    perm = _FFN_PERM.get(F_)
    if perm is None:
        base = torch.tensor([0, 1, 2, 3, 8, 9, 10, 11, 4, 5, 6, 7, 12, 13, 14, 15])
        perm = _FFN_PERM[F_] = (torch.arange(0, F_, 16)[:, None] + base[None, :]).reshape(-1)
    w2, b2, _ = split_weight(lin2, "w_ffn_perm", [lin2.weight, lin2.bias], lambda: lin2.weight[:, perm.to(lin2.weight.device)], lambda: lin2.bias)
    lead = x_hl8.shape[:-1]
    x2 = x_hl8.reshape(-1, x_hl8.shape[-1])
    if x2.dtype != torch.float16 or x2.stride(-1) != 1 or x2.shape[-1] != 512:
        raise RuntimeError("ffn_fused: x must be HL8 rows of 2 * 256 fp16 values")
    M = x2.shape[0]
    out = torch.empty(M, 256, dtype=torch.float32, device=x2.device)
    rc = lib.hipie_ffn_fused(x2.data_ptr(), x2.stride(0), w1.data_ptr(), b1.data_ptr(), w2.data_ptr(), b2.data_ptr(), out.data_ptr(), 256,
                             M, 256, F_, _stream())
    _lib.check(rc, "hipie_ffn_fused")
    return out.view(*lead, 256)


def split_ok(K):
    return K % 32 == 0


def split_linear(x, owner, key, weight, bias=None, act=ACT_NONE, out_fmt=F32, resid=None, x_hl8=False, weight_fn=None, bias_fn=None,
                 tag="gemm", params=None, out=None, out_row=None, a_row=None):
    if params is None:
        params = [weight] + ([bias] if bias is not None else [])
    w, b, N = split_weight(owner, key, params, weight_fn or (lambda: weight), bias_fn or ((lambda: bias) if bias is not None else None))
    if x_hl8:
        a = x
    elif x.dtype == torch.float32 and x.stride(-1) == 1 and x.data_ptr() % 16 == 0 and (x.dim() < 2 or x.stride(-2) % 4 == 0):
        a = x if x.dim() <= 2 or x.is_contiguous() else x.contiguous()
    else:
        a = to_hl8(x if x.dtype in (torch.float32, torch.float16) else x.float())
    if out is not None or out_row is not None or a_row is not None:
        if N != w.shape[0]:
            raise RuntimeError("split_linear: in-place / row-mapped outputs need N % 8 == 0")
        return gemm(a, w, b, resid, out_fmt=out_fmt, act=act, split=True, tag=tag, out=out, out_row=out_row, a_row=a_row)
    out = gemm(a, w, b, resid, out_fmt=out_fmt, act=act, split=True, tag=tag)
    if N != w.shape[0]:
        out = out[..., :(2 * N if out_fmt == HL8 else N)].contiguous()
    return out



@_timed("to_f8x")
def to_f8x(x_hl8):
    lib = _lib.load()
    if x_hl8.dtype != torch.float16 or not x_hl8.is_cuda or x_hl8.shape[-1] % 64:
        raise RuntimeError("to_f8x: HL8 rows (fp16, 2K columns with K a multiple of 32) on the device")
    x2 = x_hl8.reshape(-1, x_hl8.shape[-1])
    if x2.stride(-1) != 1:
        x2 = x2.contiguous()
    R, K = x2.shape[0], x2.shape[1] // 2
    q = torch.empty(R, 2 * K, dtype=torch.uint8, device=x_hl8.device)
    sc = torch.empty(R, K // 32, 2, dtype=torch.uint8, device=x_hl8.device)
    rc = lib.hipie_to_f8x(x2.data_ptr(), x2.stride(0), q.data_ptr(), 2 * K, sc.data_ptr(), R, K, _stream())
    _lib.check(rc, "hipie_to_f8x")
    return q, sc


def f8x_weight(owner, key, params, weight_fn, bias_fn=None):
    def build():
        from . import fp8x
        w, b, N = _padded_f32(weight_fn, bias_fn)
        w_hl8 = hl8_pack(w)
        q, sc = to_f8x(w_hl8) if w_hl8.is_cuda else (None, None)
        w8, wsc = fp8x.pack_from_hl8(w_hl8, q, sc)
        return w8, wsc, b, N
    return derived(owner, ("f8x", key), params, build)


@_timed("gemm_f8x")
def gemm_f8x(a, w8, wsc, bias=None, resid=None, out_fmt=F32, act=ACT_NONE, alpha=1.0, oscale=1.0, out=None, out_row=None, out_rows=None):
    lib = _lib.load()
    if a.dtype != torch.float16 or w8.dtype != torch.uint8 or wsc.dtype != torch.uint8 or not a.is_cuda:
        raise RuntimeError("gemm_f8x: a HL8 (fp16) rows, w8 / wsc uint8, on the device")
    N, K = w8.shape[0], w8.shape[1] // 4
    a2 = a if a.dim() == 2 else a.reshape(-1, a.shape[-1])
    if a2.stride(-1) != 1 or a2.shape[-1] != 2 * K or not w8.is_contiguous() or tuple(wsc.shape) != (N, K // 32, 2) or not wsc.is_contiguous():
        raise RuntimeError("gemm_f8x: a rows %s against an f8x weight %s / scales %s" % (tuple(a.shape), tuple(w8.shape), tuple(wsc.shape)))
    M = a2.shape[0]
    lead = a.shape[:-1]
    if out_row is not None:
        if out is None:
            lead = (int(out_rows),)
        if out_row.dtype != torch.int32 or out_row.numel() != M or not out_row.is_contiguous():
            raise RuntimeError("gemm_f8x: out_row must be a contiguous int32 vector with one entry per row of a")
    if out is None:
        dt, width = {F32: (torch.float32, N), F16: (torch.float16, N), HL8: (torch.float16, 2 * N)}[out_fmt]
        out = torch.empty(*lead, width, dtype=dt, device=a.device)
    o2 = out.reshape(-1, out.shape[-1])
    r2 = None
    if resid is not None:
        r2 = resid.reshape(-1, N)
        if r2.dtype != torch.float32 or r2.stride(-1) != 1:
            raise RuntimeError("gemm_f8x: resid must be fp32 with contiguous rows")
    if bias is not None and (bias.dtype != torch.float32 or not bias.is_contiguous()):
        raise RuntimeError("gemm_f8x: bias must be contiguous fp32")
    rc = lib.hipie_gemm_f8x(a2.data_ptr(), a2.stride(0), _chk(w8, "w8"), 2 * K, _chk(wsc, "wsc"), None if bias is None else bias.data_ptr(),
                            None if r2 is None else r2.data_ptr(), 0 if r2 is None else r2.stride(0), o2.data_ptr(), o2.stride(0),
                            None if out_row is None else out_row.data_ptr(), M, N, K, HL8, int(out_fmt), int(act), float(alpha), float(oscale), _stream())
    _lib.check(rc, "hipie_gemm_f8x")
    return out


def f8x_linear(x_hl8, owner, key, weight, bias=None, act=ACT_NONE, out_fmt=F32, resid=None, out=None):
    params = [weight] + ([bias] if bias is not None else [])
    w8, wsc, b, N = f8x_weight(owner, key, params, lambda: weight, (lambda: bias) if bias is not None else None)
    if N != w8.shape[0]:
        raise RuntimeError("f8x_linear: N %% 8 == 0 expected (got %d)" % N)
    return gemm_f8x(x_hl8, w8, wsc, b, resid, out_fmt=out_fmt, act=act, out=out)

def split_linear_ln_ok(x, weight, norm_weight):
    return (x.is_cuda and weight.dtype == torch.float32 and weight.shape[0] == 256 and norm_weight.numel() == 256 and weight.shape[1] % 32 == 0
            and not torch.is_grad_enabled())


@_timed("gemm_ln")
def split_linear_ln(x, owner, key, weight, bias, resid, norm_weight, norm_bias, eps, x_hl8=False, want_hl8=True):
    lib = _lib.load()
    w, b, N = split_weight(owner, key, [weight] + ([bias] if bias is not None else []), lambda: weight, (lambda: bias) if bias is not None else None)
    if N != 256 or w.shape[0] != 256:
        raise RuntimeError("split_linear_ln: 256 output features expected")
    K = w.shape[1] // 2
    a_f32 = not x_hl8
    if a_f32 and (x.dtype != torch.float32 or x.stride(-1) != 1):
        raise RuntimeError("split_linear_ln: x must be fp32 rows or HL8")
    a2 = x.reshape(-1, x.shape[-1])
    if a2.shape[-1] != (K if a_f32 else 2 * K) or (a_f32 and (a2.stride(0) % 4 or a2.data_ptr() % 16)):
        raise RuntimeError("split_linear_ln: operand rows %s against weight %s" % (tuple(x.shape), tuple(weight.shape)))
    r2 = resid.reshape(-1, 256)
    M = a2.shape[0]
    if r2.dtype != torch.float32 or r2.stride(-1) != 1 or r2.shape[0] != M or not r2.is_cuda:
        raise RuntimeError("split_linear_ln: resid must be (rows, 256) fp32 on the device")
    out = torch.empty(*resid.shape[:-1], 256, dtype=torch.float32, device=x.device)
    o16 = torch.empty(*resid.shape[:-1], 512, dtype=torch.float16, device=x.device) if want_hl8 else None
    rc = lib.hipie_gemm_ln(a2.data_ptr(), a2.stride(0), _chk(w, "w"), w.shape[1], None if b is None else b.data_ptr(), r2.data_ptr(), r2.stride(0),
                           _chk(norm_weight, "norm_weight", torch.float32), _chk(norm_bias, "norm_bias", torch.float32), float(eps),
                           out.data_ptr(), 256, None if o16 is None else o16.data_ptr(), 512, M, K, F32 if a_f32 else HL8, 1.0, _stream())
    _lib.check(rc, "hipie_gemm_ln")
    return out, o16


_SHUFFLE_MAPS = {}


def _shuffle_maps(B, H, W, device):
    key = (B, H, W, str(device))
    m = _SHUFFLE_MAPS.get(key)
    if m is None:
        b = torch.arange(B, device=device).view(B, 1, 1)
        h = torch.arange(H, device=device).view(1, H, 1)
        w = torch.arange(W, device=device).view(1, 1, W)
        m = [((b * 2 * H + 2 * h + i) * 2 * W + 2 * w + j).reshape(-1).to(torch.int32).contiguous() for i in range(2) for j in range(2)]
        if len(_SHUFFLE_MAPS) > 16:
            _RETIRED.extend(_SHUFFLE_MAPS.values())
            _SHUFFLE_MAPS.clear()
        _SHUFFLE_MAPS[key] = m
    return m


def convt2x2_split(rows, owner, key, weight, bias, B, H, W):
    Cin, Cout = weight.shape[0], weight.shape[1]
    if rows.dim() != 2 or rows.shape[0] != B * H * W or rows.shape[1] != Cin or Cout % 8:
        raise RuntimeError("convt2x2_split: rows (B*H*W, C_in), weight (C_in, C_out, 2, 2) with C_out %% 8 == 0, got %s / %s" % (tuple(rows.shape), tuple(weight.shape)))
    out = torch.empty(B, 2 * H, 2 * W, Cout, dtype=torch.float32, device=rows.device)
    o2 = out.view(-1, Cout)
    maps = _shuffle_maps(B, H, W, rows.device)
    a = rows if rows.dtype == torch.float32 and rows.is_contiguous() else rows.float().contiguous()
    for t in range(4):
        i, j = divmod(t, 2)
        split_linear(a, owner, "%s_tap%d" % (key, t), weight, bias, weight_fn=lambda i=i, j=j: weight[:, :, i, j].t().contiguous(),
                     out=o2, out_row=maps[t], tag="gemm_convt")
    return out


@_timed("topk")
def topk(x, k, want_values=False):
    lib = _lib.load()
    if x.dim() != 2 or x.dtype != torch.float32 or not x.is_cuda or x.stride(1) != 1:
        raise RuntimeError("topk: (rows, n) fp32 device tensor with contiguous rows expected")
    rows, n = x.shape
    idx = torch.empty(rows, k, dtype=torch.int64, device=x.device)
    val = torch.empty(rows, k, dtype=torch.float32, device=x.device) if want_values else None
    rc = lib.hipie_topk(x.data_ptr(), x.stride(0), rows, n, int(k), idx.data_ptr(), None if val is None else val.data_ptr(), _stream())
    _lib.check(rc, "hipie_topk")
    return (idx, val) if want_values else idx


def topk_ok(x, k):
    return x.is_cuda and x.dtype == torch.float32 and x.dim() == 2 and x.stride(1) == 1 and 0 < k <= min(1024, x.shape[1])
```

### include/hipie_mi355.h

```cpp
#ifndef HIPIE_MI355_H
#define HIPIE_MI355_H

#include <stdint.h>

#ifdef __cplusplus
extern "C" {
#endif

#define HIPIE_ABI_VERSION 13

#define HIPIE_F32 0
#define HIPIE_F16 1
#define HIPIE_BF16 2
#define HIPIE_F64 3
#define HIPIE_HL8 4

#define HIPIE_OUT_F32 0x100
#define HIPIE_K_HL8_HI 0x200

#define HIPIE_ATTN_FAST 1

#define HIPIE_OK 0
#define HIPIE_EINVAL (-22)
#define HIPIE_ELAUNCH (-5)

int hipie_version(void);
const char* hipie_last_error(void);

int hipie_msda_forward(const void* value, const int64_t* spatial_shapes, const int64_t* level_start,
                       const void* sampling_loc, const void* attn_weight, void* out,
                       int B, int S, int M, int D, int L, int Lq, int P, int value_dtype, void* stream);

int hipie_msda_backward(const void* value, const int64_t* spatial_shapes, const int64_t* level_start, const void* sampling_loc,
                        const void* attn_weight, const void* grad_output, void* grad_value, void* grad_sampling_loc,
                        void* grad_attn_weight, int B, int S, int M, int D, int L, int Lq, int P, int dtype, void* stream);

int64_t hipie_msda_backward_workspace(int B, int S, int M, int L, int Lq, int P);
int hipie_msda_backward_ws(const void* value, const int64_t* spatial_shapes, const int64_t* level_start, const void* sampling_loc,
                           const void* attn_weight, const void* grad_output, void* grad_value, void* grad_sampling_loc,
                           void* grad_attn_weight, int B, int S, int M, int D, int L, int Lq, int P, int dtype, void* workspace,
                           int64_t workspace_bytes, void* stream);

int hipie_msda_fused_forward(const void* value, const int64_t* spatial_shapes, const int64_t* level_start,
                             const float* ref, const void* offsets, const void* logits, void* out,
                             int B, int S, int M, int D, int L, int Lq, int P, int ref_dim, int value_dtype,
                             int aux_dtype, int64_t off_row_stride, int64_t logit_row_stride, void* stream);

int hipie_msda_fused_forward_strided(const void* value, int64_t value_row_stride, const int64_t* spatial_shapes,
                                     const int64_t* level_start, const float* ref, const void* offsets, const void* logits,
                                     void* out, int B, int S, int M, int D, int L, int Lq, int P, int ref_dim, int value_dtype,
                                     int aux_dtype, int64_t off_row_stride, int64_t logit_row_stride, void* stream);

int hipie_flash_attn(const void* q, const void* k, const void* v, void* out,
                     int B, int H, int Nq, int Nk, int head_dim,
                     int64_t q_sb, int64_t q_st, int64_t q_sh, int64_t k_sb, int64_t k_st, int64_t k_sh,
                     int64_t v_sb, int64_t v_st, int64_t v_sh, int64_t o_sb, int64_t o_st, int64_t o_sh,
                     const float* bias_h, const float* bias_w, int kh, int kw,
                     const uint8_t* key_mask, float scale, float clamp, int dtype, void* stream);

int hipie_vit_attn(const void* qkv, const float* rel_h, const float* rel_w, void* out,
                   int B, int gh, int gw, int heads, int hd, float scale, int dtype, void* stream);

int hipie_bi_xattn(const void* q, const void* k, const void* vv, const void* vl, const uint8_t* text_mask,
                   void* out_v, void* out_l, int B, int H, int Nv, int L, int hd, float clamp, int dtype, void* stream);

int64_t hipie_bi_xattn_workspace(int B, int H, int Nv, int L, int head_dim);
int hipie_bi_xattn_ws(const void* q, const void* k, const void* vv, const void* vl, const uint8_t* text_mask,
                      void* out_v, void* out_l, void* workspace, int64_t workspace_bytes, int B, int H, int Nv, int L,
                      int head_dim, float clamp, int dtype, void* stream);

int hipie_mask_einsum(const float* embed, const float* feats, void* out, int B, int Q, int C, int HW,
                      int precision, int out_dtype, void* stream);

int64_t hipie_mask_einsum_workspace(int B, int Q, int C);
int hipie_mask_einsum_ws(const float* embed, const float* feats, const float* row_bias, void* out, void* workspace,
                         int64_t workspace_bytes, int B, int Q, int C, int HW, int precision, int out_dtype, void* stream);

int hipie_mask_einsum16(const void* embed_hi, const void* embed_lo, const void* feats, const float* row_bias, void* out, int B,
                        int Q, int C, int HW, int dtype, int out_dtype, void* stream);

int hipie_dynamic_mask(const float* feats, const float* refs, const float* params, void* out,
                       int B, int Q, int H, int W, int stride, int up, int out_dtype, void* stream);

int hipie_dynamic_mask_backward(const float* feats, const float* refs, const float* params, const float* grad_out, float* grad_feats,
                                float* grad_refs, float* grad_params, int B, int Q, int H, int W, int stride, int up, void* stream);

int hipie_dynamic_mask16(const float* feats, const float* refs, const float* params, void* out,
                         int B, int Q, int H, int W, int stride, int dtype, int out_dtype, void* stream);

int hipie_vit_relpos(const void* qkv, const void* tab_h, const void* tab_w, float* rel_h, float* rel_w,
                     int B, int gh, int gw, int heads, int hd, int dtype, void* stream);

int hipie_add_layernorm(const void* x, const void* delta, const float* gamma, const float* beta, void* res_out,
                        void* norm_out, int64_t rows, int C, float eps, int x_dtype, int delta_dtype, int norm_dtype,
                        void* stream);

int hipie_layernorm_backward(const float* s, const float* gy, const float* gres, const float* gamma, float* dx, float* dgamma,
                             float* dbeta, void* ws, int64_t ws_bytes, int64_t rows, int C, float eps, void* stream);
int64_t hipie_layernorm_backward_ws_bytes(int64_t rows, int C);

int hipie_act_forward(const float* u, float* a, int64_t rows, int N, int act, void* stream);
int hipie_act_backward(const float* u, const float* g, float* du, float* a, float* dbias, void* ws, int64_t rows, int N, int act,
                       void* stream);
int64_t hipie_act_backward_ws_bytes(int64_t rows, int N);

int hipie_vit_attn_fused(const void* qkv, const void* tab_h, const void* tab_w, void* out, int B, int gh, int gw, int heads,
                         int hd, float scale, int dtype, void* stream);

int hipie_vit_attn_rel(const void* qkv, const void* tab_h, const void* tab_w, void* out, int B, int gh, int gw, int heads,
                       int hd, int dtype, int flags, void* stream);

int hipie_add_layernorm_rows(const void* x, const void* delta, const float* gamma, const float* beta, void* res_out,
                             void* norm_out, int64_t out_rows, int C, float eps, int x_dtype, int delta_dtype,
                             int norm_dtype, const int32_t* delta_row, const int32_t* out_src, void* stream);

int hipie_add_layernorm_sum(const void* x, const void* delta, const float* gamma, const float* beta, void* res_out,
                            void* norm_out, const void* addend, void* sum_out, int64_t rows, int C, float eps,
                            int x_dtype, int delta_dtype, int norm_dtype, void* stream);

int hipie_add_layernorm_dec(const float* x, const void* delta, const float* gamma, const float* beta, float* norm_out,
                            void* norm16_out, const void* addend, void* sum16_out, int64_t rows, int C, float eps,
                            int delta_dtype, int aux_dtype, void* stream);

int hipie_ref_point_mlp(const float* ref, const float* dim_t, const void* w1t, const void* b1, const void* w2t, const void* b2,
                        void* out, int64_t n, int ref_stride, float scale, int dtype, void* stream);
int hipie_box_head(const float* x, const float* ref, const float* w1t, const float* b1, const float* w2t, const float* b2,
                   const float* w3t, const float* b3, float* out, int64_t n, float eps, void* stream);

int hipie_group_norm(const void* x, const float* prebias, const float* gamma, const float* beta, void* out, float* workspace,
                     int B, int C, int HW, int groups, int channels_last, float eps, int relu, int x_dtype, int out_dtype,
                     void* stream);

int hipie_add_cast(const float* a, const void* b, void* out, int64_t n, int dtype, void* stream);

int hipie_batched_nms(const float* boxes, const int64_t* classes, const int32_t* order, int32_t* keep, int32_t* count,
                      int B, int Q, float iou_threshold, int coordinate_trick, void* stream);

int hipie_mask_finalize(const void* masks, int dtype, const int32_t* qidx, int n, int hm, int wm, int up, int crop_h,
                        int crop_w, int out_h, int out_w, float threshold, uint8_t* out, void* stream);

int hipie_sem_pan(const float* masks, const void* cls_hi, const void* cls_lo, const float* pscore, float* sem,
                  int32_t* pan_idx, uint8_t* pan_own, int32_t* area, int N, int Npad, int C, int hm, int wm, int up,
                  int crop_h, int crop_w, int out_h, int out_w, int precision, void* stream);

int hipie_sine_embed(const float* ref, const float* dim_t, void* out, int64_t n, int n_coord, int num_pos_feats, int ref_stride,
                     float scale, int out_dtype, void* stream);

int hipie_box_refine(const void* delta, const float* ref, float* out, int64_t n, float eps, int delta_dtype, void* stream);

int hipie_gemm(const void* A, int64_t lda, const void* W, int64_t ldw, const float* bias, const float* resid, int64_t ldr,
               void* out, int64_t ldo, const int32_t* out_row, int M, int N, int K, int in_fmt, int out_fmt, int act, float alpha,
               float oscale, void* stream);

int hipie_gemm_f8x(const void* A, int64_t lda, const void* W, int64_t ldw, const void* w_scale, const float* bias, const float* resid,
                   int64_t ldr, void* out, int64_t ldo, const int32_t* out_row, int M, int N, int K, int in_fmt, int out_fmt, int act,
                   float alpha, float oscale, void* stream);

int hipie_to_f8x(const void* x, int64_t ldx, void* out, int64_t ldo, void* scale, int64_t rows, int K, void* stream);

int hipie_gemm_ln(const void* A, int64_t lda, const void* W, int64_t ldw, const float* bias, const float* resid, int64_t ldr,
                  const float* gamma, const float* beta, float eps, float* out, int64_t ldo, void* out_hl8, int64_t ldo_hl8, int M, int K,
                  int in_fmt, float alpha, void* stream);

int hipie_gemm_gather(const void* A, int64_t lda, int64_t a_rows, const int32_t* a_row, const void* W, int64_t ldw, const float* bias,
                      const float* resid, int64_t ldr, void* out, int64_t ldo, const int32_t* out_row, int M, int N, int K, int in_fmt,
                      int out_fmt, int act, float alpha, float oscale, void* stream);

int hipie_vit_attn_split(const void* qkv, const void* tab_h, const void* tab_w, void* out, int B, int gh, int gw, int heads,
                         int hd, void* stream);

int hipie_attn_train_forward(const void* q_hi, const void* q_lo, const void* k_hi, const void* k_lo, const void* v_hi, const void* v_lo,
                             void* out, void* lse, int BH, int N, void* stream);
int hipie_to_f16_pair(const void* x, int64_t ldx, void* hi, void* lo, int64_t rows, int C, int Cp, const void* scale, void* stream);
int hipie_attn_train_backward(const void* q_hi, const void* q_lo, const void* k_hi, const void* k_lo, const void* v_hi, const void* v_lo,
                              const void* do_hi, const void* do_lo, const void* lse, const void* delta, void* dq, void* dk, void* dv,
                              int BH, int N, void* stream);

int hipie_fill_rows(void* dst, int64_t ld_bytes, const int32_t* rows, int64_t n_rows, const void* src_row, int64_t row_bytes, void* stream);

int hipie_to_hl8(const void* x, int64_t ldx, void* out, int64_t ldo, int64_t rows, int K, int x_dtype, float scale, void* stream);

int hipie_to_hl8_t(const void* x, int64_t ldx, void* out, int64_t ldo, int64_t rows, int C, int64_t rows_p, float scale, void* stream);

int hipie_gemm_batched(const void* A, int64_t lda, int64_t a_outer, int64_t a_inner, const void* W, int64_t ldw, int64_t w_outer,
                       int64_t w_inner, void* out, int64_t ldo, int64_t o_outer, int64_t o_inner, int n_outer, int n_inner, int M, int N,
                       int K, int out_fmt, float alpha, void* stream);

int hipie_gemm_batched_softmax(const void* A, int64_t lda, int64_t a_outer, int64_t a_inner, const void* W, int64_t ldw, int64_t w_outer,
                               int64_t w_inner, void* out, int64_t ldo, int64_t o_outer, int64_t o_inner, int n_outer, int n_inner, int M,
                               int N, int K, const unsigned char* mask, int L, float clamp, float alpha, void* stream);

int hipie_gemm_batched_softmax_bias(const void* A, int64_t lda, int64_t a_outer, int64_t a_inner, const void* W, int64_t ldw, int64_t w_outer,
                                    int64_t w_inner, void* out, int64_t ldo, int64_t o_outer, int64_t o_inner, int n_outer, int n_inner,
                                    int M, int N, int K, const unsigned char* mask, int L, const float* col_bias, float clamp, float alpha,
                                    void* stream);
int hipie_gemm_batched_resid(const void* A, int64_t lda, int64_t a_outer, int64_t a_inner, const void* W, int64_t ldw, int64_t w_outer,
                             int64_t w_inner, const float* bias, const float* resid, int64_t ldr, int64_t r_outer, int64_t r_inner, float* out,
                             int64_t ldo, int64_t o_outer, int64_t o_inner, int n_outer, int n_inner, int M, int N, int K, float alpha,
                             void* stream);

int hipie_softmax_hl8(const float* S, int64_t lds, void* P, int64_t ldp, int64_t rows, int L, int Lp, const unsigned char* mask,
                      int64_t rows_per_batch, float clamp, void* stream);

int hipie_attn_f32(const float* q, const float* k, const float* v, const unsigned char* key_mask, float* out, int B, int H, int Nq, int Nk,
                   int head_dim, int64_t q_sb, int64_t q_st, int64_t k_sb, int64_t k_st, int64_t v_sb, int64_t v_st, float scale,
                   void* stream);

int hipie_attn_f32_rows(const float* q, const float* k, const float* v, const unsigned char* query_mask, float* out, int B, int H, int Nq,
                        int Nk, int head_dim, int64_t q_sb, int64_t q_st, int64_t k_sb, int64_t k_st, int64_t v_sb, int64_t v_st, float scale,
                        void* stream);
int hipie_attn_split_rows(const float* q, const float* k, const float* v, const unsigned char* query_mask, float* out, int B, int H, int Nq,
                          int Nk, int head_dim, int64_t q_sb, int64_t q_st, int64_t k_sb, int64_t k_st, int64_t v_sb, int64_t v_st, float scale,
                          void* stream);

int hipie_attn_split(const float* q, const float* k, const float* v, const unsigned char* key_mask, float* out, int B, int H, int Nq, int Nk,
                   int head_dim, int64_t q_sb, int64_t q_st, int64_t k_sb, int64_t k_st, int64_t v_sb, int64_t v_st, float scale,
                   void* stream);

int hipie_ffn_fused(const void* x, int64_t ldx, const void* w1, const float* b1, const void* w2p, const float* b2, float* out, int64_t ldo,
                    int M, int D, int F, void* stream);

int hipie_conv3x3_split(const void* x, int64_t ldx, const void* w, const float* bias, void* out, int64_t ldo, int64_t rows, int Wp, int C,
                        int N, int in_fmt, int out_fmt, int act, void* stream);

int hipie_topk(const float* x, int64_t row_stride, int rows, int n, int k, int64_t* idx_out, float* val_out, void* stream);

int hipie_selftest(int which, const uint16_t* a, const uint16_t* b, float* out, void* stream);

#ifdef __cplusplus
}
#endif
#endif
```

Before: 40.98 images/sec.

## Write input-projection GroupNorm and conv outputs directly into flattened encoder token rows

Adds row-addressed variants of GroupNorm and the 3x3 split conv so that each level's input projection writes straight into a shared (B, S, C) token buffer, optionally with an HL8 split copy. This replaces the per-level flatten/transpose/cat and a separate to_hl8 pass. The conv path now uses a crop row map so the padded-border rows are not copied out afterwards. The trade-off is more plumbing (project_levels, token passing through the transformers) and extra writes for the HL8 output inside the GroupNorm kernel.

```diff
diff --git a/hipie_amd/_lib.py b/hipie_amd/_lib.py
--- a/hipie_amd/_lib.py
+++ b/hipie_amd/_lib.py
@@ -48,6 +48,7 @@
     "hipie_add_layernorm_dec": [c_p, c_p, c_p, c_p, c_p, c_p, c_p, c_p, c_l, c_i, c_f, c_i, c_i, c_p],
     "hipie_add_cast": [c_p, c_p, c_p, c_l, c_i, c_p],
     "hipie_group_norm": [c_p, c_p, c_p, c_p, c_p, c_p, c_i, c_i, c_i, c_i, c_i, c_f, c_i, c_i, c_i, c_p],
+    "hipie_group_norm_rows": [c_p, c_p, c_p, c_p, c_p, c_l, c_p, c_l, c_l, c_l, c_p, c_i, c_i, c_i, c_i, c_f, c_i, c_i, c_i, c_p],
     "hipie_gemm": [c_p, c_l, c_p, c_l, c_p, c_p, c_l, c_p, c_l, c_p] + [c_i] * 6 + [c_f, c_f, c_p],
     "hipie_gemm_f8x": [c_p, c_l, c_p, c_l, c_p, c_p, c_p, c_l, c_p, c_l, c_p] + [c_i] * 6 + [c_f, c_f, c_p],
     "hipie_to_f8x": [c_p, c_l, c_p, c_l, c_p, c_l, c_i, c_p],
@@ -67,6 +68,7 @@
     "hipie_attn_f32_rows": [c_p] * 5 + [c_i] * 5 + [c_l] * 6 + [c_f, c_p],
     "hipie_attn_split_rows": [c_p] * 5 + [c_i] * 5 + [c_l] * 6 + [c_f, c_p],
     "hipie_conv3x3_split": [c_p, c_l, c_p, c_p, c_p, c_l, c_l] + [c_i] * 6 + [c_p],
+    "hipie_conv3x3_split_rows": [c_p, c_l, c_p, c_p, c_p, c_l, c_p, c_l] + [c_i] * 6 + [c_p],
     "hipie_ffn_fused": [c_p, c_l, c_p, c_p, c_p, c_p, c_p, c_l, c_i, c_i, c_i, c_p],
     "hipie_topk": [c_p, c_l, c_i, c_i, c_i, c_p, c_p, c_p],
     "hipie_fill_rows": [c_p, c_l, c_p, c_l, c_p, c_l, c_p],
diff --git a/hipie_amd/csrc/gemm.hip b/hipie_amd/csrc/gemm.hip
--- a/hipie_amd/csrc/gemm.hip
+++ b/hipie_amd/csrc/gemm.hip
@@ -213,8 +213,8 @@
   return launch_gemm<256, true>(p, (hipStream_t)stream, n_outer * n_inner);
 }
 
-extern "C" int hipie_conv3x3_split(const void* x, int64_t ldx, const void* w, const float* bias, void* out, int64_t ldo, int64_t rows, int Wp,
-                                   int C, int N, int in_fmt, int out_fmt, int act, void* stream) {
+static int conv3x3_impl(const void* x, int64_t ldx, const void* w, const float* bias, void* out, int64_t ldo, const int32_t* out_row, int64_t rows,
+                        int Wp, int C, int N, int in_fmt, int out_fmt, int act, void* stream) {
   HIPIE_REQUIRE(x && w && out, "conv3x3_split: null pointer");
   HIPIE_REQUIRE(in_fmt == HIPIE_HL8 || in_fmt == HIPIE_F32, "conv3x3_split: input format %d (HIPIE_HL8 | HIPIE_F32 rows)", in_fmt);
   HIPIE_REQUIRE(out_fmt == HIPIE_F32 || out_fmt == HIPIE_HL8, "conv3x3_split: output format %d (HIPIE_F32 | HIPIE_HL8)", out_fmt);
@@ -228,12 +228,24 @@
   HIPIE_TRY(gm_check_aligned("conv3x3_split", {x, w, out, bias}));
   GemmParams p;
   gm_set_operands(p, x, ldx, w, (long)2 * 9 * C, (int)rows, N, 9 * C);
-  p.bias = bias; p.out = (char*)out; p.ldo = ldo; p.out_fmt = out_fmt; p.act = act;
+  p.bias = bias; p.out = (char*)out; p.ldo = ldo; p.out_fmt = out_fmt; p.act = act; p.out_row = out_row;
   p.conv_kpt = C / 32; p.conv_wp = Wp;
   hipStream_t st = (hipStream_t)stream;
   const bool wide = (N % 320 == 0);
   if (in_fmt == HIPIE_F32) return wide ? launch_gemm<320, true, 2>(p, st) : launch_gemm<256, true, 2>(p, st);
   return wide ? launch_gemm<320, true>(p, st) : launch_gemm<256, true>(p, st);
+}
+
+extern "C" int hipie_conv3x3_split(const void* x, int64_t ldx, const void* w, const float* bias, void* out, int64_t ldo, int64_t rows, int Wp,
+                                   int C, int N, int in_fmt, int out_fmt, int act, void* stream) {
+  return conv3x3_impl(x, ldx, w, bias, out, ldo, nullptr, rows, Wp, C, N, in_fmt, out_fmt, act, stream);
+}
+
+extern "C" int hipie_conv3x3_split_rows(const void* x, int64_t ldx, const void* w, const float* bias, void* out, int64_t ldo,
+                                        const int32_t* out_row, int64_t rows, int Wp, int C, int N, int in_fmt, int out_fmt, int act,
+                                        void* stream) {
+  HIPIE_REQUIRE(out_row != nullptr, "conv3x3_split: out_row map");
+  return conv3x3_impl(x, ldx, w, bias, out, ldo, out_row, rows, Wp, C, N, in_fmt, out_fmt, act, stream);
 }
 
 extern "C" int hipie_to_hl8(const void* x, int64_t ldx, void* out, int64_t ldo, int64_t rows, int K, int x_dtype, float scale, void* stream) {
diff --git a/hipie_amd/csrc/groupnorm.hip b/hipie_amd/csrc/groupnorm.hip
--- a/hipie_amd/csrc/groupnorm.hip
+++ b/hipie_amd/csrc/groupnorm.hip
@@ -50,11 +50,17 @@
   }
 }
 
+struct GnOut {
+  long ldo, obs;
+  f16_t* hl8;
+  long ldo_h, obs_h;
+};
+
 template <typename T, typename OutT>
 __global__ __launch_bounds__(256) void gn_apply_nhwc_kernel(const T* __restrict__ x, const float* __restrict__ prebias,
                                                             const float* __restrict__ part, const float* __restrict__ gamma,
-                                                            const float* __restrict__ beta, OutT* __restrict__ out, int HW, int G,
-                                                            int nchunk, int per, float eps, int relu) {
+                                                            const float* __restrict__ beta, OutT* __restrict__ out, const GnOut o, int HW,
+                                                            int G, int nchunk, int per, float eps, int relu) {
   __shared__ float stat[2][64];
   const int b = blockIdx.y, chunk = blockIdx.x;
   const int g = threadIdx.x % G, pl = threadIdx.x / G, npl = 256 / G;
@@ -84,7 +90,20 @@
     V8<T>::ld(x + off, v);
 #pragma unroll
     for (int i = 0; i < 8; ++i) { v[i] = fmaf(v[i], sc[i], sh[i]); if (relu) v[i] = fmaxf(v[i], 0.f); }
-    V8<OutT>::st(out + off, v);
+    V8<OutT>::st(out + (long)b * o.obs + (long)p * o.ldo + g * 8, v);
+    if (o.hl8 != nullptr) {
+      f16x8 h, l;
+#pragma unroll
+      for (int i = 0; i < 8; ++i) {
+        f16_t hh, ll;
+        hl_split(v[i], hh, ll);
+        h[i] = hh;
+        l[i] = ll;
+      }
+      f16_t* dst = o.hl8 + (long)b * o.obs_h + (long)p * o.ldo_h + 16 * g;
+      *reinterpret_cast<f16x8*>(dst) = h;
+      *reinterpret_cast<f16x8*>(dst + 8) = l;
+    }
   }
 }
 
@@ -208,8 +227,8 @@
 }
 
 template <typename T, typename OutT>
-static int launch_gn(const void* x, const float* prebias, const float* gamma, const float* beta, void* out, float* part, int B,
-                     int C, int HW, int nhwc, float eps, int relu, hipStream_t st) {
+static int launch_gn(const void* x, const float* prebias, const float* gamma, const float* beta, void* out, const GnOut* rows, float* part,
+                     int B, int C, int HW, int nhwc, float eps, int relu, hipStream_t st) {
   const int G = C / GN_CPG;
   if (nhwc) {
     const int npl = 256 / G;
@@ -226,8 +245,9 @@
                          eps, relu);
       return check_launch("group_norm");
     }
+    const GnOut o = rows != nullptr ? *rows : GnOut{(long)C, (long)HW * C, nullptr, 0, 0};
     hipLaunchKernelGGL((gn_apply_nhwc_kernel<T, OutT>), dim3(nchunk, B), dim3(256), 0, st, (const T*)x, prebias, part, gamma, beta,
-                       (OutT*)out, HW, G, nchunk, per, eps, relu);
+                       (OutT*)out, o, HW, G, nchunk, per, eps, relu);
   } else {
     int nchunk = max(1, min(GN_MAXK / GN_CPG, HW / 8192));
     int per = (HW + nchunk - 1) / nchunk;
@@ -241,13 +261,23 @@
 }
 
 template <typename T>
-static int gn_out(int od, const void* x, const float* prebias, const float* gamma, const float* beta, void* out, float* part, int B,
-                  int C, int HW, int nhwc, float eps, int relu, hipStream_t st) {
+static int gn_out(int od, const void* x, const float* prebias, const float* gamma, const float* beta, void* out, const GnOut* rows,
+                  float* part, int B, int C, int HW, int nhwc, float eps, int relu, hipStream_t st) {
   switch (od) {
-    case HIPIE_F32: return launch_gn<T, float>(x, prebias, gamma, beta, out, part, B, C, HW, nhwc, eps, relu, st);
-    case HIPIE_F16: return launch_gn<T, f16_t>(x, prebias, gamma, beta, out, part, B, C, HW, nhwc, eps, relu, st);
-    case HIPIE_BF16: return launch_gn<T, bf16_t>(x, prebias, gamma, beta, out, part, B, C, HW, nhwc, eps, relu, st);
+    case HIPIE_F32: return launch_gn<T, float>(x, prebias, gamma, beta, out, rows, part, B, C, HW, nhwc, eps, relu, st);
+    case HIPIE_F16: return launch_gn<T, f16_t>(x, prebias, gamma, beta, out, rows, part, B, C, HW, nhwc, eps, relu, st);
+    case HIPIE_BF16: return launch_gn<T, bf16_t>(x, prebias, gamma, beta, out, rows, part, B, C, HW, nhwc, eps, relu, st);
     default: return set_err(HIPIE_EINVAL, "group_norm: bad out dtype %d", od);
+  }
+}
+
+template <typename... A>
+static int gn_in(int xd, A... a) {
+  switch (xd) {
+    case HIPIE_F32: return gn_out<float>(a...);
+    case HIPIE_F16: return gn_out<f16_t>(a...);
+    case HIPIE_BF16: return gn_out<bf16_t>(a...);
+    default: return set_err(HIPIE_EINVAL, "group_norm: bad x dtype %d", xd);
   }
 }
 
@@ -266,10 +296,28 @@
                 "group_norm: channels_last %d (0 NCHW, 1 channels-last, 2 channels-last in / NCHW out: H*W %% 64 == 0, got %d)", channels_last, HW);
   if (B == 0) return HIPIE_OK;
   hipStream_t st = (hipStream_t)stream;
-  switch (x_dtype) {
-    case HIPIE_F32: return gn_out<float>(out_dtype, x, prebias, gamma, beta, out, workspace, B, C, HW, channels_last, eps, relu, st);
-    case HIPIE_F16: return gn_out<f16_t>(out_dtype, x, prebias, gamma, beta, out, workspace, B, C, HW, channels_last, eps, relu, st);
-    case HIPIE_BF16: return gn_out<bf16_t>(out_dtype, x, prebias, gamma, beta, out, workspace, B, C, HW, channels_last, eps, relu, st);
-    default: return set_err(HIPIE_EINVAL, "group_norm: bad x dtype %d", x_dtype);
-  }
-}
+  return gn_in(x_dtype, out_dtype, x, prebias, gamma, beta, out, (const GnOut*)nullptr, workspace, B, C, HW, channels_last, eps, relu, st);
+}
+
+extern "C" int hipie_group_norm_rows(const void* x, const float* prebias, const float* gamma, const float* beta, void* out, int64_t ldo,
+                                     void* out_hl8, int64_t ldo_hl8, int64_t out_rows, int64_t row0, float* workspace, int B, int C, int HW,
+                                     int groups, float eps, int relu, int x_dtype, int out_dtype, void* stream) {
+  using namespace hipie;
+  HIPIE_REQUIRE(x && gamma && beta && out && workspace, "group_norm_rows: null pointer");
+  HIPIE_REQUIRE(B >= 0 && C > 0 && HW > 0, "group_norm_rows: bad shape");
+  HIPIE_REQUIRE(groups > 0 && C == groups * GN_CPG && groups <= 64 && 256 % groups == 0,
+                "group_norm_rows: %d channels in %d groups unsupported (8 channels per group, 256 %% groups == 0)", C, groups);
+  HIPIE_REQUIRE(out_dtype == HIPIE_F32 || ((out_dtype == HIPIE_F16 || out_dtype == HIPIE_BF16) && out_hl8 == nullptr),
+                "group_norm_rows: out dtype %d (f32 | f16 | bf16; the HL8 second output goes with f32 rows)", out_dtype);
+  HIPIE_REQUIRE((uintptr_t)out % 32 == 0 && (uintptr_t)out_hl8 % 32 == 0, "group_norm_rows: outputs must be 32-byte aligned");
+  HIPIE_REQUIRE(ldo >= C && ldo % 8 == 0, "group_norm_rows: output row stride %ld (>= %d, a multiple of 8)", (long)ldo, C);
+  HIPIE_REQUIRE(out_hl8 == nullptr || (ldo_hl8 >= 2 * C && ldo_hl8 % 16 == 0), "group_norm_rows: HL8 output row stride %ld (>= %d, a multiple of 16)",
+                (long)ldo_hl8, 2 * C);
+  HIPIE_REQUIRE(row0 >= 0 && out_rows > 0 && row0 <= out_rows - HW, "group_norm_rows: rows %ld .. %ld beyond the buffer's %ld rows per image",
+                (long)row0, (long)row0 + HW, (long)out_rows);
+  if (B == 0) return HIPIE_OK;
+  const GnOut o = {(long)ldo, (long)out_rows * ldo, out_hl8 ? (f16_t*)out_hl8 + row0 * ldo_hl8 : nullptr, (long)ldo_hl8, (long)out_rows * ldo_hl8};
+  const size_t esz = out_dtype == HIPIE_F32 ? 4 : 2;
+  return gn_in(x_dtype, out_dtype, x, prebias, gamma, beta, (void*)((char*)out + (size_t)row0 * ldo * esz), &o, workspace, B, C, HW, 1, eps, relu,
+               (hipStream_t)stream);
+}
diff --git a/hipie_amd/modeling/ddetrs_dn.py b/hipie_amd/modeling/ddetrs_dn.py
--- a/hipie_amd/modeling/ddetrs_dn.py
+++ b/hipie_amd/modeling/ddetrs_dn.py
@@ -5,7 +5,7 @@
 from .. import ops
 from .maskdino import MaskDINOHead
 from .transformer import (MLP, FeatureResizer, NestedTensor, PConv2d, _get_clones, agg_lang_feat, expand_tokens, geo_cached, inverse_sigmoid,
-                          nested_tensor_from_images)
+                          nested_tensor_from_images, project_levels)
 
 
 _SIDE_STREAMS = {}
@@ -83,23 +83,28 @@
             lang_feat_pool = agg_lang_feat(language_dict_features["hidden"], language_dict_features["masks"]).unsqueeze(1)
         elif task != "detection":
             raise ValueError("task must be detection or grounding")
-        srcs, masks, poses = [], [], []
+        srcs, masks, poses, tokens = [], [], [], None
+        nf, nl = len(features), self.detr.num_feature_levels
+        if nl <= nf + 1:
+            srcs, tokens, _ = project_levels(self.detr.input_proj, [f.tensors for f in features] + [features[-1].tensors] * (nl - nf))
         for l, feat in enumerate(features):
             src, mask = feat.decompose()
-            srcs.append(self.detr.input_proj[l](src))
+            if nl > nf + 1:
+                srcs.append(self.detr.input_proj[l](src))
             masks.append(mask)
             poses.append(pos[l])
         gk = samples.geo_key
-        for l in range(len(features), self.detr.num_feature_levels):
-            src = self.detr.input_proj[l](features[-1].tensors if l == len(features) else srcs[-1])
+        for l in range(nf, nl):
+            src = srcs[l] if l < len(srcs) else self.detr.input_proj[l](features[-1].tensors if l == nf else srcs[-1])
             hw = tuple(src.shape[-2:])
             mask = geo_cached(gk, ("level_mask0", hw),
                               lambda: F.interpolate(masks[0][None].float(), size=hw).to(torch.bool)[0])
-            srcs.append(src)
+            if l >= len(srcs):
+                srcs.append(src)
             masks.append(mask)
             poses.append(geo_cached(gk, ("pos0", hw, src.dtype), lambda: self.detr.backbone[1](mask).to(src.dtype)))
         hs, memory, init_reference, inter_references, _, _, language_dict_features, spatial_shapes = \
-            self.detr.transformer(srcs, masks, poses, language_dict_features, task=task, geo_key=gk)
+            self.detr.transformer(srcs, masks, poses, language_dict_features, task=task, geo_key=gk, tokens=tokens)
 
         lang = lang_feat_pool if task in ("grounding", "sot") else language_dict_features["hidden"]
         if overlap:
diff --git a/hipie_amd/modeling/maskdino.py b/hipie_amd/modeling/maskdino.py
--- a/hipie_amd/modeling/maskdino.py
+++ b/hipie_amd/modeling/maskdino.py
@@ -7,7 +7,7 @@
 from .. import ops
 from .transformer import (MLP, _select_topk, DeformableTransformerDecoderLayer, DeformableTransformerEncoderLayer, FeatureResizer, geo_cached, level_pos_flat,
                           PConv2d, PGroupNorm, PLayerNorm, PLinear, PositionEmbeddingSine, _get_clones, encoder_reference_points,
-                          gen_encoder_output_proposals, level_tensors,
+                          gen_encoder_output_proposals, level_tensors, project_levels,
                           batched_decoder_values, decoder_box_refine, decoder_split_values, selected_proposal_boxes, decoder_fast_path, decoder_query_pos)
 
 
@@ -51,9 +51,9 @@
         self.encoder = MSDeformAttnTransformerEncoder(layer, num_layers)
         self.level_embed = nn.Parameter(torch.randn(num_levels, d_model))
 
-    def forward(self, srcs, pos_embeds):
+    def forward(self, srcs, pos_embeds, tokens=None, tokens_hl8=None):
         shapes_list = [tuple(int(v) for v in s.shape[-2:]) for s in srcs]
-        src = torch.cat([s.flatten(2).transpose(1, 2) for s in srcs], 1)
+        src = tokens if tokens is not None else torch.cat([s.flatten(2).transpose(1, 2) for s in srcs], 1)
         B = src.shape[0]
         gk = ("md_enc", B, tuple(shapes_list), str(src.device), src.dtype)
         pos = level_pos_flat(self, pos_embeds, src.dtype, gk)
@@ -61,6 +61,8 @@
         refs = geo_cached(gk, "enc_refs", lambda: encoder_reference_points(
             shapes_list, torch.ones(B, len(srcs), 2, device=src.device), src.device))
         q, n = None, len(self.encoder.layers)
+        if tokens is not None and tokens_hl8 is not None and self.encoder.layers[0].takes_hl8(src):
+            q = {"src_h": tokens_hl8}
         for i, layer in enumerate(self.encoder.layers):
             if i + 1 < n:
                 src, q = layer(src, pos, refs, spatial_shapes, level_start_index, None, query=q, want_query=True)
@@ -101,11 +103,12 @@
 
     def forward_features(self, features, masks=None):
         f3, f4, f5 = features["res3"], features["res4"], features["res5"]
-        extra = self.input_proj[3](f5)
-        srcs = [self.input_proj[i](f) for i, f in enumerate((f3, f4, f5))] + [extra]
+        l0 = self.transformer.encoder.layers[0]
+        srcs, tokens, tokens_hl8 = project_levels(self.input_proj, (f3, f4, f5, f5), want_hl8=getattr(l0, "split", False)
+                                                  and l0.linear1.weight.dtype == torch.float32)
         pos = [geo_cached(("md_pe", tuple(s.shape[0:1]) + tuple(s.shape[2:]), str(s.device)), "pos", lambda s=s: self.pe_layer(
             torch.zeros(s.shape[0], s.shape[2], s.shape[3], dtype=torch.bool, device=s.device))) for s in srcs]
-        y, shapes = self.transformer(srcs, pos)
+        y, shapes = self.transformer(srcs, pos, tokens, tokens_hl8)
         B = y.shape[0]
         out, st = [], 0
         y = y.contiguous()
diff --git a/hipie_amd/modeling/transformer.py b/hipie_amd/modeling/transformer.py
--- a/hipie_amd/modeling/transformer.py
+++ b/hipie_amd/modeling/transformer.py
@@ -86,6 +86,38 @@
             x = x + prebias.view(1, -1, 1, 1).to(x.dtype)
         y = F.group_norm(x, self.num_groups, self.weight.to(x.dtype), self.bias.to(x.dtype), self.eps)
         return F.relu(y) if relu else y
+
+
+TOKEN_STREAM_GN = True
+TOKEN_STREAM_HL8 = True
+
+
+def project_levels(projs, inputs, want_hl8=False):
+    if not (TOKEN_STREAM_GN and all(isinstance(p, nn.Sequential) and len(p) == 2 and isinstance(p[1], PGroupNorm) for p in projs)):
+        return [p(x) for p, x in zip(projs, inputs)], None, None
+    ys = [p[0](x) for p, x in zip(projs, inputs)]
+    rows_ok = [ops.group_norm_rows_ok(y, p[1].num_groups, p[1].weight) for p, y in zip(projs, ys)]
+    if not any(rows_ok) or any(y.dtype != ys[0].dtype or y.shape[:2] != ys[0].shape[:2] for y in ys):
+        return [p[1](y) for p, y in zip(projs, ys)], None, None
+    B, C = ys[0].shape[:2]
+    S = sum(y.shape[2] * y.shape[3] for y in ys)
+    tokens = torch.empty(B, S, C, dtype=ys[0].dtype, device=ys[0].device)
+    hl8 = None
+    if want_hl8 and TOKEN_STREAM_HL8 and tokens.dtype == torch.float32:
+        hl8 = torch.empty(B, S, 2 * C, dtype=torch.float16, device=tokens.device)
+    srcs, st = [], 0
+    for proj, y, ok in zip(projs, ys, rows_ok):
+        gn, n = proj[1], y.shape[2] * y.shape[3]
+        if ok:
+            srcs.append(ops.group_norm_rows(y, gn.num_groups, gn.weight, gn.bias, gn.eps, tokens, st, out_hl8=hl8))
+        else:
+            rows = tokens[:, st:st + n]
+            rows.copy_(gn(y).flatten(2).transpose(1, 2))
+            if hl8 is not None:
+                hl8[:, st:st + n].copy_(ops.to_hl8(rows.contiguous()))
+            srcs.append(rows.transpose(1, 2).unflatten(2, tuple(y.shape[2:])))
+        st += n
+    return srcs, tokens, hl8
 
 
 def cast_head(module, dtype, act=torch.float32):
@@ -447,8 +479,11 @@
         self.linear1, self.linear2 = PLinear(d_model, d_ffn), PLinear(d_ffn, d_model)
         self.norm2 = PLayerNorm(d_model)
 
+    def takes_hl8(self, src):
+        return getattr(self, "split", False) and src.is_cuda and src.dtype == torch.float32 and self.linear1.weight.dtype == torch.float32
+
     def forward(self, src, pos, reference_points, spatial_shapes, level_start_index, padding_mask=None, query=None, want_query=False):
-        if getattr(self, "split", False) and src.is_cuda and src.dtype == torch.float32 and self.linear1.weight.dtype == torch.float32:
+        if self.takes_hl8(src):
             return self._forward_split(src, pos, reference_points, spatial_shapes, level_start_index, padding_mask, query, want_query)
         q = src + pos if query is None else query
         src2 = self.self_attn(q, reference_points, src, spatial_shapes, level_start_index, padding_mask)
@@ -465,7 +500,8 @@
     attn = self.self_attn
     src = src.contiguous()
     if isinstance(carry, dict):
-        src_h, q_h = carry["src_h"], carry["q_h"]
+        src_h = carry["src_h"]
+        q_h = carry["q_h"] if "q_h" in carry else ops.add_to_hl8(src, _pos_hl8(self, pos))
     elif carry is None:
         src_h, q_h = ops.to_hl8(src), ops.add_to_hl8(src, _pos_hl8(self, pos))
     else:
@@ -772,9 +808,9 @@
         self.pinned_topk = None
         self.last_topk = None
 
-    def forward(self, srcs, masks, pos_embeds, language_dict_features, task=None, geo_key=None):
+    def forward(self, srcs, masks, pos_embeds, language_dict_features, task=None, geo_key=None, tokens=None):
         shapes_list = [tuple(int(v) for v in s.shape[-2:]) for s in srcs]
-        src = torch.cat([s.flatten(2).transpose(1, 2) for s in srcs], 1)
+        src = tokens if tokens is not None else torch.cat([s.flatten(2).transpose(1, 2) for s in srcs], 1)
         gk = None if geo_key is None else (geo_key, tuple(shapes_list), src.dtype)
         mask = geo_cached(gk, "mask_flat", lambda: torch.cat([m.flatten(1) for m in masks], 1))
         pos = level_pos_flat(self, pos_embeds, src.dtype, gk)
diff --git a/hipie_amd/ops.py b/hipie_amd/ops.py
--- a/hipie_amd/ops.py
+++ b/hipie_amd/ops.py
@@ -744,16 +744,46 @@
         out = torch.empty(B, C, H, W, dtype=out_dtype, device=x.device)
     else:
         out = torch.empty_like(x, dtype=out_dtype)
-    key = (str(x.device), B * groups, torch.cuda.current_stream(x.device).cuda_stream)
-    ws = _GN_WS.get(key)
-    if ws is None:
-        ws = _GN_WS[key] = torch.empty(2 * B * groups * 512, dtype=torch.float32, device=x.device)
+    ws = _gn_workspace(x, B, groups)
     rc = lib.hipie_group_norm(x.data_ptr(), None if prebias is None else _chk(prebias, "prebias", torch.float32),
                               _chk(weight, "weight", torch.float32), _chk(bias, "bias", torch.float32), out.data_ptr(),
                               ws.data_ptr(), B, C, H * W, groups, int(nhwc), float(eps), 1 if relu else 0,
                               _DT[x.dtype], _DT[out_dtype], _stream())
     _lib.check(rc, "hipie_group_norm")
     return out
+
+
+def _gn_workspace(x, B, groups):
+    key = (str(x.device), B * groups, torch.cuda.current_stream(x.device).cuda_stream)
+    ws = _GN_WS.get(key)
+    if ws is None:
+        ws = _GN_WS[key] = torch.empty(2 * B * groups * 512, dtype=torch.float32, device=x.device)
+    return ws
+
+
+def group_norm_rows_ok(x, groups, weight):
+    return (weight.dtype == torch.float32 and group_norm_ok(x, groups) and x.is_contiguous(memory_format=torch.channels_last)
+            and not (x.is_contiguous() and x.shape[1] > 1 and x.shape[2] * x.shape[3] > 1))
+
+
+@_timed("group_norm")
+def group_norm_rows(x, groups, weight, bias, eps, out, row0, out_hl8=None, relu=False, prebias=None):
+    lib = _lib.load()
+    B, C, H, W = x.shape
+    if not group_norm_rows_ok(x, groups, weight):
+        raise RuntimeError("group_norm_rows: x must be a channels-last (B, 8 * groups, H, W) device tensor")
+    if out.dim() != 3 or out.shape[0] != B or out.shape[2] != C or not out.is_contiguous() or out.dtype not in _DT or out.device != x.device:
+        raise RuntimeError("group_norm_rows: out must be a dense (B, S, C) device tensor")
+    if out_hl8 is not None and (out_hl8.shape != (B, out.shape[1], 2 * C) or out_hl8.dtype != torch.float16 or not out_hl8.is_contiguous()
+                                or out_hl8.device != x.device):
+        raise RuntimeError("group_norm_rows: out_hl8 must be a dense (B, S, 2C) fp16 device tensor")
+    rc = lib.hipie_group_norm_rows(x.data_ptr(), None if prebias is None else _chk(prebias, "prebias", torch.float32),
+                                   _chk(weight, "weight", torch.float32), _chk(bias, "bias", torch.float32), out.data_ptr(), C,
+                                   None if out_hl8 is None else out_hl8.data_ptr(), 2 * C, out.shape[1], int(row0),
+                                   _gn_workspace(x, B, groups).data_ptr(), B, C, H * W, groups, float(eps), 1 if relu else 0,
+                                   _DT[x.dtype], _DT[out.dtype], _stream())
+    _lib.check(rc, "hipie_group_norm_rows")
+    return out[:, row0:row0 + H * W].transpose(1, 2).unflatten(2, (H, W))
 
 
 @_timed("add_cast")
@@ -1236,7 +1266,7 @@
 
 
 @_timed("conv3x3_split")
-def conv3x3_split(x, conv, act=ACT_NONE):
+def conv3x3_split(x, conv, act=ACT_NONE, out=None, out_row=None):
     lib = _lib.load()
     B, C, H, W = x.shape
     N = conv.out_channels
@@ -1252,12 +1282,36 @@
     buf[guard:guard + rows].view(B, Hp, Wp, C)[:, 1:-1, 1:-1].copy_(x.permute(0, 2, 3, 1))
     w, b, _ = split_weight(conv, "w3x3", [conv.weight] + ([conv.bias] if conv.bias is not None else []),
                            lambda: conv.weight.permute(0, 2, 3, 1).reshape(N, 9 * C), (lambda: conv.bias) if conv.bias is not None else None)
+    xin = buf[guard:]
+    if out is not None or out_row is not None:
+        if (out is None or out_row is None or out.dim() != 2 or out.shape[1] != N or out_row.dtype != torch.int32 or out_row.numel() != rows
+                or out.device != x.device or out_row.device != x.device):
+            raise RuntimeError("conv3x3_split: out (rows_out, N) fp32 and out_row (B * (H + 2) * (W + 2)) int32 go together, on x's device")
+        rc = lib.hipie_conv3x3_split_rows(xin.data_ptr(), C, w.data_ptr(), None if b is None else b.data_ptr(), _chk(out, "out", torch.float32), N,
+                                          _chk(out_row, "out_row"), rows, Wp, C, N, F32, F32, int(act), _stream())
+        _lib.check(rc, "hipie_conv3x3_split_rows")
+        return out
+    if CONV3X3_ROW_MAP:
+        omap = derived(conv, "crop_rows", [], lambda: _crop_row_map(B, H, W, x.device), extra=(B, H, W, str(x.device)), keep=8)
+        out = torch.empty(B, H, W, N, dtype=torch.float32, device=x.device)
+        rc = lib.hipie_conv3x3_split_rows(xin.data_ptr(), C, w.data_ptr(), None if b is None else b.data_ptr(), out.data_ptr(), N,
+                                          omap.data_ptr(), rows, Wp, C, N, F32, F32, int(act), _stream())
+        _lib.check(rc, "hipie_conv3x3_split_rows")
+        return out.permute(0, 3, 1, 2)
     out = torch.empty(rows, N, dtype=torch.float32, device=x.device)
-    xin = buf[guard:]
     rc = lib.hipie_conv3x3_split(xin.data_ptr(), C, w.data_ptr(), None if b is None else b.data_ptr(), out.data_ptr(), N, rows, Wp, C, N,
                                  F32, F32, int(act), _stream())
     _lib.check(rc, "hipie_conv3x3_split")
     return out.view(B, Hp, Wp, N)[:, 1:-1, 1:-1].permute(0, 3, 1, 2).contiguous(memory_format=torch.channels_last)
+
+
+CONV3X3_ROW_MAP = True
+
+
+def _crop_row_map(B, H, W, device):
+    m = torch.full((B, H + 2, W + 2), -1, dtype=torch.int32)
+    m[:, 1:-1, 1:-1] = torch.arange(B * H * W, dtype=torch.int32).view(B, H, W)
+    return m.reshape(-1).to(device)
 
 
 _FFN_PERM = {}
diff --git a/include/hipie_mi355.h b/include/hipie_mi355.h
--- a/include/hipie_mi355.h
+++ b/include/hipie_mi355.h
@@ -130,6 +130,10 @@
 int hipie_group_norm(const void* x, const float* prebias, const float* gamma, const float* beta, void* out, float* workspace,
                      int B, int C, int HW, int groups, int channels_last, float eps, int relu, int x_dtype, int out_dtype,
                      void* stream);
+
+int hipie_group_norm_rows(const void* x, const float* prebias, const float* gamma, const float* beta, void* out, int64_t ldo,
+                          void* out_hl8, int64_t ldo_hl8, int64_t out_rows, int64_t row0, float* workspace, int B, int C, int HW,
+                          int groups, float eps, int relu, int x_dtype, int out_dtype, void* stream);
 
 int hipie_add_cast(const float* a, const void* b, void* out, int64_t n, int dtype, void* stream);
 
@@ -222,6 +226,8 @@
 
 int hipie_conv3x3_split(const void* x, int64_t ldx, const void* w, const float* bias, void* out, int64_t ldo, int64_t rows, int Wp, int C,
                         int N, int in_fmt, int out_fmt, int act, void* stream);
+int hipie_conv3x3_split_rows(const void* x, int64_t ldx, const void* w, const float* bias, void* out, int64_t ldo, const int32_t* out_row,
+                             int64_t rows, int Wp, int C, int N, int in_fmt, int out_fmt, int act, void* stream);
 
 int hipie_topk(const float* x, int64_t row_stride, int rows, int n, int k, int64_t* idx_out, float* val_out, void* stream);
 
```

Result: no change. 40.93 images/sec (-0.1%).
